# RichealYoung/BRIEF_PyTorch

Hardware: AMD Instinct MI355X
Metric: encode_voxels_per_sec (higher is better)
Workload: dtype f32; 1 GPU; SingleTask 512^3 synthetic uint16 volume, SIREN 4x256 (layers=5, features=256, w0=20), randompoint sample_size=100000, datal2, Adamax lr=1e-3; layers=5, features=256, sample_size=100000, params=198657

## Files before the change

### brief_pytorch_amd/csrc/brief_device.inc

```
typedef float f32x16 __attribute__((ext_vector_type(16)));
#define MFMA(a, b, c) __builtin_amdgcn_mfma_f32_32x32x2f32((a), (b), (c), 0, 0, 0)

#define ROWMAP(r, hi) (((r) & 3) + 8 * ((r) >> 2) + 4 * (hi))
template <int V> struct RoleC { static constexpr int value = V; };

template <int NT, bool INFER = false>
struct KCfg {
    static constexpr int WM = INFER ? brief_wm_infer(NT) : brief_wm(NT);
    static constexpr int WS = 4 / WM;
    static constexpr int MTW = (NT + WM - 1) / WM;
    static constexpr bool EXACT = (NT % WM) == 0;
    static constexpr int FP = 32 * NT;
    static constexpr int XS_FLOATS = WS * NT * 1024;
    static constexpr int TROWS = 32 * MTW;
    static constexpr int RS = (TROWS + 63) / 64;
    static constexpr int T_FLOATS = 4 * TROWS * 33;
    static constexpr int G_FLOATS = 4 * 256;
};

struct GridArgs {
    int ndim;
    int64_t dims[3];
    float lo, hi;
    float step[3];
    int fast;
    uint64_t magic[3];
};

struct BoxArgs {
    int64_t start[3], step[3], extent[3];
    uint64_t magic[3];
    int fast;
};

__device__ __forceinline__ uint32_t fast_div(uint32_t nn, uint64_t magic, uint32_t dv)
{
    return dv == 1 ? nn : (uint32_t)__umul64hi(magic, (uint64_t)nn);
}

struct FusedArgs {
    brief_siren_desc d;
    const float *pk;
    const float *coords;
    const float *targets;
    const float *weights;
    const int64_t *idx;
    int64_t offset;
    int64_t n;
    uint64_t rng_pop, rng_seed, rng_step;
    GridArgs grid;
    int loss_kind;
    float thr, beta, inv_count;
    float *Z;
    float *D;
    int64_t npad;
    float *rec;
    int64_t n_begin, n_end;
    int rec_base;
    void *S16[5];
    float *slabs;
    float *yhat_out;
    void *out;
    int out_kind;
    float scale_min, den, span, vmin;
    int stagger_cus;
    int stagger;
    int pers_wgs;
    int64_t pers_tiles;
    int diag;
};
struct FusedBoxArgs : FusedArgs {
    BoxArgs box;
};
template <bool BOX> struct KArgsT { using type = FusedArgs; };
template <> struct KArgsT<true> { using type = FusedBoxArgs; };
typedef const __attribute__((address_space(4))) FusedBoxArgs *kargs_box;

__device__ __forceinline__ void lds_barrier()
{
    asm volatile("s_waitcnt lgkmcnt(0)" ::: "memory");
    __builtin_amdgcn_s_barrier();
    asm volatile("" ::: "memory");
}

__device__ __forceinline__ float lin_coord(const GridArgs &g, int a, int64_t i)
{
    const int64_t nn = g.dims[a];
    if (nn == 1) return g.lo;
    return i < nn / 2 ? __fmaf_rn(g.step[a], (float)i, g.lo) : __fmaf_rn(-g.step[a], (float)(nn - 1 - i), g.hi);
}

__device__ __forceinline__ float lin_coord32(const GridArgs &g, int a, uint32_t i)
{
    const uint32_t nn = (uint32_t)g.dims[a];
    if (nn == 1) return g.lo;
    return i < nn / 2 ? __fmaf_rn(g.step[a], (float)i, g.lo) : __fmaf_rn(-g.step[a], (float)(nn - 1 - i), g.hi);
}

__device__ __forceinline__ void grid_coords(const GridArgs &g, int cin, int64_t j, float &x0, float &x1, float &x2)
{
    if (cin == 3) {
        int64_t id, ih, iw;
        if (g.fast) {
            const uint32_t ju = (uint32_t)j, d2 = (uint32_t)g.dims[2], d1 = (uint32_t)g.dims[1];
            const uint32_t t2 = fast_div(ju, g.magic[2], d2);
            const uint32_t t1 = fast_div(t2, g.magic[1], d1);
            x0 = lin_coord32(g, 0, t1);
            x1 = lin_coord32(g, 1, t2 - t1 * d1);
            x2 = lin_coord32(g, 2, ju - t2 * d2);
            return;
        } else {
            iw = j % g.dims[2];
            const int64_t t2 = j / g.dims[2];
            ih = t2 % g.dims[1]; id = t2 / g.dims[1];
        }
        x0 = lin_coord(g, 0, id);
        x1 = lin_coord(g, 1, ih);
        x2 = lin_coord(g, 2, iw);
    } else {
        int64_t ih, iw;
        if (g.fast) {
            const uint32_t ju = (uint32_t)j, d1 = (uint32_t)g.dims[1];
            const uint32_t t1 = fast_div(ju, g.magic[1], d1);
            x0 = lin_coord32(g, 0, t1);
            x1 = lin_coord32(g, 1, ju - t1 * d1);
            return;
        } else {
            iw = j % g.dims[1]; ih = j / g.dims[1];
        }
        x0 = lin_coord(g, 0, ih);
        x1 = lin_coord(g, 1, iw);
    }
}

__device__ __forceinline__ void box_coords(const GridArgs &g, int cin, int64_t b, float &x0, float &x1, float &x2)
{
    kargs_box ap = (kargs_box)__builtin_amdgcn_kernarg_segment_ptr();
    asm volatile("" : "+s"(ap));
    uint32_t i0, i1, i2 = 0u;
    if (cin == 3) {
        const uint32_t e2 = (uint32_t)ap->box.extent[2], e1 = (uint32_t)ap->box.extent[1];
        if (ap->box.fast) {
            const uint32_t bu = (uint32_t)b;
            const uint32_t t2 = fast_div(bu, ap->box.magic[2], e2);
            const uint32_t t1 = fast_div(t2, ap->box.magic[1], e1);
            i0 = t1; i1 = t2 - t1 * e1; i2 = bu - t2 * e2;
        } else {
            const int64_t t2 = b / (int64_t)e2, t1 = t2 / (int64_t)e1;
            i0 = (uint32_t)t1; i1 = (uint32_t)(t2 - t1 * e1); i2 = (uint32_t)(b - t2 * e2);
        }
    } else {
        const uint32_t e1 = (uint32_t)ap->box.extent[1];
        if (ap->box.fast) {
            const uint32_t bu = (uint32_t)b;
            const uint32_t t1 = fast_div(bu, ap->box.magic[1], e1);
            i0 = t1; i1 = bu - t1 * e1;
        } else {
            const int64_t t1 = b / (int64_t)e1;
            i0 = (uint32_t)t1; i1 = (uint32_t)(b - t1 * e1);
        }
    }
    x0 = lin_coord32(g, 0, (uint32_t)ap->box.start[0] + (uint32_t)ap->box.step[0] * i0);
    x1 = lin_coord32(g, 1, (uint32_t)ap->box.start[1] + (uint32_t)ap->box.step[1] * i1);
    if (cin == 3) x2 = lin_coord32(g, 2, (uint32_t)ap->box.start[2] + (uint32_t)ap->box.step[2] * i2);
}

template <bool BOX>
__device__ __forceinline__ void sample_coords(const GridArgs &g, int cin, int64_t j, float &x0, float &x1, float &x2)
{
    if constexpr (BOX) box_coords(g, cin, j, x0, x1, x2);
    else grid_coords(g, cin, j, x0, x1, x2);
}

typedef unsigned int u32x4 __attribute__((ext_vector_type(4)));

__device__ __forceinline__ float4 bload4(__amdgpu_buffer_rsrc_t rs, int voff, int soff)
{
    const u32x4 v = __builtin_amdgcn_raw_buffer_load_b128(rs, voff, soff, 0);
    return make_float4(__uint_as_float(v.x), __uint_as_float(v.y), __uint_as_float(v.z), __uint_as_float(v.w));
}
#ifndef BRIEF_WGRAD_AUX
#define BRIEF_WGRAD_AUX 0
#endif
__device__ __forceinline__ float4 bload4w(__amdgpu_buffer_rsrc_t rs, int voff, int soff)
{
    const u32x4 v = __builtin_amdgcn_raw_buffer_load_b128(rs, voff, soff, BRIEF_WGRAD_AUX);
    return make_float4(__uint_as_float(v.x), __uint_as_float(v.y), __uint_as_float(v.z), __uint_as_float(v.w));
}
__device__ __forceinline__ float bload1(__amdgpu_buffer_rsrc_t rs, int voff, int soff)
{
    return __uint_as_float(__builtin_amdgcn_raw_buffer_load_b32(rs, voff, soff, 0));
}
__device__ __forceinline__ void bstore1(float v, __amdgpu_buffer_rsrc_t rs, int voff, int soff)
{
    __builtin_amdgcn_raw_buffer_store_b32(__float_as_uint(v), rs, voff, soff, 0);
}
#ifndef BRIEF_STASH_LD_AUX
#define BRIEF_STASH_LD_AUX 0
#endif
#ifndef BRIEF_X3_STASH_AUX
#define BRIEF_X3_STASH_AUX 0
#endif
__device__ __forceinline__ float bload1s(__amdgpu_buffer_rsrc_t rs, int voff, int soff)
{
    return __uint_as_float(__builtin_amdgcn_raw_buffer_load_b32(rs, voff, soff, BRIEF_STASH_LD_AUX));
}
__device__ __forceinline__ void bstore1s(float v, __amdgpu_buffer_rsrc_t rs, int voff, int soff)
{
    __builtin_amdgcn_raw_buffer_store_b32(__float_as_uint(v), rs, voff, soff, BRIEF_X3_STASH_AUX);
}

template <int NT, bool INFER = false>
__device__ __forceinline__ void chain(f32x16 (&acc)[(KCfg<NT, INFER>::MTW)], __amdgpu_buffer_rsrc_t rs, int soff_layer ,
                                      const float4 *Xs, int wm, int lane, int kit)
{
    using K = KCfg<NT, INFER>;
    constexpr int NIT = NT * 4;
    constexpr int PD = NIT < 4 ? NIT : 4;
    const int voff = lane * 16;
    int soff_w = soff_layer + wm * (NT * 4 * 1024);
    asm volatile("" : "+s"(soff_w));
    constexpr int smul = 1024;
    float4 areg[NIT][K::MTW];
    float4 breg[NIT];
#pragma unroll
    for (int it = 0; it < PD; ++it)
#pragma unroll
        for (int t = 0; t < K::MTW; ++t)
            if (K::EXACT || wm + K::WM * t < NT) areg[it][t] = bload4(rs, voff, soff_w + (K::WM * t * NT * 4 + it) * smul);
    breg[0] = Xs[lane];
#pragma unroll
    for (int it = 0; it < NIT; ++it) {
        if (it >= NIT - 3 && it >= kit) break;
        if (it + PD < NIT) {
#pragma unroll
            for (int t = 0; t < K::MTW; ++t)
                if (K::EXACT || wm + K::WM * t < NT) {
                    areg[it + PD][t] = bload4(rs, voff, soff_w + (K::WM * t * NT * 4 + it + PD) * smul);
                }
        }
        if (it + 1 < NIT) breg[it + 1] = Xs[(it + 1) * 64 + lane];
        __builtin_amdgcn_sched_barrier(0);
        const float4 b = breg[it];
#pragma unroll
        for (int t = 0; t < K::MTW; ++t) {
            if (K::EXACT || wm + K::WM * t < NT) {
                const float4 a = areg[it][t];
                acc[t] = MFMA(a.x, b.x, acc[t]);
                acc[t] = MFMA(a.y, b.y, acc[t]);
                acc[t] = MFMA(a.z, b.z, acc[t]);
                acc[t] = MFMA(a.w, b.w, acc[t]);
            }
        }
    }
}

template <int NT, bool INFER = false>
__device__ __forceinline__ void write_image(float4 *Xs, const f32x16 (&h)[(KCfg<NT, INFER>::MTW)], int wm, int lane)
{
    using K = KCfg<NT, INFER>;
#pragma unroll
    for (int t = 0; t < K::MTW; ++t) {
        const int mt = wm + K::WM * t;
        if (K::EXACT || mt < NT) {
#pragma unroll
            for (int q = 0; q < 4; ++q)
                Xs[(mt * 4 + q) * 64 + lane] = make_float4(h[t][4 * q], h[t][4 * q + 1], h[t][4 * q + 2], h[t][4 * q + 3]);
        }
    }
}

__device__ __forceinline__ void philox_round(uint32_t (&c)[4], uint32_t k0, uint32_t k1)
{
    const uint64_t p0 = (uint64_t)0xD2511F53u * c[0], p1 = (uint64_t)0xCD9E8D57u * c[2];
    const uint32_t n0 = (uint32_t)(p1 >> 32) ^ c[1] ^ k0, n1 = (uint32_t)p1;
    const uint32_t n2 = (uint32_t)(p0 >> 32) ^ c[3] ^ k1, n3 = (uint32_t)p0;
    c[0] = n0; c[1] = n1; c[2] = n2; c[3] = n3;
}

__device__ __forceinline__ int64_t philox_index(int64_t i, uint64_t pop, uint64_t seed, uint64_t step)
{
    uint32_t c[4] = {(uint32_t)i, (uint32_t)((uint64_t)i >> 32), (uint32_t)step, (uint32_t)(step >> 32)};
    uint32_t k0 = (uint32_t)seed, k1 = (uint32_t)(seed >> 32);
#pragma unroll
    for (int r = 0; r < 10; ++r) {
        philox_round(c, k0, k1);
        k0 += 0x9E3779B9u; k1 += 0xBB67AE85u;
    }
    const uint64_t r64 = ((uint64_t)c[0] << 32) | c[1];
    return (int64_t)__umul64hi(r64, pop);
}

#ifndef BRIEF_FUSED64
#ifndef BRIEF_LEAN_RM3
#define BRIEF_LEAN_RM3 1
#endif
#define BRIEF_FUSED64 0
#endif
#ifndef BRIEF_KERNARG_RELOAD
#define BRIEF_KERNARG_RELOAD 1
#endif
#ifndef BRIEF_TRAIN_WPE
#define BRIEF_TRAIN_WPE 2
#endif
#if defined(BRIEF_STAMPS) && BRIEF_STAMPS + 0 != 2
#define STAMP(slot) { const long long t_ = clock64(); st_acc[slot] += (float)(t_ - st_last); st_last = t_; }
#else
#define STAMP(slot)
#endif
```

### brief_pytorch_amd/csrc/brief_fused.inc

```
template <int NT, bool INFER = false>
struct FusedLds {
    using K = KCfg<NT, INFER>;
    static constexpr int R_FLOATS = K::XS_FLOATS > K::T_FLOATS ? K::XS_FLOATS : K::T_FLOATS;
    static constexpr int G_OFF = R_FLOATS;
    static constexpr int HW_OFF = G_OFF + K::G_FLOATS;
    static constexpr int TOTAL = HW_OFF + 4 * K::FP + 4;
};

#ifndef BRIEF_LEAN
#define BRIEF_LEAN 1
#endif
#ifndef BRIEF_LEAN7
#define BRIEF_LEAN7 0
#endif
constexpr bool fused_lean(int NT) { return BRIEF_LEAN && (NT == 8 || NT == BRIEF_LEAN7); }
constexpr int fused_train_wpe(int NT) { return NT > 8 ? 1 : (NT <= 4 || fused_lean(NT) ? (BRIEF_TRAIN_WPE > 3 ? BRIEF_TRAIN_WPE : 3) : BRIEF_TRAIN_WPE); }
template <int NT, bool TRAIN, bool BOX = false>
__global__ __launch_bounds__(256, TRAIN ? fused_train_wpe(NT) : (NT > 8 ? 2 : 3)) void k_fused(const typename KArgsT<BOX>::type a)
{
    static_assert(!(TRAIN && BOX), "the box mapping is an inference instantiation");
#ifdef BRIEF_STAMPS
    float st_acc[10] = {0.f, 0.f, 0.f, 0.f, 0.f, 0.f, 0.f, 0.f, 0.f, 0.f};
    long long st_last = clock64();
    const long long st_c0 = st_last, st_r0 = wall_clock64();
#endif
    using K = KCfg<NT, !TRAIN>;
    using LD = FusedLds<NT, !TRAIN>;
    extern __shared__ __attribute__((aligned(16))) float smem[];
    float4 *X = reinterpret_cast<float4 *>(smem);
    float *T = smem;
    float *G = smem + LD::G_OFF;
    float *HW = smem + LD::HW_OFF;

    const int lane = threadIdx.x & 63;
    const int wave = __builtin_amdgcn_readfirstlane(threadIdx.x >> 6);
    const int hi = lane >> 5, ln = lane & 31;
    const int wm = wave % K::WM, ws = wave / K::WM;
    const brief_siren_desc &d = a.d;
    const int L = d.layers, cin = d.cin, cout = d.cout;
    const int kit = (d.features + 7) >> 3;
    const int64_t npad = a.npad;
    const float *pk = a.pk;
    float4 *Xs = X + ws * (NT * 256);
    float *Tw = T + wave * (K::TROWS * 33);
    float *Gw = G + wave * 256;
    const float4 *W0p = reinterpret_cast<const float4 *>(pk + brief_pk_w0(d));
    const __amdgpu_buffer_rsrc_t rs_pk =
        __builtin_amdgcn_make_buffer_rsrc((void *)pk, 0, (int)(brief_pk_count(d) * 4), 0x00020000);
    const int stash_bytes = (a.diag & 1) ? 0 : (int)((int64_t)K::FP * npad * 4);

    {
        const float *headp = pk + brief_pk_head(d);
        for (int e = threadIdx.x; e < 4 * K::FP + 4; e += 256) HW[e] = headp[e];
    }
    {
        const int slot = (int)blockIdx.x < a.pers_wgs ? blockIdx.x / a.stagger_cus : 0;
        for (int i = 0; i < slot * a.stagger; ++i) __builtin_amdgcn_s_sleep(127);
    }
    lds_barrier();

    float acc0[K::RS][4], accWh[K::RS][4];
#pragma unroll
    for (int rs = 0; rs < K::RS; ++rs)
#pragma unroll
        for (int c = 0; c < 4; ++c) { acc0[rs][c] = 0.f; accWh[rs][c] = 0.f; }
    float accbh[4] = {0.f, 0.f, 0.f, 0.f};
    float lsum = 0.f;

    const bool pers = (int)blockIdx.x < a.pers_wgs;
    const int64_t tile_end = pers ? a.pers_tiles : a.pers_tiles + ((int64_t)blockIdx.x - a.pers_wgs) + 1;
    const int64_t tile_step = pers ? a.pers_wgs : 1;
    for (int64_t tile = pers ? (int64_t)blockIdx.x : a.pers_tiles + ((int64_t)blockIdx.x - a.pers_wgs); tile < tile_end; tile += tile_step) {
        const int64_t n0 = (tile * K::WS + ws) * 32;
        const int64_t n = n0 + ln;
        const bool valid = n < a.n;
#if BRIEF_KERNARG_RELOAD
        typedef const __attribute__((address_space(4))) FusedArgs *kargs_f;
        kargs_f ap = (kargs_f)__builtin_amdgcn_kernarg_segment_ptr();
        asm volatile("" : "+s"(ap));
        const int64_t *k_idx = ap->idx;
        const float *k_tg = ap->targets, *k_wt = ap->weights, *k_co = ap->coords;
        const uint64_t k_pop = ap->rng_pop, k_seed = ap->rng_seed, k_step = ap->rng_step;
        const int64_t k_off = ap->offset;
        GridArgs kg;
        kg.ndim = ap->grid.ndim; kg.lo = ap->grid.lo; kg.hi = ap->grid.hi; kg.fast = ap->grid.fast;
#pragma unroll
        for (int ax = 0; ax < 3; ++ax) { kg.dims[ax] = ap->grid.dims[ax]; kg.step[ax] = ap->grid.step[ax]; kg.magic[ax] = ap->grid.magic[ax]; }
#else
        const int64_t *k_idx = a.idx;
        const float *k_tg = a.targets, *k_wt = a.weights, *k_co = a.coords;
        const uint64_t k_pop = a.rng_pop, k_seed = a.rng_seed, k_step = a.rng_step;
        const int64_t k_off = a.offset;
        const GridArgs &kg = a.grid;
#endif
        int64_t j = 0;
        if (valid) j = k_idx ? k_idx[n] : (k_pop ? philox_index(n, k_pop, k_seed, k_step) : n + k_off);
        float x0 = 0.f, x1 = 0.f, x2 = 0.f;
        float yv[4] = {0.f, 0.f, 0.f, 0.f}, wv4[4] = {1.f, 1.f, 1.f, 1.f};
        if (valid) {
            if (TRAIN) {
#pragma unroll
                for (int c = 0; c < 4; ++c) {
                    if (c < cout) {
                        yv[c] = k_tg[j * cout + c];
                        if (k_wt) wv4[c] = k_wt[j * cout + c];
                    }
                }
            }
            if (k_co) {
                x0 = k_co[j * cin];
                x1 = k_co[j * cin + 1];
                if (cin == 3) x2 = k_co[j * cin + 2];
            } else {
                sample_coords<BOX>(kg, cin, j, x0, x1, x2);
            }
        }
        f32x16 acc[K::MTW];
        f32x16 creg[K::MTW];
        f32x16 hreg[K::MTW];
        float4 bnext[K::MTW][4];
#pragma unroll
        for (int t = 0; t < K::MTW; ++t) {
#pragma unroll
            for (int r = 0; r < 16; ++r) { creg[t][r] = 0.f; hreg[t][r] = 0.f; }
#pragma unroll
            for (int q = 0; q < 4; ++q) bnext[t][q] = make_float4(0.f, 0.f, 0.f, 0.f);
        }
#define FUSED_LOAD_BIAS(layer)                                                                          \
    {                                                                                                   \
        const float *bp_ = pk + brief_pk_hidden(d, (layer)) + 2 * K::FP * K::FP;                        \
        _Pragma("unroll") for (int t = 0; t < K::MTW; ++t) {                                            \
            const int mt = wm + K::WM * t;                                                              \
            if (K::EXACT || mt < NT) {                                                                  \
                _Pragma("unroll") for (int q = 0; q < 4; ++q)                                           \
                    bnext[t][q] = *reinterpret_cast<const float4 *>(bp_ + 32 * mt + 8 * q + 4 * hi);    \
            }                                                                                           \
        }                                                                                               \
    }
        {
            const float b0 = hi ? x1 : x0;
            const float b1 = hi ? 1.0f : x2;
#pragma unroll
            for (int t = 0; t < K::MTW; ++t) {
                const int mt = wm + K::WM * t;
#pragma unroll
                for (int r = 0; r < 16; ++r) acc[t][r] = 0.f;
                if (K::EXACT || mt < NT) {
                    const float4 w = W0p[32 * mt + ln];
                    acc[t] = MFMA(hi ? w.y : w.x, b0, acc[t]);
                    acc[t] = MFMA(hi ? w.w : w.z, b1, acc[t]);
                }
            }
        }
        STAMP(0)
        for (int l = 0; l <= L - 2; ++l) {
            const bool last = (l == L - 2);
            if (l > 0) {
                if (TRAIN && fused_lean(NT)) FUSED_LOAD_BIAS(l)
#pragma unroll
                for (int t = 0; t < K::MTW; ++t) {
#pragma unroll
                    for (int q = 0; q < 4; ++q) {
                        acc[t][4 * q] = bnext[t][q].x; acc[t][4 * q + 1] = bnext[t][q].y;
                        acc[t][4 * q + 2] = bnext[t][q].z; acc[t][4 * q + 3] = bnext[t][q].w;
                    }
                }
                if (TRAIN) __builtin_amdgcn_s_setprio(3);
                chain<NT, !TRAIN>(acc, rs_pk, (int)(brief_pk_hidden(d, l) * 4), Xs, wm, lane, kit);
                if (TRAIN) __builtin_amdgcn_s_setprio(0);
                STAMP(1)
                lds_barrier();
                STAMP(2)
            }
            if (!last && !(TRAIN && fused_lean(NT))) FUSED_LOAD_BIAS(l + 1)
#pragma unroll
            for (int t = 0; t < K::MTW; ++t) {
                const int mt = wm + K::WM * t;
                if (K::EXACT || mt < NT) {
#pragma unroll
                    for (int r = 0; r < 16; ++r) acc[t][r] = __builtin_amdgcn_fractf(acc[t][r]);
                    if (TRAIN && !last) {
                        const __amdgpu_buffer_rsrc_t rz =
                            __builtin_amdgcn_make_buffer_rsrc((void *)(a.Z + (int64_t)l * K::FP * npad), 0, stash_bytes, 0x00020000);
                        const int voff = (int)(n0 * (K::FP * 4)) + ln * 4 + hi * 4 * 128;
#pragma unroll
                        for (int r = 0; r < 16; ++r)
                            bstore1(acc[t][r], rz, voff, (32 * mt + (r & 3) + 8 * (r >> 2)) * 128);
                    }
#pragma unroll
                    for (int r = 0; r < 16; ++r) hreg[t][r] = BRIEF_SIN_REV(acc[t][r]);
                }
            }
            if (TRAIN && last) {
                asm volatile("" ::: "memory");
#pragma unroll
                for (int t = 0; t < K::MTW; ++t) {
                    if (K::EXACT || wm + K::WM * t < NT) {
#pragma unroll
                        for (int r = 0; r < 16; ++r) creg[t][r] = BRIEF_COS_REV(acc[t][r]);
                    }
                }
            }
            write_image<NT, !TRAIN>(Xs, hreg, wm, lane);
            STAMP(3)
            lds_barrier();
            STAMP(4)
        }
        float zo[4], yh[4], g[4];
#pragma unroll
        for (int c = 0; c < 4; ++c) {
            zo[c] = 0.f; yh[c] = 0.f; g[c] = 0.f;
            if (c < cout) {
                float p = 0.f;
                const float *wrow = HW + c * K::FP;
#pragma unroll
                for (int kt = 0; kt < NT; ++kt) {
#pragma unroll
                    for (int q = 0; q < 4; ++q) {
                        const float4 hv = Xs[(kt * 4 + q) * 64 + lane];
                        const float4 wv = *reinterpret_cast<const float4 *>(wrow + 32 * kt + 8 * q + 4 * hi);
                        p = __fmaf_rn(wv.x, hv.x, p); p = __fmaf_rn(wv.y, hv.y, p);
                        p = __fmaf_rn(wv.z, hv.z, p); p = __fmaf_rn(wv.w, hv.w, p);
                    }
                }
                p += __shfl_xor(p, 32);
                zo[c] = p + HW[4 * K::FP + c];
                yh[c] = d.output_act ? brief_fast_sinf(d.w0_hidden * zo[c]) : zo[c];
            }
        }
        if (!TRAIN) {
            if (wm == 0 && hi == 0 && valid) {
#pragma unroll
                for (int c = 0; c < 4; ++c) {
                    if (c >= cout) break;
                    if (a.out_kind == BRIEF_OUT_F32) {
                        reinterpret_cast<float *>(a.out)[n * cout + c] = yh[c];
                    } else {
                        float t = __fsub_rn(yh[c], a.scale_min);
                        t = __fdiv_rn(t, a.den);
                        t = fminf(fmaxf(t, 0.f), 1.f);
                        const float u = __fadd_rn(__fmul_rn(t, a.span), a.vmin);
                        if (a.out_kind == BRIEF_OUT_U16) reinterpret_cast<uint16_t *>(a.out)[n * cout + c] = (uint16_t)(int)u;
                        else reinterpret_cast<uint8_t *>(a.out)[n * cout + c] = (uint8_t)(int)u;
                    }
                }
            }
            lds_barrier();
            continue;
        }
#pragma unroll
        for (int c = 0; c < 4; ++c) {
            if (c < cout && valid) {
                float we = wv4[c];
                if (a.thr != 0.f && yh[c] <= a.thr) we = 1.0f;
                const float df = yh[c] - yv[c];
                float li, gi;
                if (a.loss_kind == BRIEF_LOSS_L2) { li = df * df; gi = 2.0f * df; }
                else if (a.loss_kind == BRIEF_LOSS_SMOOTHL1) {
                    const float ad = fabsf(df);
                    if (ad < a.beta) { li = 0.5f * df * df / a.beta; gi = df / a.beta; }
                    else { li = ad - 0.5f * a.beta; gi = df < 0.f ? -1.0f : 1.0f; }
                } else { li = 0.f; gi = 0.f; }
                if (wm == 0 && hi == 0) lsum += li * we;
                g[c] = a.loss_kind == BRIEF_LOSS_EXTERNAL ? yv[c] : gi * we * a.inv_count;
                if (d.output_act) g[c] *= d.w0_hidden * brief_fast_cosf(d.w0_hidden * zo[c]);
                if (a.yhat_out && wm == 0 && hi == 0) a.yhat_out[n * cout + c] = yh[c];
            }
        }
        STAMP(5)
        lds_barrier();
#pragma unroll
        for (int t = 0; t < K::MTW; ++t) {
#pragma unroll
            for (int r = 0; r < 16; ++r) Tw[(32 * t + ROWMAP(r, hi)) * 33 + ln] = hreg[t][r];
        }
        if (hi == 0) *reinterpret_cast<float4 *>(Gw + ln * 4) = make_float4(g[0], g[1], g[2], g[3]);
        else *reinterpret_cast<float4 *>(Gw + 128 + ln * 4) = make_float4(x0, x1, x2, 1.0f);
        lds_barrier();
#pragma unroll
        for (int rs = 0; rs < K::RS; ++rs) {
            float4 sW = make_float4(0.f, 0.f, 0.f, 0.f), sb = make_float4(0.f, 0.f, 0.f, 0.f);
            const int row = lane + 64 * rs;
            const float *trow = Tw + (row < K::TROWS ? row : 0) * 33;
            if (cout == 1) {
#pragma unroll 8
                for (int s = 0; s < 32; ++s) {
                    const float gv = Gw[s * 4];
                    sW.x = __fmaf_rn(trow[s], gv, sW.x);
                    sb.x += gv;
                }
            } else {
#pragma unroll 4
                for (int s = 0; s < 32; ++s) {
                    const float hv = trow[s];
                    const float4 gv = *reinterpret_cast<const float4 *>(Gw + s * 4);
                    sW.x = __fmaf_rn(hv, gv.x, sW.x); sW.y = __fmaf_rn(hv, gv.y, sW.y);
                    sW.z = __fmaf_rn(hv, gv.z, sW.z); sW.w = __fmaf_rn(hv, gv.w, sW.w);
                    sb.x += gv.x; sb.y += gv.y; sb.z += gv.z; sb.w += gv.w;
                }
            }
            if (row < K::TROWS) { accWh[rs][0] += sW.x; accWh[rs][1] += sW.y; accWh[rs][2] += sW.z; accWh[rs][3] += sW.w; }
            if (rs == 0) { accbh[0] += sb.x; accbh[1] += sb.y; accbh[2] += sb.z; accbh[3] += sb.w; }
        }
        f32x16 dl[K::MTW];
        float gom[4];
        {
            const float om_top = (L - 2) == 0 ? d.w0_first : d.w0_hidden;
#pragma unroll
            for (int c = 0; c < 4; ++c) gom[c] = om_top * g[c];
        }
#pragma unroll
        for (int t = 0; t < K::MTW; ++t) {
            const int mt = wm + K::WM * t;
#pragma unroll
            for (int r = 0; r < 16; ++r) dl[t][r] = 0.f;
            if (K::EXACT || mt < NT) {
#pragma unroll
                for (int q = 0; q < 4; ++q) {
                    float4 sacc = make_float4(0.f, 0.f, 0.f, 0.f);
#pragma unroll
                    for (int c = 0; c < 4; ++c) {
                        if (c < cout) {
                            const float4 wv = *reinterpret_cast<const float4 *>(HW + c * K::FP + 32 * mt + 8 * q + 4 * hi);
                            sacc.x = __fmaf_rn(wv.x, gom[c], sacc.x); sacc.y = __fmaf_rn(wv.y, gom[c], sacc.y);
                            sacc.z = __fmaf_rn(wv.z, gom[c], sacc.z); sacc.w = __fmaf_rn(wv.w, gom[c], sacc.w);
                        }
                    }
                    dl[t][4 * q] = creg[t][4 * q] * sacc.x; dl[t][4 * q + 1] = creg[t][4 * q + 1] * sacc.y;
                    dl[t][4 * q + 2] = creg[t][4 * q + 2] * sacc.z; dl[t][4 * q + 3] = creg[t][4 * q + 3] * sacc.w;
                }
            }
        }
        STAMP(6)
        for (int l = L - 2; l >= 1; --l) {
            const __amdgpu_buffer_rsrc_t rd =
                __builtin_amdgcn_make_buffer_rsrc((void *)(a.D + (int64_t)(l - 1) * K::FP * npad), 0, stash_bytes, 0x00020000);
            const int voff_s = (int)(n0 * (K::FP * 4)) + ln * 4 + hi * 4 * 128;
#pragma unroll
            for (int t = 0; t < K::MTW; ++t) {
                const int mt = wm + K::WM * t;
                if (K::EXACT || mt < NT) {
#pragma unroll
                    for (int r = 0; r < 16; ++r)
                        bstore1(dl[t][r], rd, voff_s, (32 * mt + (r & 3) + 8 * (r >> 2)) * 128);
                }
            }
            const __amdgpu_buffer_rsrc_t rzp =
                __builtin_amdgcn_make_buffer_rsrc((void *)(a.Z + (int64_t)(l - 1) * K::FP * npad), 0, stash_bytes, 0x00020000);
            float zr[K::MTW][16];
            constexpr bool ZPRE = !fused_lean(NT);
#define FUSED_LOAD_Z()                                                                                  \
    _Pragma("unroll") for (int t = 0; t < K::MTW; ++t) {                                                \
        const int mt = wm + K::WM * t;                                                                  \
        _Pragma("unroll") for (int r = 0; r < 16; ++r) {                                                \
            zr[t][r] = 0.f;                                                                             \
            if (K::EXACT || mt < NT) zr[t][r] = bload1s(rzp, voff_s, (32 * mt + (r & 3) + 8 * (r >> 2)) * 128); \
        }                                                                                               \
    }
            if (ZPRE) FUSED_LOAD_Z()
            STAMP(7)
            lds_barrier();
            write_image<NT, !TRAIN>(Xs, dl, wm, lane);
            lds_barrier();
            STAMP(8)
#pragma unroll
            for (int t = 0; t < K::MTW; ++t)
#pragma unroll
                for (int r = 0; r < 16; ++r) acc[t][r] = 0.f;
            __builtin_amdgcn_s_setprio(3);
            chain<NT, !TRAIN>(acc, rs_pk, (int)((brief_pk_hidden(d, l) + K::FP * K::FP) * 4), Xs, wm, lane, kit);
            __builtin_amdgcn_s_setprio(0);
            STAMP(9)
            if (!ZPRE) FUSED_LOAD_Z()
#undef FUSED_LOAD_Z
#pragma unroll
            for (int t = 0; t < K::MTW; ++t) {
                const int mt = wm + K::WM * t;
                if (K::EXACT || mt < NT) {
#pragma unroll
                    for (int r = 0; r < 16; ++r)
                        dl[t][r] = acc[t][r] * BRIEF_COS_REV(zr[t][r]);
                }
            }
        }
        STAMP(7)
        lds_barrier();
#pragma unroll
        for (int t = 0; t < K::MTW; ++t) {
#pragma unroll
            for (int r = 0; r < 16; ++r) Tw[(32 * t + ROWMAP(r, hi)) * 33 + ln] = dl[t][r];
        }
        lds_barrier();
#pragma unroll
        for (int rs = 0; rs < K::RS; ++rs) {
            float4 s0 = make_float4(0.f, 0.f, 0.f, 0.f);
            const int row = lane + 64 * rs;
            const float *trow = Tw + (row < K::TROWS ? row : 0) * 33;
#pragma unroll 4
            for (int s = 0; s < 32; ++s) {
                const float dv = trow[s];
                const float4 xv = *reinterpret_cast<const float4 *>(Gw + 128 + s * 4);
                s0.x = __fmaf_rn(dv, xv.x, s0.x); s0.y = __fmaf_rn(dv, xv.y, s0.y);
                s0.z = __fmaf_rn(dv, xv.z, s0.z); s0.w = __fmaf_rn(dv, xv.w, s0.w);
            }
            if (row < K::TROWS) { acc0[rs][0] += s0.x; acc0[rs][1] += s0.y; acc0[rs][2] += s0.z; acc0[rs][3] += s0.w; }
        }
        lds_barrier();
        STAMP(6)
    }
#undef FUSED_LOAD_BIAS
    if (TRAIN) {
        float *rec = a.rec + (((int64_t)blockIdx.x + a.rec_base) * 4 + wave) * BRIEF_REC_FLOATS;
#pragma unroll
        for (int rs = 0; rs < K::RS; ++rs) {
            const int row = lane + 64 * rs;
            if (row < 128) {
#pragma unroll
                for (int c = 0; c < 4; ++c) {
                    rec[row * 4 + c] = acc0[rs][c];
                    rec[BRIEF_REC_DWH + c * 128 + row] = accWh[rs][c];
                }
            }
        }
        for (int off = 32; off >= 1; off >>= 1) lsum += __shfl_xor(lsum, off);
        if (lane == 0) {
#pragma unroll
            for (int c = 0; c < 4; ++c) rec[BRIEF_REC_DBH + c] = accbh[c];
            rec[BRIEF_REC_LOSS] = lsum;
#ifdef BRIEF_STAMPS
            for (int i = 0; i < 10; ++i) rec[BRIEF_REC_STAMPS + i] = st_acc[i];
            rec[BRIEF_REC_STAMPS + 10] = (float)(clock64() - st_c0);
            rec[BRIEF_REC_STAMPS + 11] = (float)(wall_clock64() - st_r0);
            rec[BRIEF_REC_STAMPS + 12] = (float)(st_r0 & 0xFFFFFF);
            rec[BRIEF_REC_STAMPS + 13] = (float)(__builtin_amdgcn_s_getreg(20 | (0 << 6) | (3 << 11)) & 15);
            rec[BRIEF_REC_STAMPS + 14] = (float)(__builtin_amdgcn_s_getreg(4 | (0 << 6) | (15 << 11)) & 0xFFFF);
#endif
        }
    }
}
```

### brief_pytorch_amd/csrc/brief_layout.h

```cpp
#pragma once
#include <stddef.h>
#include <stdint.h>
#include "../../include/brief_hip.h"

#if defined(__HIPCC__)
#define BL_HD __host__ __device__ __forceinline__
#else
#define BL_HD static inline
#endif

#define BRIEF_MAX_NT 128
#define BRIEF_REC_FLOATS 1056
#define BRIEF_REC_DWH 512
#define BRIEF_REC_DBH 1024
#define BRIEF_REC_LOSS 1028
#define BRIEF_REC_STAMPS 1030
BL_HD int brief_rec_tr(int nt) { return nt > 32 ? 32 * ((nt + 3) / 4) : (nt > 16 ? 256 : 128); }
BL_HD int brief_rec_floats(int nt) { return 8 * brief_rec_tr(nt) + 32; }

BL_HD int64_t brief_canon_hidden_off(const brief_siren_desc &d, int l )
{
    const int64_t F = d.features;
    return F * d.cin + F + (int64_t)(l - 1) * (F * F + F);
}
BL_HD int64_t brief_canon_head_off(const brief_siren_desc &d)
{
    const int64_t F = d.features;
    return F * d.cin + F + (int64_t)(d.layers - 2) * (F * F + F);
}
BL_HD int64_t brief_canon_count(const brief_siren_desc &d)
{
    return brief_canon_head_off(d) + (int64_t)d.features * d.cout + d.cout;
}

BL_HD int brief_nt(const brief_siren_desc &d)
{
    const int nt = (d.features + 31) / 32;
    if (d.precision == BRIEF_PREC_BF16) return nt <= 8 ? 8 : 16;
    if (d.precision == BRIEF_PREC_BF16X3) return 8;
    return nt;
}
#ifndef BRIEF_LEAN3
#define BRIEF_LEAN3 1
#endif
BL_HD bool brief_use_wide(const brief_siren_desc &d) { return d.precision == BRIEF_PREC_F32 && (d.features + 31) / 32 > 32; }
BL_HD bool brief_use_lean(const brief_siren_desc &d, bool train)
{
    const int nt = brief_nt(d);
    if (nt > 32) return false;
    if (train) return (nt >= 5 && nt != 8) || (BRIEF_LEAN3 && nt == 3);
    return (nt >= 5 && nt <= 7) || (nt >= 9 && nt != 12 && nt != 16);
}
BL_HD int64_t brief_pk_w0(const brief_siren_desc &) { return 0; }
BL_HD int64_t brief_pk_hidden_stride(const brief_siren_desc &d)
{
    const int64_t FP = 32 * brief_nt(d);
    return 2 * FP * FP + FP;
}
BL_HD int64_t brief_pk_hidden(const brief_siren_desc &d, int l )
{
    const int64_t FP = 32 * brief_nt(d);
    return FP * 4 + (int64_t)(l - 1) * brief_pk_hidden_stride(d);
}
BL_HD int64_t brief_pk_head(const brief_siren_desc &d)
{
    const int64_t FP = 32 * brief_nt(d);
    return FP * 4 + (int64_t)(d.layers - 2) * brief_pk_hidden_stride(d);
}
BL_HD int64_t brief_pk_count32(const brief_siren_desc &d)
{
    const int64_t FP = 32 * brief_nt(d);
    return brief_pk_head(d) + 4 * FP + 4;
}
BL_HD int64_t brief_pk16_off(const brief_siren_desc &d, int l )
{
    const int64_t FP = 32 * brief_nt(d);
    return ((brief_pk_count32(d) + 3) / 4) * 4 + (int64_t)(l - 1) * FP * FP;
}
BL_HD int64_t brief_pk16_region(const brief_siren_desc &d)
{
    const int64_t FP = 32 * brief_nt(d), hidden = d.layers - 2 > 0 ? d.layers - 2 : 0;
    return hidden * FP * FP;
}
BL_HD int64_t brief_pk_count(const brief_siren_desc &d)
{
    if (d.precision == BRIEF_PREC_BF16) return brief_pk16_off(d, 1) + brief_pk16_region(d);
    if (d.precision == BRIEF_PREC_BF16X3) return brief_pk16_off(d, 1) + 2 * brief_pk16_region(d);
    return brief_pk_count32(d);
}
BL_HD int64_t brief_frag16_index(int NT, int row, int col)
{
    const int mt = row >> 5, i = row & 31, kt = col >> 5, rem = col & 31;
    const int s = rem >> 4, r16 = rem & 15, hi = (r16 >> 2) & 1, j = ((r16 >> 3) << 2) | (r16 & 3);
    return ((((int64_t)mt * NT + kt) * 2 + s) * 64 + 32 * hi + i) * 8 + j;
}

BL_HD float brief_om_prev(const brief_siren_desc &d, int l) { return l - 1 == 0 ? d.w0_first : d.w0_hidden; }
BL_HD float brief_phase_scale(const brief_siren_desc &d, int l) { return (l == 0 ? d.w0_first : d.w0_hidden) * 0.15915494309189535f; }

BL_HD constexpr int brief_wm(int nt) { return nt >= 3 ? 4 : nt; }
BL_HD constexpr int brief_wm_infer(int nt) { return nt == 3 ? 1 : (nt == 5 ? 4 : brief_wm(nt)); }
BL_HD constexpr int brief_ws(int nt) { return 4 / brief_wm(nt); }
BL_HD int64_t brief_wg_samples(int nt) { return 32 * brief_ws(nt); }
BL_HD int64_t brief_npad(int nt, int64_t n)
{
    const int64_t g = brief_wg_samples(nt);
    return (n + g - 1) / g * g;
}
BL_HD int64_t brief_npad_d(const brief_siren_desc &d, int64_t n) { return brief_npad(brief_nt(d), n); }
```

### brief_pytorch_amd/csrc/brief_lean.inc

```
#ifndef BRIEF_LEAN_KTAIL
#define BRIEF_LEAN_KTAIL 1
#endif
constexpr bool lean_ktail(int MTW, bool train) { return BRIEF_LEAN_KTAIL && (!train || MTW != 2); }
struct LeanLds { int r, g_off, hw_off, part_off, total; };
__host__ __device__ inline LeanLds lean_lds(int SH, int MTW, int nt)
{
    LeanLds l;
    const int img = SH * nt * 1024, t = SH * 4 * 32 * MTW * 33;
    l.r = img > t ? img : t;
    l.g_off = l.r;
    l.hw_off = l.g_off + 4 * 256;
    l.part_off = l.hw_off + 4 * 32 * nt;
    l.total = l.part_off + SH * 4 * 32 * 4;
    return l;
}

template <int SH, int MTW, int RM, bool KTAIL>
__device__ __forceinline__ void lean_chain_rt(f32x16 (&acc)[SH][MTW], f32x16 &px, __amdgpu_buffer_rsrc_t rs, int soff_layer , const float4 *X,
                                              int wave, int lane, int nt, int kit, bool two)
{
    constexpr int KF = RM == 0 ? MTW : MTW - 1;
    const int voff = lane * 16;
    const int HALF = nt * 256;
    const int rho = RM == 1 ? ((wave + 1) & 3) : (RM == 2 ? (((wave >> 1) + 1) & 1) : (RM == 3 ? ((0x3201 >> (4 * wave)) & 3) : 0));
    int soff_t[KF > 0 ? KF : 1];
#pragma unroll
    for (int t = 0; t < KF; ++t) {
        const int mt = wave + 4 * t;
        soff_t[t] = soff_layer + (mt < nt ? mt : nt - 1) * nt * 4096;
    }
    const int soff_e = soff_layer + (RM == 1 ? nt - 1 : (RM == 2 ? nt - 2 + (wave & 1) : nt - 3 + ((wave + 1) >> 1))) * nt * 4096;
    const int soff_a = soff_layer + (nt - 3 + (wave & 2)) * nt * 4096;
    float4 areg[4][KF > 0 ? KF : 1];
    float4 aext[RM == 3 ? 3 : 2];
#pragma unroll
    for (int q = 0; q < 4; ++q) {
        const int it0 = (q + rho) & 3;
#pragma unroll
        for (int t = 0; t < KF; ++t) areg[q][t] = bload4(rs, voff, soff_t[t] + it0 * 1024);
        if ((RM == 1 && q == 3) || (RM == 2 && (q & 1))) aext[q >> 1] = bload4(rs, voff, soff_e + it0 * 1024);
        if (RM == 3 && q < 3) aext[q] = bload4(rs, voff, (q == 0 ? soff_a : soff_e) + it0 * 1024);
        __builtin_amdgcn_sched_barrier(0);
    }
#define LEAN_POS_MFMAS(q, B)                                                                                 \
    {                                                                                                        \
        _Pragma("unroll") for (int t = 0; t < KF; ++t) {                                                     \
            const float4 a = areg[q][t];                                                                     \
            _Pragma("unroll") for (int h = 0; h < SH; ++h) {                                                 \
                if (SH == 2 && h == 1 && !two) continue;                                                     \
                acc[h][t] = MFMA(a.x, B[h].x, acc[h][t]);                                                    \
                acc[h][t] = MFMA(a.y, B[h].y, acc[h][t]);                                                    \
                acc[h][t] = MFMA(a.z, B[h].z, acc[h][t]);                                                    \
                acc[h][t] = MFMA(a.w, B[h].w, acc[h][t]);                                                    \
            }                                                                                                \
        }                                                                                                    \
        if ((RM == 1 && q == 3) || (RM == 2 && (q & 1)) || (RM == 3 && (q == 1 || q == 2))) {                \
            const float4 a = aext[RM == 3 ? q : q >> 1];                                                     \
            _Pragma("unroll") for (int h = 0; h < SH; ++h) {                                                 \
                if (SH == 2 && h == 1 && !two) continue;                                                     \
                acc[h][MTW - 1] = MFMA(a.x, B[h].x, acc[h][MTW - 1]);                                        \
                acc[h][MTW - 1] = MFMA(a.y, B[h].y, acc[h][MTW - 1]);                                        \
                acc[h][MTW - 1] = MFMA(a.z, B[h].z, acc[h][MTW - 1]);                                        \
                acc[h][MTW - 1] = MFMA(a.w, B[h].w, acc[h][MTW - 1]);                                        \
            }                                                                                                \
        }                                                                                                    \
        if (RM == 3 && q == 0) {                                                                             \
            const float4 a = aext[0];                                                                        \
            px = MFMA(a.x, B[0].x, px); px = MFMA(a.y, B[0].y, px);                                          \
            px = MFMA(a.z, B[0].z, px); px = MFMA(a.w, B[0].w, px);                                          \
        }                                                                                                    \
    }
    float4 bcur[SH], bnxt[SH];
#pragma unroll
    for (int h = 0; h < SH; ++h) bcur[h] = X[h * HALF + rho * 64 + lane];
    const int nkt = KTAIL ? kit >> 2 : (kit + 3) >> 2;
    for (int kt = 0; kt < nkt; ++kt) {
#pragma unroll
        for (int q = 0; q < 4; ++q) {
            const int it = kt * 4 + ((q + rho) & 3);
            const int itn = q < 3 ? kt * 4 + ((q + 1 + rho) & 3) : kt * 4 + 4 + rho;
#pragma unroll
            for (int h = 0; h < SH; ++h) bnxt[h] = X[h * HALF + itn * 64 + lane];
            __builtin_amdgcn_sched_barrier(0);
            LEAN_POS_MFMAS(q, bcur)
            __builtin_amdgcn_sched_barrier(0);
#pragma unroll
            for (int t = 0; t < KF; ++t) areg[q][t] = bload4(rs, voff, soff_t[t] + (it + 4) * 1024);
            if ((RM == 1 && q == 3) || (RM == 2 && (q & 1))) aext[q >> 1] = bload4(rs, voff, soff_e + (it + 4) * 1024);
            if (RM == 3 && q < 3) aext[q] = bload4(rs, voff, (q == 0 ? soff_a : soff_e) + (it + 4) * 1024);
#pragma unroll
            for (int h = 0; h < SH; ++h) bcur[h] = bnxt[h];
        }
    }
    if (KTAIL && (kit & 3)) {
#pragma unroll
        for (int q = 0; q < 4; ++q) {
            const int it = nkt * 4 + ((q + rho) & 3);
            if (it < kit) {
                float4 bt[SH];
#pragma unroll
                for (int h = 0; h < SH; ++h) bt[h] = X[h * HALF + it * 64 + lane];
                LEAN_POS_MFMAS(q, bt)
            }
        }
    }
#undef LEAN_POS_MFMAS
}

template <int SH, int MTW, int RM>
__device__ __forceinline__ void lean_fold_shared(f32x16 (&acc)[SH][MTW], float *PS, int wave, int lane, bool two)
{
    if (RM != 0) {
        const bool giver = RM == 1 ? wave != 0 : wave >= 2;
        const int slot = RM == 1 ? wave - 1 : wave - 2;
        if (giver) {
#pragma unroll
            for (int h = 0; h < SH; ++h) {
                if (SH == 2 && h == 1 && !two) continue;
#pragma unroll
                for (int r = 0; r < 16; ++r) PS[((h * 3 + slot) * 16 + r) * 64 + lane] = acc[h][MTW - 1][r];
            }
        }
    }
    lds_barrier();
    if (RM == 1 && wave == 0) {
#pragma unroll
        for (int h = 0; h < SH; ++h) {
            if (SH == 2 && h == 1 && !two) continue;
#pragma unroll
            for (int s3 = 0; s3 < 3; ++s3)
#pragma unroll
                for (int r = 0; r < 16; ++r) acc[h][MTW - 1][r] += PS[((h * 3 + s3) * 16 + r) * 64 + lane];
        }
    }
    if (RM == 2 && wave < 2) {
#pragma unroll
        for (int h = 0; h < SH; ++h) {
            if (SH == 2 && h == 1 && !two) continue;
#pragma unroll
            for (int r = 0; r < 16; ++r) acc[h][MTW - 1][r] += PS[((h * 3 + wave) * 16 + r) * 64 + lane];
        }
    }
}

template <int MTW>
__device__ __forceinline__ void lean_fold3(f32x16 (&acc)[1][MTW], f32x16 &px, float *img, int wave, int lane)
{
    lds_barrier();
    if (wave == 3) {
#pragma unroll
        for (int r = 0; r < 16; ++r) img[2048 + r * 64 + lane] = acc[0][MTW - 1][r] + px[r];
    } else if (wave == 2) {
#pragma unroll
        for (int r = 0; r < 16; ++r) { img[1024 + r * 64 + lane] = acc[0][MTW - 1][r]; acc[0][MTW - 1][r] = px[r]; }
    } else if (wave == 1) {
#pragma unroll
        for (int r = 0; r < 16; ++r) img[r * 64 + lane] = px[r];
    } else {
#pragma unroll
        for (int r = 0; r < 16; ++r) acc[0][MTW - 1][r] += px[r];
    }
    lds_barrier();
    if (wave < 3) {
#pragma unroll
        for (int r = 0; r < 16; ++r) acc[0][MTW - 1][r] += img[wave * 1024 + r * 64 + lane];
    }
}

template <int SH, int MTW, int NTC>
__device__ __forceinline__ void lean_chain_ct(f32x16 (&acc)[SH][MTW], __amdgpu_buffer_rsrc_t rs, int soff_layer , const float4 *X,
                                              int wave, int lane, int kit, bool two)
{
    constexpr int NT = NTC > 0 ? NTC : 1, NIT = NT * 4, PD = 4, HALF = NT * 256;
    constexpr bool EXACT = MTW * 4 == NT;
    const int voff = lane * 16;
    int soff_w = soff_layer + wave * (NT * 4 * 1024);
    asm volatile("" : "+s"(soff_w));
    float4 areg[NIT][MTW];
    float4 breg[NIT][SH];
#pragma unroll
    for (int it = 0; it < PD; ++it)
#pragma unroll
        for (int t = 0; t < MTW; ++t)
            if (EXACT || wave + 4 * t < NT) areg[it][t] = bload4(rs, voff, soff_w + (4 * t * NT * 4 + it) * 1024);
#pragma unroll
    for (int h = 0; h < SH; ++h) breg[0][h] = X[h * HALF + lane];
#pragma unroll
    for (int it = 0; it < NIT; ++it) {
        if (it >= NIT - 3 && it >= kit) break;
        if (it + PD < NIT) {
#pragma unroll
            for (int t = 0; t < MTW; ++t)
                if (EXACT || wave + 4 * t < NT) areg[it + PD][t] = bload4(rs, voff, soff_w + (4 * t * NT * 4 + it + PD) * 1024);
        }
        if (it + 1 < NIT) {
#pragma unroll
            for (int h = 0; h < SH; ++h) breg[it + 1][h] = X[h * HALF + (it + 1) * 64 + lane];
        }
        __builtin_amdgcn_sched_barrier(0);
#pragma unroll
        for (int t = 0; t < MTW; ++t) {
            if (EXACT || wave + 4 * t < NT) {
                const float4 a = areg[it][t];
#pragma unroll
                for (int h = 0; h < SH; ++h) {
                    if (h == 1 && !two) continue;
                    const float4 b = breg[it][h];
                    acc[h][t] = MFMA(a.x, b.x, acc[h][t]);
                    acc[h][t] = MFMA(a.y, b.y, acc[h][t]);
                    acc[h][t] = MFMA(a.z, b.z, acc[h][t]);
                    acc[h][t] = MFMA(a.w, b.w, acc[h][t]);
                }
            }
        }
    }
}

#ifndef BRIEF_LEAN_WPE2
#define BRIEF_LEAN_WPE2 3
#endif
constexpr int lean_wpe(int SH, int MTW) { return SH == 1 && MTW <= 2 ? BRIEF_LEAN_WPE2 : (SH == 2 || MTW <= 4 ? 2 : 1); }

template <int SH, int MTW, int NTC, bool TRAIN, int RM = 0, bool BOX = false>
__global__ __launch_bounds__(256, lean_wpe(SH, MTW)) void k_lean(const typename KArgsT<BOX>::type a)
{
    static_assert(!(TRAIN && BOX), "the box mapping is an inference instantiation");
    static_assert(SH == 1 || SH == 2, "one or two 32-sample halves per tile");
    static_assert(RM == 0 || (NTC == 0 && SH == 1 && (MTW >= 2 || RM == 3)), "shared left-over tiles: run-time widths only (MTW = 1: the three tiles of a 3-tile net)");
    constexpr int TROWS = 32 * MTW;
    constexpr int RS = (TROWS + 63) / 64;
    constexpr int TR = MTW > 4 ? 256 : 128;
    const brief_siren_desc &d = a.d;
    const int nt = NTC > 0 ? NTC : brief_nt(d);
    const int FP = 32 * nt, HALF = nt * 256;
    extern __shared__ __attribute__((aligned(16))) float smem[];
    const LeanLds lds = lean_lds(SH, MTW, nt);
    float4 *X = reinterpret_cast<float4 *>(smem);
    float *T = smem;
    float *G = smem + lds.g_off;
    float *HW = smem + lds.hw_off;
    float4 *PART = reinterpret_cast<float4 *>(smem + lds.part_off);
    const int lane = threadIdx.x & 63;
    const int wave_hw = __builtin_amdgcn_readfirstlane(threadIdx.x >> 6);
    const int wave = (NTC == 0 && lean_wpe(SH, MTW) == 2) ? ((wave_hw + 2 * (((int)blockIdx.x / a.stagger_cus) & 1)) & 3) : wave_hw;
    const int hi = lane >> 5, ln = lane & 31;
    const int L = d.layers, cin = d.cin, cout = d.cout;
    const int kit = (d.features + 7) >> 3;
    const int64_t npad = a.npad;
    const float *pk = a.pk;
    float *Gw = G + wave * 256;
    const float4 *W0p = reinterpret_cast<const float4 *>(pk + brief_pk_w0(d));
    const __amdgpu_buffer_rsrc_t rs_pk = __builtin_amdgcn_make_buffer_rsrc((void *)pk, 0, (int)(brief_pk_count(d) * 4), 0x00020000);
    const int stash_bytes = (int)((int64_t)FP * npad * 4);
    const int64_t hstride = brief_pk_hidden_stride(d);
    bool tv[MTW];
#pragma unroll
    for (int t = 0; t < MTW; ++t) tv[t] = wave + 4 * t < nt;
    {
        const float *headp = pk + brief_pk_head(d);
        for (int e = threadIdx.x; e < 4 * FP; e += 256) HW[e] = headp[e];
    }
    lds_barrier();
    float acc0[RS][4], accWh[RS][4];
#pragma unroll
    for (int rs = 0; rs < RS; ++rs)
#pragma unroll
        for (int c = 0; c < 4; ++c) { acc0[rs][c] = 0.f; accWh[rs][c] = 0.f; }
    float accbh[4] = {0.f, 0.f, 0.f, 0.f};
    float lsum = 0.f;
    const int64_t T0 = SH == 1 ? a.n_begin >> 5 : 0;
    const int64_t Hn = ((SH == 1 && a.n_end > 0 ? a.n_end : a.n) + 31) >> 5;
    const int64_t G_ = gridDim.x, w_ = blockIdx.x;
    const int64_t R_ = SH == 2 ? Hn / (2 * G_) : (Hn - T0 > w_ ? (Hn - T0 - w_ + G_ - 1) / G_ : 0);
    const int64_t Hr = Hn - 2 * G_ * R_;
    const int64_t npair_x = Hr > G_ ? Hr - G_ : 0;
    const int64_t nsing_x = Hr > G_ ? G_ - npair_x : Hr;
    const int extra = SH == 2 ? (w_ < npair_x ? 2 : (w_ < npair_x + nsing_x ? 1 : 0)) : 0;
    const int64_t ht_x = 2 * G_ * R_ + (w_ < npair_x ? 2 * w_ : 2 * npair_x + (w_ - npair_x));
    for (int64_t it_ = 0; it_ < R_ + (extra ? 1 : 0); ++it_) {
        const int64_t ht = SH == 2 ? (it_ < R_ ? 2 * (it_ * G_ + w_) : ht_x) : T0 + it_ * G_ + w_;
        const bool two = SH == 2 && (it_ < R_ || extra == 2);
        typedef const __attribute__((address_space(4))) FusedArgs *kargs_f;
        kargs_f ap = (kargs_f)__builtin_amdgcn_kernarg_segment_ptr();
        asm volatile("" : "+s"(ap));
        const int64_t *k_idx = ap->idx;
        const float *k_tg = ap->targets, *k_wt = ap->weights, *k_co = ap->coords;
        const uint64_t k_pop = ap->rng_pop, k_seed = ap->rng_seed, k_step = ap->rng_step;
        const int64_t k_off = ap->offset;
        GridArgs kg;
        kg.ndim = ap->grid.ndim; kg.lo = ap->grid.lo; kg.hi = ap->grid.hi; kg.fast = ap->grid.fast;
#pragma unroll
        for (int ax = 0; ax < 3; ++ax) { kg.dims[ax] = ap->grid.dims[ax]; kg.step[ax] = ap->grid.step[ax]; kg.magic[ax] = ap->grid.magic[ax]; }
        float x0[SH], x1[SH], x2[SH];
        int64_t jidx[SH];
        bool valid[SH];
        f32x16 acc[SH][MTW];
        f32x16 px;
        {
            const int64_t n64 = ht * 32 + (SH == 2 ? lane : ln);
            const bool v64 = (SH == 1 || lane < 32 || two) && n64 < a.n;
            int64_t j = 0;
            if (v64) j = k_idx ? k_idx[n64] : (k_pop ? philox_index(n64, k_pop, k_seed, k_step) : n64 + k_off);
            float c0 = 0.f, c1 = 0.f, c2 = 0.f;
            if (v64) {
                if (k_co) {
                    c0 = k_co[j * cin];
                    c1 = k_co[j * cin + 1];
                    if (cin == 3) c2 = k_co[j * cin + 2];
                } else {
                    sample_coords<BOX>(kg, cin, j, c0, c1, c2);
                }
            }
            if (SH == 2) {
                const int jl = (int)(uint32_t)(uint64_t)j, jh = (int)(uint32_t)((uint64_t)j >> 32);
#pragma unroll
                for (int h = 0; h < SH; ++h) {
                    const int src = 32 * h + ln;
                    x0[h] = __shfl(c0, src); x1[h] = __shfl(c1, src); x2[h] = __shfl(c2, src);
                    jidx[h] = (int64_t)(((uint64_t)(uint32_t)__shfl(jh, src) << 32) | (uint32_t)__shfl(jl, src));
                    valid[h] = (h == 0 || two) && (ht + h) * 32 + ln < a.n;
                }
            } else {
                x0[0] = c0; x1[0] = c1; x2[0] = c2; jidx[0] = j; valid[0] = v64;
            }
        }
#pragma unroll
        for (int h = 0; h < SH; ++h) {
            const float b0 = hi ? x1[h] : x0[h];
            const float b1 = hi ? 1.0f : x2[h];
#pragma unroll
            for (int t = 0; t < MTW; ++t) {
#pragma unroll
                for (int r = 0; r < 16; ++r) acc[h][t][r] = 0.f;
                if (tv[t]) {
                    const float4 w = W0p[32 * (wave + 4 * t) + ln];
                    acc[h][t] = MFMA(hi ? w.y : w.x, b0, acc[h][t]);
                    acc[h][t] = MFMA(hi ? w.w : w.z, b1, acc[h][t]);
                }
            }
        }
        for (int l = 0; l <= L - 2; ++l) {
            const bool last = (l == L - 2);
            if (l > 0) {
                const float *bp_ = pk + FP * 4 + (int64_t)(l - 1) * hstride + 2 * (int64_t)FP * FP;
#pragma unroll
                for (int t = 0; t < MTW; ++t) {
                    if (tv[t]) {
#pragma unroll
                        for (int q = 0; q < 4; ++q) {
                            const float4 b4 = *reinterpret_cast<const float4 *>(bp_ + 32 * (wave + 4 * t) + 8 * q + 4 * hi);
#pragma unroll
                            for (int h = 0; h < SH; ++h) {
                                acc[h][t][4 * q] = b4.x; acc[h][t][4 * q + 1] = b4.y; acc[h][t][4 * q + 2] = b4.z; acc[h][t][4 * q + 3] = b4.w;
                            }
                        }
                    } else if (RM != 0 && t == MTW - 1) {
#pragma unroll
                        for (int h = 0; h < SH; ++h)
#pragma unroll
                            for (int r = 0; r < 16; ++r) acc[h][t][r] = 0.f;
                    }
                }
                const int soff_l = (int)((FP * 4 + (int64_t)(l - 1) * hstride) * 4);
                __builtin_amdgcn_s_setprio(3);
                if (RM == 3) {
#pragma unroll
                    for (int r = 0; r < 16; ++r) {
                        px[r] = wave == 2 ? acc[0][MTW - 1][r] : 0.f;
                        if (wave == 2) acc[0][MTW - 1][r] = 0.f;
                    }
                }
                if (NTC > 0) lean_chain_ct<SH, MTW, NTC>(acc, rs_pk, soff_l, X, wave, lane, kit, two);
                else lean_chain_rt<SH, MTW, RM, lean_ktail(MTW, TRAIN)>(acc, px, rs_pk, soff_l, X, wave, lane, nt, kit, two);
                __builtin_amdgcn_s_setprio(0);
                if constexpr (RM == 3) lean_fold3<MTW>(acc, px, T, wave, lane);
                else lean_fold_shared<SH, MTW, RM>(acc, T + SH * nt * 1024, wave, lane, two);
                if (RM != 0 && TRAIN && last) lds_barrier();
            }
            float pph[SH][4];
#pragma unroll
            for (int h = 0; h < SH; ++h) {
#pragma unroll
                for (int c = 0; c < 4; ++c) pph[h][c] = 0.f;
                if (h == 1 && !two) continue;
                const int voff = (int)(((ht + h) * 32) * ((int64_t)FP * 4)) + ln * 4 + hi * 4 * 128;
#pragma unroll
                for (int t = 0; t < MTW; ++t) {
                    if (!tv[t]) continue;
                    const int mt = wave + 4 * t;
#pragma unroll
                    for (int r = 0; r < 16; ++r) acc[h][t][r] = __builtin_amdgcn_fractf(acc[h][t][r]);
                    f32x16 hv;
                    if (!last) {
                        if (TRAIN) {
                            const __amdgpu_buffer_rsrc_t rz =
                                __builtin_amdgcn_make_buffer_rsrc((void *)(a.Z + (int64_t)l * FP * npad), 0, stash_bytes, 0x00020000);
#pragma unroll
                            for (int r = 0; r < 16; ++r) bstore1(acc[h][t][r], rz, voff, (32 * mt + (r & 3) + 8 * (r >> 2)) * 128);
                        }
#pragma unroll
                        for (int r = 0; r < 16; ++r) hv[r] = BRIEF_SIN_REV(acc[h][t][r]);
#pragma unroll
                        for (int q = 0; q < 4; ++q)
                            X[h * HALF + (mt * 4 + q) * 64 + lane] = make_float4(hv[4 * q], hv[4 * q + 1], hv[4 * q + 2], hv[4 * q + 3]);
                    } else {
#pragma unroll
                        for (int r = 0; r < 16; ++r) { hv[r] = BRIEF_SIN_REV(acc[h][t][r]); if (TRAIN) acc[h][t][r] = BRIEF_COS_REV(acc[h][t][r]); }
#pragma unroll
                        for (int c = 0; c < 4; ++c) {
                            if (c < cout) {
#pragma unroll
                                for (int q = 0; q < 4; ++q) {
                                    const float4 wv = *reinterpret_cast<const float4 *>(HW + c * FP + 32 * mt + 8 * q + 4 * hi);
                                    pph[h][c] = __fmaf_rn(wv.x, hv[4 * q], pph[h][c]); pph[h][c] = __fmaf_rn(wv.y, hv[4 * q + 1], pph[h][c]);
                                    pph[h][c] = __fmaf_rn(wv.z, hv[4 * q + 2], pph[h][c]); pph[h][c] = __fmaf_rn(wv.w, hv[4 * q + 3], pph[h][c]);
                                }
                            }
                        }
                        if (TRAIN) {
                            float *Th = T + (wave * SH + h) * (TROWS * 33);
#pragma unroll
                            for (int r = 0; r < 16; ++r) Th[(32 * t + ROWMAP(r, hi)) * 33 + ln] = hv[r];
                        }
                    }
                }
                if (last) {
#pragma unroll
                    for (int c = 0; c < 4; ++c) pph[h][c] += __shfl_xor(pph[h][c], 32);
                    if (hi == 0) PART[(h * 4 + wave) * 32 + ln] = make_float4(pph[h][0], pph[h][1], pph[h][2], pph[h][3]);
                }
            }
            lds_barrier();
        }
        float zo[SH][4], yh[SH][4], g[SH][4];
#pragma unroll
        for (int h = 0; h < SH; ++h) {
            float4 tot = PART[(h * 4) * 32 + ln];
#pragma unroll
            for (int w = 1; w < 4; ++w) {
                const float4 v = PART[(h * 4 + w) * 32 + ln];
                tot.x += v.x; tot.y += v.y; tot.z += v.z; tot.w += v.w;
            }
            const float tt[4] = {tot.x, tot.y, tot.z, tot.w};
            const int64_t n = (ht + h) * 32 + ln;
#pragma unroll
            for (int c = 0; c < 4; ++c) {
                zo[h][c] = 0.f; yh[h][c] = 0.f; g[h][c] = 0.f;
                if (c < cout) {
                    zo[h][c] = tt[c] + pk[brief_pk_head(d) + 4 * (int64_t)FP + c];
                    yh[h][c] = d.output_act ? brief_fast_sinf(d.w0_hidden * zo[h][c]) : zo[h][c];
                }
                if (!TRAIN) {
                    if (c < cout && valid[h] && wave == 0 && hi == 0) {
                        if (a.out_kind == BRIEF_OUT_F32) {
                            reinterpret_cast<float *>(a.out)[n * cout + c] = yh[h][c];
                        } else {
                            float t_ = __fsub_rn(yh[h][c], a.scale_min);
                            t_ = __fdiv_rn(t_, a.den);
                            t_ = fminf(fmaxf(t_, 0.f), 1.f);
                            const float u_ = __fadd_rn(__fmul_rn(t_, a.span), a.vmin);
                            if (a.out_kind == BRIEF_OUT_U16) reinterpret_cast<uint16_t *>(a.out)[n * cout + c] = (uint16_t)(int)u_;
                            else reinterpret_cast<uint8_t *>(a.out)[n * cout + c] = (uint8_t)(int)u_;
                        }
                    }
                    continue;
                }
                if (c < cout && valid[h]) {
                    const float yvc = k_tg[jidx[h] * cout + c];
                    float we = k_wt ? k_wt[jidx[h] * cout + c] : 1.0f;
                    if (a.thr != 0.f && yh[h][c] <= a.thr) we = 1.0f;
                    const float df = yh[h][c] - yvc;
                    float li, gi;
                    if (a.loss_kind == BRIEF_LOSS_L2) { li = df * df; gi = 2.0f * df; }
                    else if (a.loss_kind == BRIEF_LOSS_SMOOTHL1) {
                        const float ad = fabsf(df);
                        if (ad < a.beta) { li = 0.5f * df * df / a.beta; gi = df / a.beta; }
                        else { li = ad - 0.5f * a.beta; gi = df < 0.f ? -1.0f : 1.0f; }
                    } else { li = 0.f; gi = 0.f; }
                    if (wave == 0 && hi == 0) lsum += li * we;
                    g[h][c] = a.loss_kind == BRIEF_LOSS_EXTERNAL ? yvc : gi * we * a.inv_count;
                    if (d.output_act) g[h][c] *= d.w0_hidden * brief_fast_cosf(d.w0_hidden * zo[h][c]);
                    if (a.yhat_out && wave == 0 && hi == 0) a.yhat_out[n * cout + c] = yh[h][c];
                }
            }
        }
        if (!TRAIN) {
            lds_barrier();
            continue;
        }
#pragma unroll
        for (int h = 0; h < SH; ++h) {
            if (h == 1 && !two) continue;
            if (hi == 0) *reinterpret_cast<float4 *>(Gw + ln * 4) = make_float4(g[h][0], g[h][1], g[h][2], g[h][3]);
            asm volatile("s_waitcnt lgkmcnt(0)" ::: "memory");
#pragma unroll
            for (int rs = 0; rs < RS; ++rs) {
                float4 sW = make_float4(0.f, 0.f, 0.f, 0.f), sb = make_float4(0.f, 0.f, 0.f, 0.f);
                const int row = lane + 64 * rs;
                const float *trow = T + (wave * SH + h) * (TROWS * 33) + (row < TROWS ? row : 0) * 33;
                if (cout == 1) {
#pragma unroll 8
                    for (int s = 0; s < 32; ++s) {
                        const float gv = Gw[s * 4];
                        sW.x = __fmaf_rn(trow[s], gv, sW.x);
                        sb.x += gv;
                    }
                } else {
#pragma unroll 4
                    for (int s = 0; s < 32; ++s) {
                        const float hv = trow[s];
                        const float4 gv = *reinterpret_cast<const float4 *>(Gw + s * 4);
                        sW.x = __fmaf_rn(hv, gv.x, sW.x); sW.y = __fmaf_rn(hv, gv.y, sW.y);
                        sW.z = __fmaf_rn(hv, gv.z, sW.z); sW.w = __fmaf_rn(hv, gv.w, sW.w);
                        sb.x += gv.x; sb.y += gv.y; sb.z += gv.z; sb.w += gv.w;
                    }
                }
                if (row < TROWS) { accWh[rs][0] += sW.x; accWh[rs][1] += sW.y; accWh[rs][2] += sW.z; accWh[rs][3] += sW.w; }
                if (rs == 0) { accbh[0] += sb.x; accbh[1] += sb.y; accbh[2] += sb.z; accbh[3] += sb.w; }
            }
            asm volatile("s_waitcnt lgkmcnt(0)" ::: "memory");
        }
        {
            const float om_top = (L - 2) == 0 ? d.w0_first : d.w0_hidden;
#pragma unroll
            for (int h = 0; h < SH; ++h) {
                if (h == 1 && !two) continue;
                float gom[4];
#pragma unroll
                for (int c = 0; c < 4; ++c) gom[c] = om_top * g[h][c];
#pragma unroll
                for (int t = 0; t < MTW; ++t) {
                    if (!tv[t]) continue;
                    const int mt = wave + 4 * t;
#pragma unroll
                    for (int q = 0; q < 4; ++q) {
                        float4 sacc = make_float4(0.f, 0.f, 0.f, 0.f);
#pragma unroll
                        for (int c = 0; c < 4; ++c) {
                            if (c < cout) {
                                const float4 wv = *reinterpret_cast<const float4 *>(HW + c * FP + 32 * mt + 8 * q + 4 * hi);
                                sacc.x = __fmaf_rn(wv.x, gom[c], sacc.x); sacc.y = __fmaf_rn(wv.y, gom[c], sacc.y);
                                sacc.z = __fmaf_rn(wv.z, gom[c], sacc.z); sacc.w = __fmaf_rn(wv.w, gom[c], sacc.w);
                            }
                        }
                        acc[h][t][4 * q] *= sacc.x; acc[h][t][4 * q + 1] *= sacc.y;
                        acc[h][t][4 * q + 2] *= sacc.z; acc[h][t][4 * q + 3] *= sacc.w;
                    }
                }
            }
        }
        for (int l = L - 2; l >= 1; --l) {
            const __amdgpu_buffer_rsrc_t rd =
                __builtin_amdgcn_make_buffer_rsrc((void *)(a.D + (int64_t)(l - 1) * FP * npad), 0, stash_bytes, 0x00020000);
            const __amdgpu_buffer_rsrc_t rzp =
                __builtin_amdgcn_make_buffer_rsrc((void *)(a.Z + (int64_t)(l - 1) * FP * npad), 0, stash_bytes, 0x00020000);
#pragma unroll
            for (int h = 0; h < SH; ++h) {
                if (h == 1 && !two) continue;
                const int voff_s = (int)(((ht + h) * 32) * ((int64_t)FP * 4)) + ln * 4 + hi * 4 * 128;
#pragma unroll
                for (int t = 0; t < MTW; ++t) {
                    if (!tv[t]) continue;
                    const int mt = wave + 4 * t;
#pragma unroll
                    for (int r = 0; r < 16; ++r) bstore1(acc[h][t][r], rd, voff_s, (32 * mt + (r & 3) + 8 * (r >> 2)) * 128);
                }
            }
            lds_barrier();
#pragma unroll
            for (int h = 0; h < SH; ++h) {
                if (h == 1 && !two) continue;
#pragma unroll
                for (int t = 0; t < MTW; ++t) {
                    if (!tv[t]) continue;
                    const int mt = wave + 4 * t;
#pragma unroll
                    for (int q = 0; q < 4; ++q)
                        X[h * HALF + (mt * 4 + q) * 64 + lane] = make_float4(acc[h][t][4 * q], acc[h][t][4 * q + 1], acc[h][t][4 * q + 2], acc[h][t][4 * q + 3]);
                }
            }
            lds_barrier();
#pragma unroll
            for (int h = 0; h < SH; ++h)
#pragma unroll
                for (int t = 0; t < MTW; ++t)
#pragma unroll
                    for (int r = 0; r < 16; ++r) acc[h][t][r] = 0.f;
            const int soff_b = (int)((FP * 4 + (int64_t)(l - 1) * hstride + (int64_t)FP * FP) * 4);
            __builtin_amdgcn_s_setprio(3);
            if (RM == 3) {
#pragma unroll
                for (int r = 0; r < 16; ++r) px[r] = 0.f;
            }
            if (NTC > 0) lean_chain_ct<SH, MTW, NTC>(acc, rs_pk, soff_b, X, wave, lane, kit, two);
            else lean_chain_rt<SH, MTW, RM, lean_ktail(MTW, TRAIN)>(acc, px, rs_pk, soff_b, X, wave, lane, nt, kit, two);
            __builtin_amdgcn_s_setprio(0);
            if constexpr (RM == 3) lean_fold3<MTW>(acc, px, T, wave, lane);
            else if (RM != 0) lean_fold_shared<SH, MTW, RM>(acc, T + SH * nt * 1024, wave, lane, two);
#pragma unroll
            for (int h = 0; h < SH; ++h) {
                if (h == 1 && !two) continue;
                const int voff_s = (int)(((ht + h) * 32) * ((int64_t)FP * 4)) + ln * 4 + hi * 4 * 128;
#pragma unroll
                for (int t2 = 0; t2 < MTW; t2 += 2) {
                    float zr[2][16];
#pragma unroll
                    for (int u = 0; u < 2; ++u) {
                        const int t = t2 + u;
                        if (t < MTW && tv[t < MTW ? t : 0]) {
                            const int mt = wave + 4 * t;
#pragma unroll
                            for (int r = 0; r < 16; ++r) zr[u][r] = bload1s(rzp, voff_s, (32 * mt + (r & 3) + 8 * (r >> 2)) * 128);
                        }
                    }
#pragma unroll
                    for (int u = 0; u < 2; ++u) {
                        const int t = t2 + u;
                        if (t < MTW && tv[t < MTW ? t : 0]) {
#pragma unroll
                            for (int r = 0; r < 16; ++r) acc[h][t < MTW ? t : 0][r] *= BRIEF_COS_REV(zr[u][r]);
                        }
                    }
                }
            }
        }
#pragma unroll
        for (int h = 0; h < SH; ++h) {
            if (h == 1 && !two) continue;
            if (h == 0) lds_barrier();
            float *Tf = T + (wave * SH + h) * (TROWS * 33);
#pragma unroll
            for (int t = 0; t < MTW; ++t)
#pragma unroll
                for (int r = 0; r < 16; ++r) Tf[(32 * t + ROWMAP(r, hi)) * 33 + ln] = acc[h][t][r];
            if (hi == 1) *reinterpret_cast<float4 *>(Gw + 128 + ln * 4) = make_float4(x0[h], x1[h], x2[h], 1.0f);
            asm volatile("s_waitcnt lgkmcnt(0)" ::: "memory");
#pragma unroll
            for (int rs = 0; rs < RS; ++rs) {
                float4 s0 = make_float4(0.f, 0.f, 0.f, 0.f);
                const int row = lane + 64 * rs;
                const float *trow = Tf + (row < TROWS ? row : 0) * 33;
#pragma unroll 4
                for (int s = 0; s < 32; ++s) {
                    const float dv = trow[s];
                    const float4 xv = *reinterpret_cast<const float4 *>(Gw + 128 + s * 4);
                    s0.x = __fmaf_rn(dv, xv.x, s0.x); s0.y = __fmaf_rn(dv, xv.y, s0.y);
                    s0.z = __fmaf_rn(dv, xv.z, s0.z); s0.w = __fmaf_rn(dv, xv.w, s0.w);
                }
                if (row < TROWS) { acc0[rs][0] += s0.x; acc0[rs][1] += s0.y; acc0[rs][2] += s0.z; acc0[rs][3] += s0.w; }
            }
            asm volatile("s_waitcnt lgkmcnt(0)" ::: "memory");
        }
        lds_barrier();
    }
    if (!TRAIN) return;
    float *rec = a.rec + (((int64_t)blockIdx.x + a.rec_base) * 4 + wave) * (8 * TR + 32);
#pragma unroll
    for (int rs = 0; rs < RS; ++rs) {
        const int row = lane + 64 * rs;
        if (row < TROWS) {
#pragma unroll
            for (int c = 0; c < 4; ++c) {
                rec[row * 4 + c] = acc0[rs][c];
                rec[4 * TR + c * TR + row] = accWh[rs][c];
            }
        }
    }
    for (int off = 32; off >= 1; off >>= 1) lsum += __shfl_xor(lsum, off);
    if (lane == 0) {
#pragma unroll
        for (int c = 0; c < 4; ++c) rec[8 * TR + c] = accbh[c];
        rec[8 * TR + 4] = lsum;
    }
}
```

### brief_pytorch_amd/csrc/brief_wgrad.inc

```
struct WgradArgs {
    brief_siren_desc d;
    const float *Z;
    const float *D;
    int64_t npad;
    int nsplit;
    int64_t kb_lo, kb_hi;
    int split_lo, nsplit_here;
    int uneven, n_norm;
    int64_t kfix_n, kfix_s;
    float *slabs;
    float *stamps;
};

constexpr int wgrad_nq(int NT) { return (NT + 7) / 8; }
constexpr int wgrad_qt(int NT) { return (NT + wgrad_nq(NT) - 1) / wgrad_nq(NT); }
#ifndef BRIEF_WGRAD_XSPLIT
#define BRIEF_WGRAD_XSPLIT 1
#endif
#ifndef BRIEF_WGRAD_LIST
#define BRIEF_WGRAD_LIST(QT) ((QT) == 3 || (QT) == 5)
#endif
#ifndef BRIEF_WGRAD_STAGE_BIAS
#define BRIEF_WGRAD_STAGE_BIAS 1
#endif
#ifndef BRIEF_WGRAD_FRAG_PIPE
#define BRIEF_WGRAD_FRAG_PIPE 1
#endif
#ifndef BRIEF_WGRAD_FRAG_PIPE2
#define BRIEF_WGRAD_FRAG_PIPE2 1
#endif
constexpr int wgrad_wmk(int QT) { return QT >= 2 ? 2 : 1; }
constexpr int wgrad_wnk(int QT) { return QT >= 7 ? 4 : (QT >= 2 ? 2 : 1); }
constexpr bool wgrad_list(int QT) { return BRIEF_WGRAD_LIST(QT); }
constexpr int wgrad_wk(int QT) { return QT >= 7 || wgrad_list(QT) ? 1 : (QT >= 2 ? 2 : 4); }
constexpr int wgrad_lds_floats(int NT)
{
    const int QT = wgrad_qt(NT);
    const int WMk = wgrad_wmk(QT), WNk = wgrad_wnk(QT), WK = wgrad_wk(QT);
    const int NWv = WMk * WNk, TN = (QT + WNk - 1) / WNk;
    const int fold = (WK - 1) * NWv * TN * 1024 + (WK - 1) * NWv * 64, panels = 4 * 32 * QT * 36;
    return fold > panels ? fold : panels;
}

template <int NT, int QTR = 0>
__global__ __launch_bounds__(512, 2) void k_wgrad(const WgradArgs a)
{
    constexpr bool RTW = NT == 0;
    const int nt_w = RTW ? brief_nt(a.d) : NT;
    const int FP = 32 * nt_w;
    const int NQ = RTW ? (nt_w + 7) / 8 : wgrad_nq(NT);
    constexpr int QT = RTW ? QTR : wgrad_qt(NT), QP = 32 * QT;
    constexpr bool LIST = wgrad_list(QT);
    constexpr int LCNT = QT * QT / 8, LREM = QT * QT % 8;
    constexpr bool HET7 = QT == 7 && !LIST;
    constexpr bool XS = BRIEF_WGRAD_XSPLIT && (LIST || HET7) && QT * QT % 8 == 1;
    constexpr int XSLOT = LIST ? LCNT : 6;
    constexpr int WMk = HET7 || LIST ? 2 : wgrad_wmk(QT), WNk = HET7 || LIST ? 4 : wgrad_wnk(QT);
    constexpr int WK = wgrad_wk(QT);
    constexpr int NWv = WMk * WNk;
    constexpr int TM = HET7 || LIST ? 1 : (QT + WMk - 1) / WMk, TN = LIST ? LCNT + (LREM ? 1 : 0) : (HET7 ? 7 : (QT + WNk - 1) / WNk);
    constexpr bool MEX = QT % WMk == 0, NEX = QT % WNk == 0;
    constexpr int LDSW = 36;
    constexpr int NLD = (QP * 8 + 511) / 512;
    constexpr int PANEL = QP * LDSW;
    constexpr bool FULL = (QP * 8) % 512 == 0;
    extern __shared__ __attribute__((aligned(16))) float smem[];

    const int tid = threadIdx.x;
    const int lane = tid & 63;
    const int wave = __builtin_amdgcn_readfirstlane(tid >> 6);
    const int hi = lane >> 5, ln = lane & 31;
    const int wk = wave / NWv, wrem = wave % NWv;
    const int wmk = wrem / WNk, wnk = wrem % WNk;
    const bool kactive = wk < WK;
    const int quad = blockIdx.x % (NQ * NQ), bsl = blockIdx.x / (NQ * NQ);
    const int qm = quad / NQ, qn = quad % NQ;
    const bool uneven = RTW && a.uneven;
    const int hidden_l = a.d.layers - 2;
    const int l = uneven ? 1 + bsl % hidden_l : 1 + bsl / a.nsplit_here;
    const int split = uneven ? bsl / hidden_l : bsl % a.nsplit_here;
    const int64_t nchunks = a.kb_hi - a.kb_lo;
    int64_t c0 = a.kb_lo + nchunks * split / a.nsplit_here, c1 = a.kb_lo + nchunks * (split + 1) / a.nsplit_here;
    if (uneven) {
        const int g0 = a.split_lo + split, g1 = g0 + 1;
        c0 = (g0 <= a.n_norm ? g0 * a.kfix_n : a.n_norm * a.kfix_n + (g0 - a.n_norm) * a.kfix_s) >> 16;
        c1 = g1 >= a.nsplit ? a.kb_hi : ((g1 <= a.n_norm ? g1 * a.kfix_n : a.n_norm * a.kfix_n + (g1 - a.n_norm) * a.kfix_s) >> 16);
    }
    const float *Dl = a.D + (int64_t)(l - 1) * FP * a.npad + qm * QP * 32;
    const float *Zl = a.Z + (int64_t)(l - 1) * FP * a.npad + qn * QP * 32;

    f32x16 acc[TM][TN];
    float dbacc[TM];
#pragma unroll
    for (int i = 0; i < TM; ++i) {
        dbacc[i] = 0.f;
#pragma unroll
        for (int jn = 0; jn < TN; ++jn)
#pragma unroll
            for (int r = 0; r < 16; ++r) acc[i][jn][r] = 0.f;
    }
    float dbl[LIST ? TN : 1];
    int lmt[LIST ? TN : 1], lnt[LIST ? TN : 1];
    if (LIST) {
        const int first = XS ? wave * LCNT : wave * LCNT + (wave > 8 - LREM ? wave - (8 - LREM) : 0);
#pragma unroll
        for (int k = 0; k < TN; ++k) {
            const int t = first + k < QT * QT ? first + k : QT * QT - 1;
            lmt[k] = t / QT; lnt[k] = t % QT; dbl[k] = 0.f;
        }
    }
    constexpr bool SBIAS = BRIEF_WGRAD_STAGE_BIAS && QT == 8;
    const bool want_bias = SBIAS && qn == 0;
    float bsum[NLD];
#pragma unroll
    for (int i = 0; i < NLD; ++i) bsum[i] = 0.f;
    float4 ra[NLD], rb[NLD];
    const int panel_bytes = (int)((int64_t)FP * a.npad * 4) - (RTW ? 0 : (NQ - 1) * QP * 128);
    const int rows_m = RTW ? FP - qm * QP : QP, rows_n = RTW ? FP - qn * QP : QP;
    const __amdgpu_buffer_rsrc_t rsD = __builtin_amdgcn_make_buffer_rsrc((void *)Dl, 0, panel_bytes, 0x00020000);
    const __amdgpu_buffer_rsrc_t rsZ = __builtin_amdgcn_make_buffer_rsrc((void *)Zl, 0, panel_bytes, 0x00020000);
    int voffs[NLD];
#pragma unroll
    for (int i = 0; i < NLD; ++i) {
        const int e = tid + 512 * i;
        voffs[i] = e * 16;
    }
#define WG_ISSUE(cc)                                                                              \
    _Pragma("unroll") for (int i = 0; i < NLD; ++i) {                                             \
        const int e = tid + 512 * i;                                                              \
        ra[i] = make_float4(0.f, 0.f, 0.f, 0.f);                                                  \
        rb[i] = make_float4(0.f, 0.f, 0.f, 0.f);                                                  \
        if (FULL || e < QP * 8) {                                                                 \
            if (!RTW || (e >> 3) < rows_m) ra[i] = bload4w(rsD, voffs[i], (int)((cc) * (FP * 128)));     \
            if (!RTW || (e >> 3) < rows_n) rb[i] = bload4w(rsZ, voffs[i], (int)((cc) * (FP * 128)));     \
        }                                                                                         \
    }
#define WG_STAGE_A(buf, i)                                                                        \
    {                                                                                             \
        const int e = tid + 512 * (i);                                                            \
        if (FULL || e < QP * 8)                                                                   \
            *reinterpret_cast<float4 *>(smem + (buf) * 2 * PANEL + (e >> 3) * LDSW + (e & 7) * 4) = ra[i]; \
    }
#define WG_STAGE_B(buf, i)                                                                        \
    {                                                                                             \
        const int e = tid + 512 * (i);                                                            \
        if (FULL || e < QP * 8) {                                                                 \
            float4 h;                                                                             \
            h.x = BRIEF_SIN_REV(rb[i].x); h.y = BRIEF_SIN_REV(rb[i].y);    \
            h.z = BRIEF_SIN_REV(rb[i].z); h.w = BRIEF_SIN_REV(rb[i].w);                           \
            *reinterpret_cast<float4 *>(smem + (buf) * 2 * PANEL + PANEL + (e >> 3) * LDSW + (e & 7) * 4) = h; \
        }                                                                                         \
    }
#define WG_BIAS_M(i, cm_) { bsum[i] = __fmaf_rn((cm_), (ra[i].x + ra[i].y) + (ra[i].z + ra[i].w), bsum[i]); }
#define WG_BIAS(i) WG_BIAS_M(i, 1.0f)
    WG_ISSUE(c0)
#pragma unroll
    for (int i = 0; i < NLD; ++i) { WG_STAGE_A(0, i) WG_STAGE_B(0, i) }
    if (want_bias) {
#pragma unroll
        for (int i = 0; i < NLD; ++i) WG_BIAS(i)
    }
    {
        const int64_t cn = c0 + 1 < c1 ? c0 + 1 : c1 - 1;
        WG_ISSUE(cn)
    }
    lds_barrier();
#ifdef BRIEF_STAMPS
    float st_acc[10] = {0.f, 0.f, 0.f, 0.f, 0.f, 0.f, 0.f, 0.f, 0.f, 0.f};
    long long st_last = clock64();
#endif
    if constexpr (LIST || HET7) {
    auto chunk_loop = [&](auto role_c) __attribute__((always_inline)) {
    constexpr int ROLE = decltype(role_c)::value;
    for (int64_t c = c0; c < c1; ++c) {
        const int cur = (int)(c - c0) & 1;
        const float *As = smem + cur * 2 * PANEL, *Bs = As + PANEL;
        const float cm_l = want_bias && c + 1 < c1 ? 1.0f : 0.0f;
        STAMP(0)
        if constexpr (LIST) {
            constexpr int CNT = XS ? LCNT : LCNT + ROLE;
#pragma unroll
            for (int gq = 0; gq < 4; ++gq) {
#pragma unroll
                for (int k = 0; k < CNT; ++k) {
                    const float4 a_ = *reinterpret_cast<const float4 *>(As + (32 * lmt[k] + ln) * LDSW + 8 * gq + 4 * hi);
                    const float4 b_ = *reinterpret_cast<const float4 *>(Bs + (32 * lnt[k] + ln) * LDSW + 8 * gq + 4 * hi);
                    if (!SBIAS) dbl[k] += (a_.x + a_.y) + (a_.z + a_.w);
                    acc[0][k] = MFMA(a_.x, b_.x, acc[0][k]); acc[0][k] = MFMA(a_.y, b_.y, acc[0][k]);
                    acc[0][k] = MFMA(a_.z, b_.z, acc[0][k]); acc[0][k] = MFMA(a_.w, b_.w, acc[0][k]);
                }
                if (XS && gq == ROLE) {
                    const float4 a_ = *reinterpret_cast<const float4 *>(As + (32 * (QT - 1) + ln) * LDSW + 8 * gq + 4 * hi);
                    const float4 b_ = *reinterpret_cast<const float4 *>(Bs + (32 * (QT - 1) + ln) * LDSW + 8 * gq + 4 * hi);
                    acc[0][XSLOT] = MFMA(a_.x, b_.x, acc[0][XSLOT]); acc[0][XSLOT] = MFMA(a_.y, b_.y, acc[0][XSLOT]);
                    acc[0][XSLOT] = MFMA(a_.z, b_.z, acc[0][XSLOT]); acc[0][XSLOT] = MFMA(a_.w, b_.w, acc[0][XSLOT]);
                }
                if (gq >= 2) {
#pragma unroll
                    for (int i = 0; i < NLD; ++i)
                        if ((i & 1) == (gq & 1)) { WG_STAGE_A(cur ^ 1, i) WG_STAGE_B(cur ^ 1, i) if (SBIAS) WG_BIAS_M(i, cm_l) }
                }
            }
        } else if constexpr (HET7) {
#define WG_FRAG(P, row) (*reinterpret_cast<const float4 *>((P) + (32 * (row) + ln) * LDSW + 8 * gq + 4 * hi))
#define WG_MFMA4(k, A_, B_) { acc[0][k] = MFMA((A_).x, (B_).x, acc[0][k]); acc[0][k] = MFMA((A_).y, (B_).y, acc[0][k]); \
                              acc[0][k] = MFMA((A_).z, (B_).z, acc[0][k]); acc[0][k] = MFMA((A_).w, (B_).w, acc[0][k]); }
#define WG_STAGE_NEXT                                                                   \
            if (gq >= 2) {                                                              \
                _Pragma("unroll") for (int i = 0; i < NLD; ++i)                         \
                    if ((i & 1) == (gq & 1)) { WG_STAGE_A(cur ^ 1, i) WG_STAGE_B(cur ^ 1, i) if (SBIAS) WG_BIAS_M(i, cm_l) } \
            }
            if constexpr (XS ? ROLE < 5 : ROLE == 0) {
#pragma unroll
                for (int gq = 0; gq < 4; ++gq) {
                    const float4 a_ = WG_FRAG(As, wave);
                    if (!SBIAS) dbacc[0] += (a_.x + a_.y) + (a_.z + a_.w);
#pragma unroll
                    for (int jn = 0; jn < 6; ++jn) {
                        const float4 b_ = WG_FRAG(Bs, jn);
                        WG_MFMA4(jn, a_, b_)
                    }
                    if (XS && gq == ROLE) {
                        const float4 a6 = WG_FRAG(As, 6), b6 = WG_FRAG(Bs, 6);
                        WG_MFMA4(6, a6, b6)
                    }
                    WG_STAGE_NEXT
                }
            } else {
#pragma unroll
                for (int gq = 0; gq < 4; ++gq) {
                    const float4 b6 = WG_FRAG(Bs, 6);
#pragma unroll
                    for (int i = 0; i < (XS ? 6 : 7); ++i) {
                        const float4 a_ = WG_FRAG(As, i);
                        WG_MFMA4(i, a_, b6)
                    }
                    WG_STAGE_NEXT
                }
            }
#undef WG_FRAG
#undef WG_MFMA4
#undef WG_STAGE_NEXT
        }
        STAMP(1)
        {
            const int64_t cn = c + 2 < c1 ? c + 2 : c1 - 1, cn1 = c + 1 < c1 ? c + 1 : c1 - 1;
            WG_ISSUE(cn)
        }
        STAMP(2)
        lds_barrier();
        STAMP(3)
    }
    };
    if constexpr (XS) {
        if (wave == 0) chunk_loop(RoleC<0>{});
        else if (wave == 1) chunk_loop(RoleC<1>{});
        else if (wave == 2) chunk_loop(RoleC<2>{});
        else if (wave == 3) chunk_loop(RoleC<3>{});
        else if (HET7 && wave == 7) chunk_loop(RoleC<5>{});
        else chunk_loop(RoleC<4>{});
        if (wave >= 1 && wave <= 3) {
#pragma unroll
            for (int r = 0; r < 16; ++r) smem[(wave - 1) * 1024 + r * 64 + lane] = acc[0][XSLOT][r];
        }
        lds_barrier();
        if (wave == 0) {
#pragma unroll
            for (int w = 0; w < 3; ++w)
#pragma unroll
                for (int r = 0; r < 16; ++r) acc[0][XSLOT][r] += smem[w * 1024 + r * 64 + lane];
        }
    } else {
        if (LIST ? (LREM > 0 && wave >= 8 - LREM) : wave == 7) chunk_loop(RoleC<1>{});
        else chunk_loop(RoleC<0>{});
    }
    } else {
    for (int64_t c = c0; c < c1; ++c) {
        const int cur = (int)(c - c0) & 1;
        const float *As = smem + cur * 2 * PANEL, *Bs = As + PANEL;
        const float cm_r = want_bias && c + 1 < c1 ? 1.0f : 0.0f;
        STAMP(0)
#define WG_READ_FRAGS(gq_, AF, BF)                                                                                     \
        {                                                                                                              \
            _Pragma("unroll") for (int i = 0; i < TM; ++i) {                                                           \
                const int mt = wmk * TM + i;                                                                           \
                AF[i] = make_float4(0.f, 0.f, 0.f, 0.f);                                                               \
                if (MEX || mt < QT) AF[i] = *reinterpret_cast<const float4 *>(As + (32 * mt + ln) * LDSW + 8 * (gq_) + 4 * hi); \
            }                                                                                                          \
            _Pragma("unroll") for (int jn = 0; jn < TN; ++jn) {                                                        \
                const int nt = wnk * TN + jn;                                                                          \
                BF[jn] = make_float4(0.f, 0.f, 0.f, 0.f);                                                              \
                if (NEX || nt < QT) BF[jn] = *reinterpret_cast<const float4 *>(Bs + (32 * nt + ln) * LDSW + 8 * (gq_) + 4 * hi); \
            }                                                                                                          \
        }
#define WG_MFMAS(AF, BF)                                                                                               \
        {                                                                                                              \
            _Pragma("unroll") for (int i = 0; i < TM; ++i) {                                                           \
                _Pragma("unroll") for (int jn = 0; jn < TN; ++jn) {                                                    \
                    if ((MEX || wmk * TM + i < QT) && (NEX || wnk * TN + jn < QT)) {                                   \
                        acc[i][jn] = MFMA(AF[i].x, BF[jn].x, acc[i][jn]);                                              \
                        acc[i][jn] = MFMA(AF[i].y, BF[jn].y, acc[i][jn]);                                              \
                        acc[i][jn] = MFMA(AF[i].z, BF[jn].z, acc[i][jn]);                                              \
                        acc[i][jn] = MFMA(AF[i].w, BF[jn].w, acc[i][jn]);                                              \
                    }                                                                                                  \
                }                                                                                                      \
            }                                                                                                          \
        }
#define WG_STAGE_NEXT(gq_)                                                                                             \
        if ((gq_) >= 2) {                                                                                              \
            _Pragma("unroll") for (int i = 0; i < NLD; ++i)                                                            \
                if ((i & 1) == ((gq_) & 1)) {                                                                          \
                    WG_STAGE_A(cur ^ 1, i) WG_STAGE_B(cur ^ 1, i)                                                      \
                    if (SBIAS) WG_BIAS_M(i, cm_r)                                                                      \
                }                                                                                                      \
        }
        if constexpr (BRIEF_WGRAD_FRAG_PIPE && WK == 1 && QT == 8) {
            float4 af0[TM], bf0[TN], af1[TM], bf1[TN];
            WG_READ_FRAGS(0, af0, bf0)
            WG_READ_FRAGS(1, af1, bf1)
            __builtin_amdgcn_sched_barrier(0);
            WG_MFMAS(af0, bf0)
            WG_READ_FRAGS(2, af0, bf0)
            __builtin_amdgcn_sched_barrier(0);
            WG_MFMAS(af1, bf1)
            WG_READ_FRAGS(3, af1, bf1)
            __builtin_amdgcn_sched_barrier(0);
            WG_MFMAS(af0, bf0)
            WG_STAGE_NEXT(2)
            WG_MFMAS(af1, bf1)
            WG_STAGE_NEXT(3)
        } else if constexpr (BRIEF_WGRAD_FRAG_PIPE2 && WK == 2 && QT >= 4) {
            float4 af0[TM], bf0[TN], af1[TM], bf1[TN];
            WG_READ_FRAGS(wk, af0, bf0)
            WG_READ_FRAGS(wk + 2, af1, bf1)
            __builtin_amdgcn_sched_barrier(0);
#pragma unroll
            for (int i = 0; i < TM; ++i)
                if (wnk == 0) {
                    dbacc[i] += (af0[i].x + af0[i].y) + (af0[i].z + af0[i].w);
                    dbacc[i] += (af1[i].x + af1[i].y) + (af1[i].z + af1[i].w);
                }
            WG_MFMAS(af0, bf0)
            WG_STAGE_NEXT(2)
            WG_MFMAS(af1, bf1)
            WG_STAGE_NEXT(3)
        } else {
#pragma unroll
        for (int gq = 0; gq < 4; ++gq) {
            if (kactive && (WK == 1 || (gq % WK) == wk)) {
                float4 af[TM], bf[TN];
                WG_READ_FRAGS(gq, af, bf)
                if (!SBIAS) {
#pragma unroll
                    for (int i = 0; i < TM; ++i)
                        if (wnk == 0) dbacc[i] += (af[i].x + af[i].y) + (af[i].z + af[i].w);
                }
                WG_MFMAS(af, bf)
            }
            WG_STAGE_NEXT(gq)
        }
        }
#undef WG_READ_FRAGS
#undef WG_MFMAS
#undef WG_STAGE_NEXT
        STAMP(1)
        {
            const int64_t cn = c + 2 < c1 ? c + 2 : c1 - 1, cn1 = c + 1 < c1 ? c + 1 : c1 - 1;
            WG_ISSUE(cn)
        }
        STAMP(2)
        lds_barrier();
        STAMP(3)
    }
    }
#ifdef BRIEF_STAMPS
    if (lane == 0 && a.stamps) for (int i = 0; i < 4; ++i) a.stamps[((int64_t)blockIdx.x * 8 + wave) * 8 + i] = st_acc[i];
#endif
#undef WG_ISSUE
#undef WG_STAGE_A
#undef WG_STAGE_B
#undef WG_BIAS
#undef WG_BIAS_M
    if (WK > 1) {
        float *red = smem;
        float *redb = smem + (WK - 1) * NWv * TN * 1024;
#pragma unroll
        for (int i = 0; i < TM; ++i) {
            if (i > 0) lds_barrier();
            if (kactive && wk > 0) {
#pragma unroll
                for (int jn = 0; jn < TN; ++jn)
#pragma unroll
                    for (int r = 0; r < 16; ++r)
                        red[(((wk - 1) * NWv + wrem) * TN + jn) * 1024 + r * 64 + lane] = acc[i][jn][r];
                redb[((wk - 1) * NWv + wrem) * 64 + lane] = dbacc[i];
            }
            lds_barrier();
            if (wk == 0) {
                for (int w = 1; w < WK; ++w) {
#pragma unroll
                    for (int jn = 0; jn < TN; ++jn)
#pragma unroll
                        for (int r = 0; r < 16; ++r)
                            acc[i][jn][r] += red[(((w - 1) * NWv + wrem) * TN + jn) * 1024 + r * 64 + lane];
                    dbacc[i] += redb[((w - 1) * NWv + wrem) * 64 + lane];
                }
            }
        }
    }
    float *slab = a.slabs + ((int64_t)(l - 1) * a.nsplit + a.split_lo + split) * ((int64_t)FP * FP + FP);
    if (want_bias) {
#pragma unroll
        for (int i = 0; i < NLD; ++i) {
            const int e = tid + 512 * i;
            if (FULL || e < QP * 8) {
                float v = bsum[i];
                v += __shfl_xor(v, 1); v += __shfl_xor(v, 2); v += __shfl_xor(v, 4);
                if ((tid & 7) == 0 && (e >> 3) < rows_m) slab[(int64_t)FP * FP + qm * QP + (e >> 3)] = v;
            }
        }
    }
    if (wk != 0) return;
    if (LIST) {
        const int cnt = XS ? LCNT + (wave == 0 ? 1 : 0) : LCNT + (LREM > 0 && wave >= 8 - LREM ? 1 : 0);
#pragma unroll
        for (int k = 0; k < TN; ++k) {
            if (k >= cnt) break;
            const int mt = XS && k == LCNT ? QT - 1 : lmt[k], nt = XS && k == LCNT ? QT - 1 : lnt[k];
            if ((!RTW || qm * QT + mt < nt_w) && (!RTW || qn * QT + nt < nt_w)) {
#pragma unroll
                for (int r = 0; r < 16; ++r)
                    slab[(int64_t)(qm * QP + 32 * mt + ROWMAP(r, hi)) * FP + qn * QP + 32 * nt + ln] = acc[0][k][r];
            }
            if (!SBIAS && qn == 0 && nt == 0 && !(XS && k == LCNT)) {
                const float tot = dbl[k] + __shfl_xor(dbl[k], 32);
                if (hi == 0 && (!RTW || qm * QT + mt < nt_w)) slab[(int64_t)FP * FP + qm * QP + 32 * mt + ln] = tot;
            }
        }
        return;
    }
    if (HET7) {
#pragma unroll
        for (int k = 0; k < 7; ++k) {
            int mt = wave < 7 ? wave : k, nt = wave < 7 ? k : 6;
            if (XS) {
                if (k == 6) { if (wave != 0) continue; mt = 6; nt = 6; }
            } else if (wave < 7 && k == 6) continue;
            if ((!RTW || qm * QT + mt < nt_w) && (!RTW || qn * QT + nt < nt_w)) {
#pragma unroll
                for (int r = 0; r < 16; ++r)
                    slab[(int64_t)(qm * QP + 32 * mt + ROWMAP(r, hi)) * FP + qn * QP + 32 * nt + ln] = acc[0][k][r];
            }
        }
        if (!SBIAS && qn == 0 && wave < 7) {
            const float tot = dbacc[0] + __shfl_xor(dbacc[0], 32);
            if (hi == 0 && (!RTW || qm * QT + wave < nt_w)) slab[(int64_t)FP * FP + qm * QP + 32 * wave + ln] = tot;
        }
        return;
    }
#pragma unroll
    for (int i = 0; i < TM; ++i) {
        const int mt = wmk * TM + i;
        if (mt < QT && (!RTW || qm * QT + mt < nt_w)) {
#pragma unroll
            for (int jn = 0; jn < TN; ++jn) {
                const int nt = wnk * TN + jn;
                if (nt < QT && (!RTW || qn * QT + nt < nt_w)) {
#pragma unroll
                    for (int r = 0; r < 16; ++r)
                        slab[(int64_t)(qm * QP + 32 * mt + ROWMAP(r, hi)) * FP + qn * QP + 32 * nt + ln] = acc[i][jn][r];
                }
            }
            if (!SBIAS && wnk == 0 && qn == 0) {
                const float tot = dbacc[i] + __shfl_xor(dbacc[i], 32);
                if (hi == 0) slab[(int64_t)FP * FP + qm * QP + 32 * mt + ln] = tot;
            }
        }
    }
}
```

### brief_pytorch_amd/csrc/brief_wide.inc

```
constexpr int WIDE_SLAB = 32;
__host__ __device__ inline int wide_mtw(int nt)
{
    int best = 8;
    float best_cost = 1e30f;
    for (int m = 8; m >= 3; --m) {
        const int P = (nt + 4 * m - 1) / (4 * m);
        const float cost = (float)(4 * m * P) * (1.0f + 0.015f * (float)P);
        if (cost < best_cost - 1e-3f) { best_cost = cost; best = m; }
    }
    return best;
}
struct WideLds { int r, g_off, part_off, total; };
__host__ __device__ inline WideLds wide_lds(int MTW)
{
    WideLds l;
    const int slab = WIDE_SLAB * 1024, t = 4 * 32 * MTW * 33;
    l.r = (slab > t ? slab : t) + 256;
    l.g_off = l.r;
    l.part_off = l.g_off + 4 * 256;
    l.total = l.part_off + 4 * 32 * 4;
    return l;
}

__device__ __forceinline__ void wide_mem_barrier()
{
    asm volatile("s_waitcnt vmcnt(0) lgkmcnt(0)" ::: "memory");
    __builtin_amdgcn_s_barrier();
    asm volatile("" ::: "memory");
}

#ifndef BRIEF_WIDE_GLDS
#define BRIEF_WIDE_GLDS 0
#endif
__device__ __forceinline__ void wide_stage(float4 *X, const float4 *plane, int k0, int kt_n, int wave, int lane)
{
    const int nkq = kt_n * 4;
    const float4 *src = plane + (int64_t)k0 * 256 + lane;
#if BRIEF_WIDE_GLDS
    for (int e = wave; e < nkq; e += 4)
        __builtin_amdgcn_global_load_lds((const __attribute__((address_space(1))) void *)(src + e * 64),
                                         (__attribute__((address_space(3))) void *)(X + e * 64), 16, 0, 0);
    asm volatile("s_waitcnt vmcnt(0)" ::: "memory");
#else
    for (int e0 = wave; e0 < nkq; e0 += 32) {
        float4 v[8];
#pragma unroll
        for (int u = 0; u < 8; ++u) v[u] = e0 + 4 * u < nkq ? src[(e0 + 4 * u) * 64] : make_float4(0.f, 0.f, 0.f, 0.f);
#pragma unroll
        for (int u = 0; u < 8; ++u)
            if (e0 + 4 * u < nkq) X[(e0 + 4 * u) * 64 + lane] = v[u];
    }
#endif
}

__device__ __forceinline__ void wide_store_image(float4 *plane, int mt, int lane, const f32x16 &v)
{
#pragma unroll
    for (int q = 0; q < 4; ++q) plane[(mt * 4 + q) * 64 + lane] = make_float4(v[4 * q], v[4 * q + 1], v[4 * q + 2], v[4 * q + 3]);
    asm volatile("s_nop 2" ::: "memory");
}

template <int MTW, bool TRAIN, bool BOX = false>
__global__ __launch_bounds__(256, 1) void k_wide(const typename KArgsT<BOX>::type a)
{
    static_assert(!(TRAIN && BOX), "the box mapping is an inference instantiation");
    constexpr int TROWS = 32 * MTW;
    constexpr int RS = (TROWS + 63) / 64;
    const brief_siren_desc &d = a.d;
    const int nt = brief_nt(d), FP = 32 * nt;
    const int P = (nt + 4 * MTW - 1) / (4 * MTW);
    const int TR = brief_rec_tr(nt);
    extern __shared__ __attribute__((aligned(16))) float smem[];
    const WideLds lds = wide_lds(MTW);
    float4 *X = reinterpret_cast<float4 *>(smem);
    float *T = smem;
    float *G = smem + lds.g_off;
    float4 *PART = reinterpret_cast<float4 *>(smem + lds.part_off);
    const int lane = threadIdx.x & 63;
    const int wave = __builtin_amdgcn_readfirstlane(threadIdx.x >> 6);
    const int hi = lane >> 5, ln = lane & 31;
    const int L = d.layers, cin = d.cin, cout = d.cout;
    const int kit = (d.features + 7) >> 3;
    const int64_t npad = a.npad;
    const float *pk = a.pk;
    float *Gw = G + wave * 256;
    float *Tw = T + wave * (TROWS * 33);
    const float4 *W0p = reinterpret_cast<const float4 *>(pk + brief_pk_w0(d));
    const float *headp = pk + brief_pk_head(d);
    const int64_t hstride = brief_pk_hidden_stride(d);
    const int plane_bytes = FP * 128;
    const int voff = ln * 4 + hi * 512;
    float *rec = a.rec + (((int64_t)blockIdx.x + a.rec_base) * 4 + wave) * (8 * TR + 32);
    if (TRAIN) {
        for (int e = lane; e < 8 * TR + 32; e += 64) rec[e] = 0.f;
    }
    float accbh[4] = {0.f, 0.f, 0.f, 0.f};
    float lsum = 0.f;
    const int64_t Hn = ((a.n_end > 0 ? a.n_end : a.n) + 31) >> 5;
    for (int64_t tile = (a.n_begin >> 5) + blockIdx.x; tile < Hn; tile += gridDim.x) {
        typedef const __attribute__((address_space(4))) FusedArgs *kargs_f;
        kargs_f ap = (kargs_f)__builtin_amdgcn_kernarg_segment_ptr();
        asm volatile("" : "+s"(ap));
        const int64_t *k_idx = ap->idx;
        const float *k_tg = ap->targets, *k_wt = ap->weights, *k_co = ap->coords;
        const uint64_t k_pop = ap->rng_pop, k_seed = ap->rng_seed, k_step = ap->rng_step;
        const int64_t k_off = ap->offset;
        const int64_t n = tile * 32 + ln;
        const bool valid = n < a.n;
        int64_t j = 0;
        if (valid) j = k_idx ? k_idx[n] : (k_pop ? philox_index(n, k_pop, k_seed, k_step) : n + k_off);
        float x0 = 0.f, x1 = 0.f, x2 = 0.f;
        if (valid) {
            if (k_co) {
                x0 = k_co[j * cin];
                x1 = k_co[j * cin + 1];
                if (cin == 3) x2 = k_co[j * cin + 2];
            } else {
                GridArgs kg;
                kg.ndim = ap->grid.ndim; kg.lo = ap->grid.lo; kg.hi = ap->grid.hi; kg.fast = ap->grid.fast;
#pragma unroll
                for (int ax = 0; ax < 3; ++ax) { kg.dims[ax] = ap->grid.dims[ax]; kg.step[ax] = ap->grid.step[ax]; kg.magic[ax] = ap->grid.magic[ax]; }
                sample_coords<BOX>(kg, cin, j, x0, x1, x2);
            }
        }
        auto zplane = [&](int l) -> float * { return a.Z + ((int64_t)l * FP * npad + tile * (int64_t)FP * 32); };
        auto dplane = [&](int l) -> float * { return a.D + ((int64_t)(l - 1) * FP * npad + tile * (int64_t)FP * 32); };
        auto iplane = [&](int l) -> float4 * {
            return reinterpret_cast<float4 *>((TRAIN ? a.slabs : a.Z) + ((int64_t)blockIdx.x * 2 + (l & 1)) * (int64_t)FP * 32);
        };
        f32x16 acc[1][MTW];
        f32x16 px;
        bool tv[MTW];
        float pph[4] = {0.f, 0.f, 0.f, 0.f};
        for (int l = 0; l <= L - 2; ++l) {
            const bool last = (l == L - 2);
            const __amdgpu_buffer_rsrc_t rz = __builtin_amdgcn_make_buffer_rsrc((void *)(TRAIN ? zplane(l) : a.Z), 0, plane_bytes, 0x00020000);
            const float *wl = pk + FP * 4 + (int64_t)(l > 0 ? l - 1 : 0) * hstride;
            const __amdgpu_buffer_rsrc_t rsW = __builtin_amdgcn_make_buffer_rsrc((void *)wl, 0, (int)((int64_t)FP * FP * 8), 0x00020000);
            if (l > 0) wide_mem_barrier();
            for (int p = 0; p < P; ++p) {
                const int wv = wave + 4 * p * MTW;
#pragma unroll
                for (int t = 0; t < MTW; ++t) tv[t] = wv + 4 * t < nt;
                if (l == 0) {
                    const float b0 = hi ? x1 : x0;
                    const float b1 = hi ? 1.0f : x2;
#pragma unroll
                    for (int t = 0; t < MTW; ++t) {
#pragma unroll
                        for (int r = 0; r < 16; ++r) acc[0][t][r] = 0.f;
                        if (tv[t]) {
                            const float4 w = W0p[32 * (wv + 4 * t) + ln];
                            acc[0][t] = MFMA(hi ? w.y : w.x, b0, acc[0][t]);
                            acc[0][t] = MFMA(hi ? w.w : w.z, b1, acc[0][t]);
                        }
                    }
                } else {
                    const float *bp_ = wl + 2 * (int64_t)FP * FP;
#pragma unroll
                    for (int t = 0; t < MTW; ++t) {
#pragma unroll
                        for (int q = 0; q < 4; ++q) {
                            float4 b4 = make_float4(0.f, 0.f, 0.f, 0.f);
                            if (tv[t]) b4 = *reinterpret_cast<const float4 *>(bp_ + 32 * (wv + 4 * t) + 8 * q + 4 * hi);
                            acc[0][t][4 * q] = b4.x; acc[0][t][4 * q + 1] = b4.y; acc[0][t][4 * q + 2] = b4.z; acc[0][t][4 * q + 3] = b4.w;
                        }
                    }
                    for (int k0 = 0; k0 < nt; k0 += WIDE_SLAB) {
                        const int kt_n = nt - k0 < WIDE_SLAB ? nt - k0 : WIDE_SLAB;
                        const int ksteps = kit - 4 * k0 < 4 * kt_n ? kit - 4 * k0 : 4 * kt_n;
                        if (p > 0 || k0 > 0) lds_barrier();
                        wide_stage(X, iplane(l - 1), k0, kt_n, wave, lane);
                        lds_barrier();
                        __builtin_amdgcn_s_setprio(3);
                        lean_chain_rt<1, MTW, 0, true>(acc, px, rsW, k0 * 4096, X, wv, lane, nt, ksteps, false);
                        __builtin_amdgcn_s_setprio(0);
                    }
                }
#pragma unroll
                for (int t = 0; t < MTW; ++t) {
                    if (!tv[t]) continue;
                    const int mt = wv + 4 * t;
                    f32x16 hv;
#pragma unroll
                    for (int r = 0; r < 16; ++r) acc[0][t][r] = __builtin_amdgcn_fractf(acc[0][t][r]);
                    if (TRAIN) {
#pragma unroll
                        for (int r = 0; r < 16; ++r) bstore1(acc[0][t][r], rz, voff, (32 * mt + (r & 3) + 8 * (r >> 2)) * 128);
                    }
#pragma unroll
                    for (int r = 0; r < 16; ++r) hv[r] = BRIEF_SIN_REV(acc[0][t][r]);
                    if (!last) wide_store_image(iplane(l), mt, lane, hv);
                    if (last) {
#pragma unroll
                        for (int c = 0; c < 4; ++c) {
                            if (c < cout) {
#pragma unroll
                                for (int q = 0; q < 4; ++q) {
                                    const float4 wv4 = *reinterpret_cast<const float4 *>(headp + (int64_t)c * FP + 32 * mt + 8 * q + 4 * hi);
                                    pph[c] = __fmaf_rn(wv4.x, hv[4 * q], pph[c]); pph[c] = __fmaf_rn(wv4.y, hv[4 * q + 1], pph[c]);
                                    pph[c] = __fmaf_rn(wv4.z, hv[4 * q + 2], pph[c]); pph[c] = __fmaf_rn(wv4.w, hv[4 * q + 3], pph[c]);
                                }
                            }
                        }
                    }
                }
            }
        }
#pragma unroll
        for (int c = 0; c < 4; ++c) pph[c] += __shfl_xor(pph[c], 32);
        if (hi == 0) PART[wave * 32 + ln] = make_float4(pph[0], pph[1], pph[2], pph[3]);
        lds_barrier();
        float zo[4], yh[4], g[4];
        {
            float4 tot = PART[ln];
#pragma unroll
            for (int w = 1; w < 4; ++w) {
                const float4 v = PART[w * 32 + ln];
                tot.x += v.x; tot.y += v.y; tot.z += v.z; tot.w += v.w;
            }
            const float tt[4] = {tot.x, tot.y, tot.z, tot.w};
#pragma unroll
            for (int c = 0; c < 4; ++c) {
                zo[c] = 0.f; yh[c] = 0.f; g[c] = 0.f;
                if (c < cout) {
                    zo[c] = tt[c] + headp[4 * (int64_t)FP + c];
                    yh[c] = d.output_act ? brief_fast_sinf(d.w0_hidden * zo[c]) : zo[c];
                }
                if (!TRAIN) {
                    if (c < cout && valid && wave == 0 && hi == 0) {
                        if (a.out_kind == BRIEF_OUT_F32) {
                            reinterpret_cast<float *>(a.out)[n * cout + c] = yh[c];
                        } else {
                            float t_ = __fsub_rn(yh[c], a.scale_min);
                            t_ = __fdiv_rn(t_, a.den);
                            t_ = fminf(fmaxf(t_, 0.f), 1.f);
                            const float u_ = __fadd_rn(__fmul_rn(t_, a.span), a.vmin);
                            if (a.out_kind == BRIEF_OUT_U16) reinterpret_cast<uint16_t *>(a.out)[n * cout + c] = (uint16_t)(int)u_;
                            else reinterpret_cast<uint8_t *>(a.out)[n * cout + c] = (uint8_t)(int)u_;
                        }
                    }
                    continue;
                }
                if (c < cout && valid) {
                    const float yvc = k_tg[j * cout + c];
                    float we = k_wt ? k_wt[j * cout + c] : 1.0f;
                    if (a.thr != 0.f && yh[c] <= a.thr) we = 1.0f;
                    const float df = yh[c] - yvc;
                    float li, gi;
                    if (a.loss_kind == BRIEF_LOSS_L2) { li = df * df; gi = 2.0f * df; }
                    else if (a.loss_kind == BRIEF_LOSS_SMOOTHL1) {
                        const float ad = fabsf(df);
                        if (ad < a.beta) { li = 0.5f * df * df / a.beta; gi = df / a.beta; }
                        else { li = ad - 0.5f * a.beta; gi = df < 0.f ? -1.0f : 1.0f; }
                    } else { li = 0.f; gi = 0.f; }
                    if (wave == 0 && hi == 0) lsum += li * we;
                    g[c] = a.loss_kind == BRIEF_LOSS_EXTERNAL ? yvc : gi * we * a.inv_count;
                    if (d.output_act) g[c] *= d.w0_hidden * brief_fast_cosf(d.w0_hidden * zo[c]);
                    if (a.yhat_out && wave == 0 && hi == 0) a.yhat_out[n * cout + c] = yh[c];
                }
            }
        }
        if (!TRAIN) {
            lds_barrier();
            continue;
        }
        if (hi == 0) *reinterpret_cast<float4 *>(Gw + ln * 4) = make_float4(g[0], g[1], g[2], g[3]);
        else *reinterpret_cast<float4 *>(Gw + 128 + ln * 4) = make_float4(x0, x1, x2, 1.0f);
        float gom[4];
        {
            const float om_top = (L - 2) == 0 ? d.w0_first : d.w0_hidden;
#pragma unroll
            for (int c = 0; c < 4; ++c) gom[c] = om_top * g[c];
        }
        auto skinny0 = [&](int p) {
#pragma unroll
            for (int t = 0; t < MTW; ++t)
#pragma unroll
                for (int r = 0; r < 16; ++r) Tw[(32 * t + ROWMAP(r, hi)) * 33 + ln] = tv[t] ? acc[0][t][r] : 0.f;
            asm volatile("s_waitcnt lgkmcnt(0)" ::: "memory");
#pragma unroll
            for (int rs = 0; rs < RS; ++rs) {
                float4 s0 = make_float4(0.f, 0.f, 0.f, 0.f);
                const int row = lane + 64 * rs;
                const float *trow = Tw + (row < TROWS ? row : 0) * 33;
#pragma unroll 4
                for (int s = 0; s < 32; ++s) {
                    const float dv = trow[s];
                    const float4 xv = *reinterpret_cast<const float4 *>(Gw + 128 + s * 4);
                    s0.x = __fmaf_rn(dv, xv.x, s0.x); s0.y = __fmaf_rn(dv, xv.y, s0.y);
                    s0.z = __fmaf_rn(dv, xv.z, s0.z); s0.w = __fmaf_rn(dv, xv.w, s0.w);
                }
                if (row < TROWS && wave + 4 * (p * MTW + (row >> 5)) < nt) {
                    float *r0 = rec + ((int64_t)p * TROWS + row) * 4;
                    r0[0] += s0.x; r0[1] += s0.y; r0[2] += s0.z; r0[3] += s0.w;
                }
            }
            asm volatile("s_waitcnt lgkmcnt(0)" ::: "memory");
        };
        lds_barrier();
        {
            const __amdgpu_buffer_rsrc_t rzl = __builtin_amdgcn_make_buffer_rsrc((void *)zplane(L - 2), 0, plane_bytes, 0x00020000);
            const __amdgpu_buffer_rsrc_t rd = __builtin_amdgcn_make_buffer_rsrc((void *)(L - 2 >= 1 ? dplane(L - 2) : zplane(0)), 0, plane_bytes, 0x00020000);
            for (int p = 0; p < P; ++p) {
                const int wv = wave + 4 * p * MTW;
#pragma unroll
                for (int t = 0; t < MTW; ++t) tv[t] = wv + 4 * t < nt;
#pragma unroll
                for (int t = 0; t < MTW; ++t) {
#pragma unroll
                    for (int r = 0; r < 16; ++r) {
                        acc[0][t][r] = 0.f;
                        if (tv[t]) acc[0][t][r] = bload1(rzl, voff, (32 * (wv + 4 * t) + (r & 3) + 8 * (r >> 2)) * 128);
                    }
                }
#pragma unroll
                for (int t = 0; t < MTW; ++t)
#pragma unroll
                    for (int r = 0; r < 16; ++r) {
                        Tw[(32 * t + ROWMAP(r, hi)) * 33 + ln] = tv[t] ? BRIEF_SIN_REV(acc[0][t][r]) : 0.f;
                        acc[0][t][r] = BRIEF_COS_REV(acc[0][t][r]);
                    }
                asm volatile("s_waitcnt lgkmcnt(0)" ::: "memory");
#pragma unroll
                for (int rs = 0; rs < RS; ++rs) {
                    float4 sW = make_float4(0.f, 0.f, 0.f, 0.f), sb = make_float4(0.f, 0.f, 0.f, 0.f);
                    const int row = lane + 64 * rs;
                    const float *trow = Tw + (row < TROWS ? row : 0) * 33;
#pragma unroll 4
                    for (int s = 0; s < 32; ++s) {
                        const float hvs = trow[s];
                        const float4 gv = *reinterpret_cast<const float4 *>(Gw + s * 4);
                        sW.x = __fmaf_rn(hvs, gv.x, sW.x); sW.y = __fmaf_rn(hvs, gv.y, sW.y);
                        sW.z = __fmaf_rn(hvs, gv.z, sW.z); sW.w = __fmaf_rn(hvs, gv.w, sW.w);
                        sb.x += gv.x; sb.y += gv.y; sb.z += gv.z; sb.w += gv.w;
                    }
                    if (row < TROWS && wave + 4 * (p * MTW + (row >> 5)) < nt) {
                        float *rh = rec + 4 * TR + p * TROWS + row;
                        rh[0] += sW.x; rh[TR] += sW.y; rh[2 * TR] += sW.z; rh[3 * TR] += sW.w;
                    }
                    if (rs == 0 && p == 0) { accbh[0] += sb.x; accbh[1] += sb.y; accbh[2] += sb.z; accbh[3] += sb.w; }
                }
                asm volatile("s_waitcnt lgkmcnt(0)" ::: "memory");
#pragma unroll
                for (int t = 0; t < MTW; ++t) {
                    if (!tv[t]) continue;
                    const int mt = wv + 4 * t;
#pragma unroll
                    for (int q = 0; q < 4; ++q) {
                        float4 sacc = make_float4(0.f, 0.f, 0.f, 0.f);
#pragma unroll
                        for (int c = 0; c < 4; ++c) {
                            if (c < cout) {
                                const float4 wv4 = *reinterpret_cast<const float4 *>(headp + (int64_t)c * FP + 32 * mt + 8 * q + 4 * hi);
                                sacc.x = __fmaf_rn(wv4.x, gom[c], sacc.x); sacc.y = __fmaf_rn(wv4.y, gom[c], sacc.y);
                                sacc.z = __fmaf_rn(wv4.z, gom[c], sacc.z); sacc.w = __fmaf_rn(wv4.w, gom[c], sacc.w);
                            }
                        }
                        acc[0][t][4 * q] *= sacc.x; acc[0][t][4 * q + 1] *= sacc.y;
                        acc[0][t][4 * q + 2] *= sacc.z; acc[0][t][4 * q + 3] *= sacc.w;
                    }
                    if (L - 2 >= 1) {
#pragma unroll
                        for (int r = 0; r < 16; ++r) bstore1(acc[0][t][r], rd, voff, (32 * mt + (r & 3) + 8 * (r >> 2)) * 128);
                        wide_store_image(iplane(L - 2), mt, lane, acc[0][t]);
                    }
                }
                if (L - 2 == 0) skinny0(p);
            }
        }
        for (int l = L - 2; l >= 1; --l) {
            const __amdgpu_buffer_rsrc_t rzp = __builtin_amdgcn_make_buffer_rsrc((void *)zplane(l - 1), 0, plane_bytes, 0x00020000);
            const __amdgpu_buffer_rsrc_t rdout = __builtin_amdgcn_make_buffer_rsrc((void *)(l - 1 >= 1 ? dplane(l - 1) : zplane(0)), 0, plane_bytes, 0x00020000);
            const float *wl = pk + FP * 4 + (int64_t)(l - 1) * hstride;
            const __amdgpu_buffer_rsrc_t rsW = __builtin_amdgcn_make_buffer_rsrc((void *)wl, 0, (int)((int64_t)FP * FP * 8), 0x00020000);
            wide_mem_barrier();
            for (int p = 0; p < P; ++p) {
                const int wv = wave + 4 * p * MTW;
#pragma unroll
                for (int t = 0; t < MTW; ++t) {
                    tv[t] = wv + 4 * t < nt;
#pragma unroll
                    for (int r = 0; r < 16; ++r) acc[0][t][r] = 0.f;
                }
                for (int k0 = 0; k0 < nt; k0 += WIDE_SLAB) {
                    const int kt_n = nt - k0 < WIDE_SLAB ? nt - k0 : WIDE_SLAB;
                    const int ksteps = kit - 4 * k0 < 4 * kt_n ? kit - 4 * k0 : 4 * kt_n;
                    if (p > 0 || k0 > 0) lds_barrier();
                    wide_stage(X, iplane(l), k0, kt_n, wave, lane);
                    lds_barrier();
                    __builtin_amdgcn_s_setprio(3);
                    lean_chain_rt<1, MTW, 0, true>(acc, px, rsW, FP * FP * 4 + k0 * 4096, X, wv, lane, nt, ksteps, false);
                    __builtin_amdgcn_s_setprio(0);
                }
#pragma unroll
                for (int t2 = 0; t2 < MTW; t2 += 2) {
                    float zr[2][16];
#pragma unroll
                    for (int u = 0; u < 2; ++u) {
                        const int t = t2 + u < MTW ? t2 + u : MTW - 1;
#pragma unroll
                        for (int r = 0; r < 16; ++r) {
                            zr[u][r] = 0.f;
                            if (t2 + u < MTW && tv[t]) zr[u][r] = bload1s(rzp, voff, (32 * (wv + 4 * t) + (r & 3) + 8 * (r >> 2)) * 128);
                        }
                    }
#pragma unroll
                    for (int u = 0; u < 2; ++u) {
                        const int t = t2 + u < MTW ? t2 + u : MTW - 1;
                        if (t2 + u < MTW && tv[t]) {
#pragma unroll
                            for (int r = 0; r < 16; ++r) acc[0][t][r] *= BRIEF_COS_REV(zr[u][r]);
                        }
                    }
                }
                if (l - 1 >= 1) {
#pragma unroll
                    for (int t = 0; t < MTW; ++t) {
                        if (!tv[t]) continue;
#pragma unroll
                        for (int r = 0; r < 16; ++r) bstore1(acc[0][t][r], rdout, voff, (32 * (wv + 4 * t) + (r & 3) + 8 * (r >> 2)) * 128);
                        wide_store_image(iplane(l - 1), wv + 4 * t, lane, acc[0][t]);
                    }
                } else {
                    lds_barrier();
                    skinny0(p);
                }
            }
        }
        lds_barrier();
    }
    if (!TRAIN) return;
    for (int off = 32; off >= 1; off >>= 1) lsum += __shfl_xor(lsum, off);
    if (lane == 0) {
#pragma unroll
        for (int c = 0; c < 4; ++c) rec[8 * TR + c] = accbh[c];
        rec[8 * TR + 4] = lsum;
    }
}
```

### brief_pytorch_amd/csrc/brief_x3.inc

```
typedef __bf16 x3_bf16x8 __attribute__((ext_vector_type(8)));
typedef _Float16 x3_f16x8 __attribute__((ext_vector_type(8)));
union X3Frag { uint4 u; x3_bf16x8 v; x3_f16x8 f; };
#define MFMA_X3(a, b, c) __builtin_amdgcn_mfma_f32_32x32x16_bf16((a), (b), (c), 0, 0, 0)
#define MFMA_X3F(a, b, c) __builtin_amdgcn_mfma_f32_32x32x16_f16((a), (b), (c), 0, 0, 0)
#define BRIEF_X3_FWD_SCALE 64.0f
#define BRIEF_X3_FWD_UNSCALE 0.015625f
__device__ __forceinline__ void x3_split_f16(float x, uint16_t &hi, uint16_t &lo)
{
    union { _Float16 h; uint16_t u; } a, b;
    a.h = (_Float16)x;
    b.h = (_Float16)(x - (float)a.h);
    hi = a.u; lo = b.u;
}
__device__ __forceinline__ void x3_split_bf16(float x, uint16_t &hi, uint16_t &lo)
{
    union { __bf16 h; uint16_t u; } a, b;
    a.h = (__bf16)x;
    b.h = (__bf16)(x - (float)a.h);
    hi = a.u; lo = b.u;
}

template <bool F16>
__device__ __forceinline__ void x3_pack(const f32x16 &x, int s, uint4 &hi, uint4 &lo)
{
    X3Frag h, l;
#pragma unroll
    for (int j = 0; j < 8; ++j) {
        if (F16) {
            const _Float16 b = (_Float16)x[8 * s + j];
            h.f[j] = b;
            l.f[j] = (_Float16)(x[8 * s + j] - (float)b);
        } else {
            const __bf16 b = (__bf16)x[8 * s + j];
            h.v[j] = b;
            l.v[j] = (__bf16)(x[8 * s + j] - (float)b);
        }
    }
    hi = h.u; lo = l.u;
}

template <int NT, bool F16>
__device__ __forceinline__ void x3_write_image(uint4 *X16, const f32x16 (&h)[KCfg<NT>::MTW], int wm, int lane)
{
    using K = KCfg<NT>;
#pragma unroll
    for (int t = 0; t < K::MTW; ++t) {
        const int mt = wm + K::WM * t;
        if (K::EXACT || mt < NT) {
#pragma unroll
            for (int sx = 0; sx < 2; ++sx) {
                uint4 hi, lo;
                x3_pack<F16>(h[t], sx, hi, lo);
                X16[(mt * 2 + sx) * 64 + lane] = hi;
                X16[NT * 2 * 64 + (mt * 2 + sx) * 64 + lane] = lo;
            }
        }
    }
}

template <bool F16>
__device__ __forceinline__ void x3_write_tile(uint4 *X16, const f32x16 &h, int mt, int lane)
{
#pragma unroll
    for (int sx = 0; sx < 2; ++sx) {
        uint4 hi, lo;
        x3_pack<F16>(h, sx, hi, lo);
        X16[(mt * 2 + sx) * 64 + lane] = hi;
        X16[8 * 2 * 64 + (mt * 2 + sx) * 64 + lane] = lo;
    }
}

#ifndef BRIEF_X3_PD
#define BRIEF_X3_PD 2
#endif
template <int NT>
struct X3Pre { uint4 hi[BRIEF_X3_PD][KCfg<NT>::MTW], lo[BRIEF_X3_PD][KCfg<NT>::MTW]; };

#define X3_LOAD_INTO(dh_, dl_, it_)                                                                          \
    _Pragma("unroll") for (int t = 0; t < K::MTW; ++t) {                                                     \
        if (K::EXACT || wm + K::WM * t < NT) {                                                               \
            const u32x4 vh = __builtin_amdgcn_raw_buffer_load_b128(rs, voff, soff_w + (K::WM * t * NT * 2 + (it_)) * 1024, 0); \
            const u32x4 vl = __builtin_amdgcn_raw_buffer_load_b128(rs, voff, soff_w + soff_lo + (K::WM * t * NT * 2 + (it_)) * 1024, 0); \
            dh_[t] = make_uint4(vh.x, vh.y, vh.z, vh.w);                                                     \
            dl_[t] = make_uint4(vl.x, vl.y, vl.z, vl.w);                                                     \
        }                                                                                                    \
    }

template <int NT>
__device__ __forceinline__ void x3_preload(X3Pre<NT> &pre, __amdgpu_buffer_rsrc_t rs, int soff_layer, int lo_bytes, int wm, int lane)
{
    using K = KCfg<NT>;
    const int voff = lane * 16;
    int soff_w = soff_layer + wm * (NT * 2 * 1024);
    asm volatile("" : "+s"(soff_w));
    int soff_lo = lo_bytes;
    asm volatile("" : "+s"(soff_lo));
#pragma unroll
    for (int it = 0; it < BRIEF_X3_PD; ++it) X3_LOAD_INTO(pre.hi[it], pre.lo[it], it)
}

#undef X3_LOAD_INTO

struct X3TLds {
    static constexpr int IMG_FLOATS = 2 * 4 * 64 * 33;
    static constexpr int G_OFF = IMG_FLOATS;
    static constexpr int HW_OFF = G_OFF + 4 * 256;
    static constexpr int PART_OFF = HW_OFF + 4 * 256 + 4;
    static constexpr int TOTAL = PART_OFF + 2 * 4 * 32 * 4;
};

template <bool F16, bool BPRE>
__device__ __forceinline__ void x3_chain2(f32x16 (&acc)[2][2], const X3Pre<8> &pre, __amdgpu_buffer_rsrc_t rs, int soff_layer, int lo_bytes,
                                          const uint4 *X16, int wm, int lane, int kit, bool two)
{
    constexpr int NT = 8, NIT = 16, PD = BRIEF_X3_PD, HALF = 2 * NT * 2 * 64;
    using K = KCfg<8>;
    const int voff = lane * 16;
    int soff_w = soff_layer + wm * (NT * 2 * 1024);
    asm volatile("" : "+s"(soff_w));
    int soff_lo = lo_bytes;
    asm volatile("" : "+s"(soff_lo));
    uint4 ahi[NIT][2], alo[NIT][2];
    uint4 bhi[NIT][2], blo[NIT][2];
#pragma unroll
    for (int it = 0; it < PD; ++it)
#pragma unroll
        for (int t = 0; t < 2; ++t) { ahi[it][t] = pre.hi[it][t]; alo[it][t] = pre.lo[it][t]; }
#pragma unroll
    for (int h = 0; h < 2; ++h) { bhi[0][h] = X16[h * HALF + lane]; blo[0][h] = X16[h * HALF + NT * 2 * 64 + lane]; }
#pragma unroll
    for (int it = 0; it < NIT; ++it) {
        if (it + PD < NIT) {
#pragma unroll
            for (int t = 0; t < 2; ++t) {
                const u32x4 vh = __builtin_amdgcn_raw_buffer_load_b128(rs, voff, soff_w + (K::WM * t * NT * 2 + it + PD) * 1024, 0);
                const u32x4 vl = __builtin_amdgcn_raw_buffer_load_b128(rs, voff, soff_w + soff_lo + (K::WM * t * NT * 2 + it + PD) * 1024, 0);
                ahi[it + PD][t] = make_uint4(vh.x, vh.y, vh.z, vh.w);
                alo[it + PD][t] = make_uint4(vl.x, vl.y, vl.z, vl.w);
            }
        }
        if (BPRE ? it + 1 < NIT : it > 0) {
            constexpr int ahead = BPRE ? 1 : 0;
#pragma unroll
            for (int h = 0; h < 2; ++h) {
                bhi[it + ahead][h] = X16[h * HALF + (it + ahead) * 64 + lane];
                blo[it + ahead][h] = X16[h * HALF + NT * 2 * 64 + (it + ahead) * 64 + lane];
            }
        }
        __builtin_amdgcn_sched_barrier(0);
        if (it < kit) {
#pragma unroll
            for (int t = 0; t < 2; ++t) {
                X3Frag fah, fal;
                fah.u = ahi[it][t]; fal.u = alo[it][t];
#pragma unroll
                for (int h = 0; h < 2; ++h) {
                    if (h == 1 && !two) continue;
                    X3Frag fbh, fbl;
                    fbh.u = bhi[it][h]; fbl.u = blo[it][h];
                    if (F16) {
                        acc[h][t] = MFMA_X3F(fah.f, fbh.f, acc[h][t]);
                        acc[h][t] = MFMA_X3F(fah.f, fbl.f, acc[h][t]);
                        acc[h][t] = MFMA_X3F(fal.f, fbh.f, acc[h][t]);
                    } else {
                        acc[h][t] = MFMA_X3(fah.v, fbh.v, acc[h][t]);
                        acc[h][t] = MFMA_X3(fah.v, fbl.v, acc[h][t]);
                        acc[h][t] = MFMA_X3(fal.v, fbh.v, acc[h][t]);
                    }
                }
            }
        }
    }
}

template <bool TRAIN, bool BOX = false>
__global__ __launch_bounds__(256, 2) void k_fused_x3(const typename KArgsT<BOX>::type a)
{
    static_assert(!(TRAIN && BOX), "the box mapping is an inference instantiation");
#ifdef BRIEF_STAMPS
    float st_acc[10] = {0.f, 0.f, 0.f, 0.f, 0.f, 0.f, 0.f, 0.f, 0.f, 0.f};
    long long st_last = clock64();
    const long long st_c0 = st_last, st_r0 = wall_clock64();
#endif
    constexpr int NT = 8, FP = 256, HALF = 2 * NT * 2 * 64;
    using K = KCfg<8>;
    extern __shared__ __attribute__((aligned(16))) float smem[];
    uint4 *X16 = reinterpret_cast<uint4 *>(smem);
    float *T = smem;
    float *G = smem + X3TLds::G_OFF;
    float *HW = smem + X3TLds::HW_OFF;
    float4 *PART = reinterpret_cast<float4 *>(smem + X3TLds::PART_OFF);
    const int lane = threadIdx.x & 63;
    const int wave = __builtin_amdgcn_readfirstlane(threadIdx.x >> 6);
    const int hi = lane >> 5, ln = lane & 31;
    const int wm = wave;
    const brief_siren_desc &d = a.d;
    const int L = d.layers, cin = d.cin, cout = d.cout;
    const int kit16 = (d.features + 15) >> 4;
    const int64_t npad = a.npad;
    const float *pk = a.pk;
    float *Tw = T + wave * 2 * (K::TROWS * 33);
    float *Gw = G + wave * 256;
    const float4 *W0p = reinterpret_cast<const float4 *>(pk + brief_pk_w0(d));
    const __amdgpu_buffer_rsrc_t rs_x3 =
        __builtin_amdgcn_make_buffer_rsrc((void *)(a.pk + brief_pk16_off(a.d, 1)), 0, (int)(2 * brief_pk16_region(a.d) * 4), 0x00020000);
    const int x3_lo_bytes = (int)(brief_pk16_region(a.d) * 4);
    const int stash_bytes = (a.diag & 1) ? 0 : (int)((int64_t)FP * npad * 4);
    {
        const float *headp = pk + brief_pk_head(d);
        for (int e = threadIdx.x; e < 4 * FP + 4; e += 256) HW[e] = headp[e];
    }
    lds_barrier();
    float acc0[4] = {0.f, 0.f, 0.f, 0.f}, accWh[4] = {0.f, 0.f, 0.f, 0.f}, accbh[4] = {0.f, 0.f, 0.f, 0.f};
    float lsum = 0.f;
    const int64_t Hn = (a.n + 31) >> 5;
    const int64_t G_ = gridDim.x, w_ = blockIdx.x;
    const int64_t R_ = Hn / (2 * G_), Hr = Hn - 2 * G_ * R_;
    const int64_t npair_x = Hr > G_ ? Hr - G_ : 0;
    const int64_t nsing_x = Hr > G_ ? G_ - npair_x : Hr;
    const int extra = w_ < npair_x ? 2 : (w_ < npair_x + nsing_x ? 1 : 0);
    const int64_t ht_x = 2 * G_ * R_ + (w_ < npair_x ? 2 * w_ : 2 * npair_x + (w_ - npair_x));
    for (int64_t it_ = 0; it_ < R_ + (extra ? 1 : 0); ++it_) {
        const int64_t ht = it_ < R_ ? 2 * (it_ * G_ + w_) : ht_x;
        const bool two = it_ < R_ || extra == 2;
        typedef const __attribute__((address_space(4))) FusedArgs *kargs_f;
        kargs_f ap = (kargs_f)__builtin_amdgcn_kernarg_segment_ptr();
        asm volatile("" : "+s"(ap));
        const int64_t *k_idx = ap->idx;
        const float *k_tg = ap->targets, *k_wt = ap->weights, *k_co = ap->coords;
        const uint64_t k_pop = ap->rng_pop, k_seed = ap->rng_seed, k_step = ap->rng_step;
        const int64_t k_off = ap->offset;
        GridArgs kg;
        kg.ndim = ap->grid.ndim; kg.lo = ap->grid.lo; kg.hi = ap->grid.hi; kg.fast = ap->grid.fast;
#pragma unroll
        for (int ax = 0; ax < 3; ++ax) { kg.dims[ax] = ap->grid.dims[ax]; kg.step[ax] = ap->grid.step[ax]; kg.magic[ax] = ap->grid.magic[ax]; }
        float x0[2], x1[2], x2[2];
        int64_t jidx[2];
        bool valid[2];
        f32x16 acc[2][2];
        {
            const int64_t n64 = ht * 32 + lane;
            const bool v64 = (lane < 32 || two) && n64 < a.n;
            int64_t j = 0;
            if (v64) j = k_idx ? k_idx[n64] : (k_pop ? philox_index(n64, k_pop, k_seed, k_step) : n64 + k_off);
            float c0 = 0.f, c1 = 0.f, c2 = 0.f;
            if (v64) {
                if (k_co) {
                    c0 = k_co[j * cin];
                    c1 = k_co[j * cin + 1];
                    if (cin == 3) c2 = k_co[j * cin + 2];
                } else {
                    sample_coords<BOX>(kg, cin, j, c0, c1, c2);
                }
            }
            const int jl = (int)(uint32_t)(uint64_t)j, jh = (int)(uint32_t)((uint64_t)j >> 32);
#pragma unroll
            for (int h = 0; h < 2; ++h) {
                const int src = 32 * h + ln;
                x0[h] = __shfl(c0, src); x1[h] = __shfl(c1, src); x2[h] = __shfl(c2, src);
                jidx[h] = (int64_t)(((uint64_t)(uint32_t)__shfl(jh, src) << 32) | (uint32_t)__shfl(jl, src));
                valid[h] = (h == 0 || two) && (ht + h) * 32 + ln < a.n;
            }
        }
        X3Pre<8> x3pre;
        float4 bnext[2][4];
#pragma unroll
        for (int t = 0; t < 2; ++t)
#pragma unroll
            for (int q = 0; q < 4; ++q) bnext[t][q] = make_float4(0.f, 0.f, 0.f, 0.f);
#define X3T_LOAD_BIAS(layer)                                                                            \
    {                                                                                                   \
        const float *bp_ = pk + brief_pk_hidden(d, (layer)) + 2 * FP * FP;                              \
        _Pragma("unroll") for (int t = 0; t < 2; ++t) {                                                 \
            const int mt = wm + 4 * t;                                                                  \
            _Pragma("unroll") for (int q = 0; q < 4; ++q)                                               \
                bnext[t][q] = *reinterpret_cast<const float4 *>(bp_ + 32 * mt + 8 * q + 4 * hi);        \
        }                                                                                               \
    }
#pragma unroll
        for (int h = 0; h < 2; ++h) {
            const float b0 = hi ? x1[h] : x0[h];
            const float b1 = hi ? 1.0f : x2[h];
#pragma unroll
            for (int t = 0; t < 2; ++t) {
                const int mt = wm + 4 * t;
#pragma unroll
                for (int r = 0; r < 16; ++r) acc[h][t][r] = 0.f;
                const float4 w = W0p[32 * mt + ln];
                acc[h][t] = MFMA(hi ? w.y : w.x, b0, acc[h][t]);
                acc[h][t] = MFMA(hi ? w.w : w.z, b1, acc[h][t]);
            }
        }
        STAMP(0)
        for (int l = 0; l <= L - 2; ++l) {
            const bool last = (l == L - 2);
            if (l > 0) {
#pragma unroll
                for (int h = 0; h < 2; ++h)
#pragma unroll
                    for (int t = 0; t < 2; ++t)
#pragma unroll
                        for (int q = 0; q < 4; ++q) {
                            acc[h][t][4 * q] = BRIEF_X3_FWD_SCALE * bnext[t][q].x; acc[h][t][4 * q + 1] = BRIEF_X3_FWD_SCALE * bnext[t][q].y;
                            acc[h][t][4 * q + 2] = BRIEF_X3_FWD_SCALE * bnext[t][q].z; acc[h][t][4 * q + 3] = BRIEF_X3_FWD_SCALE * bnext[t][q].w;
                        }
                __builtin_amdgcn_s_setprio(3);
                x3_chain2<true, !TRAIN>(acc, x3pre, rs_x3, (l - 1) * FP * FP * 4, x3_lo_bytes, X16, wm, lane, kit16, two);
                __builtin_amdgcn_s_setprio(0);
                STAMP(1)
                lds_barrier();
                STAMP(2)
            }
            if (!last) {
                x3_preload<8>(x3pre, rs_x3, l * FP * FP * 4, x3_lo_bytes, wm, lane);
                X3T_LOAD_BIAS(l + 1)
            }
            float pph[2][4];
#pragma unroll
            for (int h = 0; h < 2; ++h) {
#pragma unroll
                for (int c = 0; c < 4; ++c) pph[h][c] = 0.f;
                if (h == 1 && !two) continue;
                const int voff = (int)(((ht + h) * 32) * (FP * 4)) + ln * 4 + hi * 4 * 128;
#pragma unroll
                for (int t = 0; t < 2; ++t) {
                    const int mt = wm + 4 * t;
#pragma unroll
                    for (int r = 0; r < 16; ++r) acc[h][t][r] = __builtin_amdgcn_fractf(l > 0 ? acc[h][t][r] * BRIEF_X3_FWD_UNSCALE : acc[h][t][r]);
                    f32x16 hv;
                    if (!last) {
                        if (TRAIN) {
                        const __amdgpu_buffer_rsrc_t rz =
                            __builtin_amdgcn_make_buffer_rsrc((void *)(a.Z + (int64_t)l * FP * npad), 0, stash_bytes, 0x00020000);
#pragma unroll
                        for (int r = 0; r < 16; ++r) bstore1s(acc[h][t][r], rz, voff, (32 * mt + (r & 3) + 8 * (r >> 2)) * 128);
                        }
#pragma unroll
                        for (int r = 0; r < 16; ++r) hv[r] = BRIEF_SIN_REV(acc[h][t][r]);
                        x3_write_tile<true>(X16 + h * HALF, hv, mt, lane);
                    } else {
#pragma unroll
                        for (int r = 0; r < 16; ++r) { hv[r] = BRIEF_SIN_REV(acc[h][t][r]); if (TRAIN) acc[h][t][r] = BRIEF_COS_REV(acc[h][t][r]); }
#pragma unroll
                        for (int c = 0; c < 4; ++c) {
                            if (c < cout) {
#pragma unroll
                                for (int q = 0; q < 4; ++q) {
                                    const float4 wv = *reinterpret_cast<const float4 *>(HW + c * FP + 32 * mt + 8 * q + 4 * hi);
                                    pph[h][c] = __fmaf_rn(wv.x, hv[4 * q], pph[h][c]); pph[h][c] = __fmaf_rn(wv.y, hv[4 * q + 1], pph[h][c]);
                                    pph[h][c] = __fmaf_rn(wv.z, hv[4 * q + 2], pph[h][c]); pph[h][c] = __fmaf_rn(wv.w, hv[4 * q + 3], pph[h][c]);
                                }
                            }
                        }
                        if (TRAIN) {
                            float *Th = T + (wave * 2 + h) * (K::TROWS * 33);
#pragma unroll
                            for (int r = 0; r < 16; ++r) Th[(32 * t + ROWMAP(r, hi)) * 33 + ln] = hv[r];
                        }
                    }
                }
                if (last) {
#pragma unroll
                    for (int c = 0; c < 4; ++c) pph[h][c] += __shfl_xor(pph[h][c], 32);
                    if (hi == 0) PART[(h * 4 + wave) * 32 + ln] = make_float4(pph[h][0], pph[h][1], pph[h][2], pph[h][3]);
                }
            }
            STAMP(3)
            lds_barrier();
            STAMP(4)
        }
        float zo[2][4], yh[2][4], g[2][4];
#pragma unroll
        for (int h = 0; h < 2; ++h) {
            float4 tot = PART[(h * 4) * 32 + ln];
#pragma unroll
            for (int w = 1; w < 4; ++w) {
                const float4 v = PART[(h * 4 + w) * 32 + ln];
                tot.x += v.x; tot.y += v.y; tot.z += v.z; tot.w += v.w;
            }
            const float tt[4] = {tot.x, tot.y, tot.z, tot.w};
            const int64_t n = (ht + h) * 32 + ln;
#pragma unroll
            for (int c = 0; c < 4; ++c) {
                zo[h][c] = 0.f; yh[h][c] = 0.f; g[h][c] = 0.f;
                if (c < cout) {
                    zo[h][c] = tt[c] + HW[4 * FP + c];
                    yh[h][c] = d.output_act ? brief_fast_sinf(d.w0_hidden * zo[h][c]) : zo[h][c];
                }
                if (!TRAIN) {
                    if (c < cout && valid[h] && wm == 0 && hi == 0) {
                        if (a.out_kind == BRIEF_OUT_F32) {
                            reinterpret_cast<float *>(a.out)[n * cout + c] = yh[h][c];
                        } else {
                            float t_ = __fsub_rn(yh[h][c], a.scale_min);
                            t_ = __fdiv_rn(t_, a.den);
                            t_ = fminf(fmaxf(t_, 0.f), 1.f);
                            const float u_ = __fadd_rn(__fmul_rn(t_, a.span), a.vmin);
                            if (a.out_kind == BRIEF_OUT_U16) reinterpret_cast<uint16_t *>(a.out)[n * cout + c] = (uint16_t)(int)u_;
                            else reinterpret_cast<uint8_t *>(a.out)[n * cout + c] = (uint8_t)(int)u_;
                        }
                    }
                    continue;
                }
                if (c < cout && valid[h]) {
                    const float yvc = k_tg[jidx[h] * cout + c];
                    float we = k_wt ? k_wt[jidx[h] * cout + c] : 1.0f;
                    if (a.thr != 0.f && yh[h][c] <= a.thr) we = 1.0f;
                    const float df = yh[h][c] - yvc;
                    float li, gi;
                    if (a.loss_kind == BRIEF_LOSS_L2) { li = df * df; gi = 2.0f * df; }
                    else if (a.loss_kind == BRIEF_LOSS_SMOOTHL1) {
                        const float ad = fabsf(df);
                        if (ad < a.beta) { li = 0.5f * df * df / a.beta; gi = df / a.beta; }
                        else { li = ad - 0.5f * a.beta; gi = df < 0.f ? -1.0f : 1.0f; }
                    } else { li = 0.f; gi = 0.f; }
                    if (wm == 0 && hi == 0) lsum += li * we;
                    g[h][c] = a.loss_kind == BRIEF_LOSS_EXTERNAL ? yvc : gi * we * a.inv_count;
                    if (d.output_act) g[h][c] *= d.w0_hidden * brief_fast_cosf(d.w0_hidden * zo[h][c]);
                    if (a.yhat_out && wm == 0 && hi == 0) a.yhat_out[n * cout + c] = yh[h][c];
                }
            }
        }
        STAMP(5)
        if (!TRAIN) continue;
#pragma unroll
        for (int h = 0; h < 2; ++h) {
            if (h == 1 && !two) continue;
            if (hi == 0) *reinterpret_cast<float4 *>(Gw + ln * 4) = make_float4(g[h][0], g[h][1], g[h][2], g[h][3]);
            asm volatile("s_waitcnt lgkmcnt(0)" ::: "memory");
            {
                float4 sW = make_float4(0.f, 0.f, 0.f, 0.f), sb = make_float4(0.f, 0.f, 0.f, 0.f);
                const float *trow = T + (wave * 2 + h) * (K::TROWS * 33) + lane * 33;
                if (cout == 1) {
#pragma unroll 8
                    for (int s = 0; s < 32; ++s) {
                        const float gv = Gw[s * 4];
                        sW.x = __fmaf_rn(trow[s], gv, sW.x);
                        sb.x += gv;
                    }
                } else {
#pragma unroll 4
                    for (int s = 0; s < 32; ++s) {
                        const float hv = trow[s];
                        const float4 gv = *reinterpret_cast<const float4 *>(Gw + s * 4);
                        sW.x = __fmaf_rn(hv, gv.x, sW.x); sW.y = __fmaf_rn(hv, gv.y, sW.y);
                        sW.z = __fmaf_rn(hv, gv.z, sW.z); sW.w = __fmaf_rn(hv, gv.w, sW.w);
                        sb.x += gv.x; sb.y += gv.y; sb.z += gv.z; sb.w += gv.w;
                    }
                }
                accWh[0] += sW.x; accWh[1] += sW.y; accWh[2] += sW.z; accWh[3] += sW.w;
                accbh[0] += sb.x; accbh[1] += sb.y; accbh[2] += sb.z; accbh[3] += sb.w;
            }
        }
        {
            const float om_top = (L - 2) == 0 ? d.w0_first : d.w0_hidden;
#pragma unroll
            for (int h = 0; h < 2; ++h) {
                if (h == 1 && !two) continue;
                float gom[4];
#pragma unroll
                for (int c = 0; c < 4; ++c) gom[c] = om_top * g[h][c];
#pragma unroll
                for (int t = 0; t < 2; ++t) {
                    const int mt = wm + 4 * t;
#pragma unroll
                    for (int q = 0; q < 4; ++q) {
                        float4 sacc = make_float4(0.f, 0.f, 0.f, 0.f);
#pragma unroll
                        for (int c = 0; c < 4; ++c) {
                            if (c < cout) {
                                const float4 wv = *reinterpret_cast<const float4 *>(HW + c * FP + 32 * mt + 8 * q + 4 * hi);
                                sacc.x = __fmaf_rn(wv.x, gom[c], sacc.x); sacc.y = __fmaf_rn(wv.y, gom[c], sacc.y);
                                sacc.z = __fmaf_rn(wv.z, gom[c], sacc.z); sacc.w = __fmaf_rn(wv.w, gom[c], sacc.w);
                            }
                        }
                        acc[h][t][4 * q] *= sacc.x; acc[h][t][4 * q + 1] *= sacc.y;
                        acc[h][t][4 * q + 2] *= sacc.z; acc[h][t][4 * q + 3] *= sacc.w;
                    }
                }
            }
        }
        STAMP(6)
        for (int l = L - 2; l >= 1; --l) {
            const __amdgpu_buffer_rsrc_t rd =
                __builtin_amdgcn_make_buffer_rsrc((void *)(a.D + (int64_t)(l - 1) * FP * npad), 0, stash_bytes, 0x00020000);
            const __amdgpu_buffer_rsrc_t rzp =
                __builtin_amdgcn_make_buffer_rsrc((void *)(a.Z + (int64_t)(l - 1) * FP * npad), 0, stash_bytes, 0x00020000);
            x3_preload<8>(x3pre, rs_x3, (l - 1) * FP * FP * 4 + FP * FP * 2, x3_lo_bytes, wm, lane);
#pragma unroll
            for (int h = 0; h < 2; ++h) {
                if (h == 1 && !two) continue;
                const int voff_s = (int)(((ht + h) * 32) * (FP * 4)) + ln * 4 + hi * 4 * 128;
#pragma unroll
                for (int t = 0; t < 2; ++t) {
                    const int mt = wm + 4 * t;
#pragma unroll
                    for (int r = 0; r < 16; ++r) bstore1s(acc[h][t][r], rd, voff_s, (32 * mt + (r & 3) + 8 * (r >> 2)) * 128);
                }
            }
            STAMP(7)
            lds_barrier();
#pragma unroll
            for (int h = 0; h < 2; ++h)
                if (h == 0 || two) x3_write_image<8, false>(X16 + h * HALF, acc[h], wm, lane);
            lds_barrier();
#pragma unroll
            for (int h = 0; h < 2; ++h)
#pragma unroll
                for (int t = 0; t < 2; ++t)
#pragma unroll
                    for (int r = 0; r < 16; ++r) acc[h][t][r] = 0.f;
            STAMP(8)
            __builtin_amdgcn_s_setprio(3);
            x3_chain2<false, false>(acc, x3pre, rs_x3, (l - 1) * FP * FP * 4 + FP * FP * 2, x3_lo_bytes, X16, wm, lane, kit16, two);
            __builtin_amdgcn_s_setprio(0);
            STAMP(9)
#pragma unroll
            for (int h = 0; h < 2; ++h) {
                if (h == 1 && !two) continue;
                float zr[2][16];
                const int voff_s = (int)(((ht + h) * 32) * (FP * 4)) + ln * 4 + hi * 4 * 128;
#pragma unroll
                for (int t = 0; t < 2; ++t) {
                    const int mt = wm + 4 * t;
#pragma unroll
                    for (int r = 0; r < 16; ++r) zr[t][r] = bload1s(rzp, voff_s, (32 * mt + (r & 3) + 8 * (r >> 2)) * 128);
                }
#pragma unroll
                for (int t = 0; t < 2; ++t)
#pragma unroll
                    for (int r = 0; r < 16; ++r) acc[h][t][r] *= BRIEF_COS_REV(zr[t][r]);
            }
        }
        STAMP(7)
#pragma unroll
        for (int h = 0; h < 2; ++h) {
            if (h == 1 && !two) continue;
            if (h == 0) lds_barrier();
            float *Tf = Tw + h * (K::TROWS * 33);
#pragma unroll
            for (int t = 0; t < 2; ++t)
#pragma unroll
                for (int r = 0; r < 16; ++r) Tf[(32 * t + ROWMAP(r, hi)) * 33 + ln] = acc[h][t][r];
            if (hi == 1) *reinterpret_cast<float4 *>(Gw + 128 + ln * 4) = make_float4(x0[h], x1[h], x2[h], 1.0f);
            asm volatile("s_waitcnt lgkmcnt(0)" ::: "memory");
            float4 s0 = make_float4(0.f, 0.f, 0.f, 0.f);
            const float *trow = Tf + lane * 33;
#pragma unroll 4
            for (int s = 0; s < 32; ++s) {
                const float dv = trow[s];
                const float4 xv = *reinterpret_cast<const float4 *>(Gw + 128 + s * 4);
                s0.x = __fmaf_rn(dv, xv.x, s0.x); s0.y = __fmaf_rn(dv, xv.y, s0.y);
                s0.z = __fmaf_rn(dv, xv.z, s0.z); s0.w = __fmaf_rn(dv, xv.w, s0.w);
            }
            acc0[0] += s0.x; acc0[1] += s0.y; acc0[2] += s0.z; acc0[3] += s0.w;
        }
        lds_barrier();
        STAMP(6)
    }
#undef X3T_LOAD_BIAS
    if (!TRAIN) return;
    float *rec = a.rec + ((int64_t)blockIdx.x * 4 + wave) * BRIEF_REC_FLOATS;
#pragma unroll
    for (int c = 0; c < 4; ++c) {
        rec[lane * 4 + c] = acc0[c];
        rec[BRIEF_REC_DWH + c * 128 + lane] = accWh[c];
    }
    for (int off = 32; off >= 1; off >>= 1) lsum += __shfl_xor(lsum, off);
    if (lane == 0) {
#pragma unroll
        for (int c = 0; c < 4; ++c) rec[BRIEF_REC_DBH + c] = accbh[c];
        rec[BRIEF_REC_LOSS] = lsum;
#ifdef BRIEF_STAMPS
        for (int i = 0; i < 10; ++i) rec[BRIEF_REC_STAMPS + i] = st_acc[i];
        rec[BRIEF_REC_STAMPS + 10] = (float)(clock64() - st_c0);
        rec[BRIEF_REC_STAMPS + 11] = (float)(wall_clock64() - st_r0);
#endif
    }
}
#ifndef BRIEF_X3W_DLY
#define BRIEF_X3W_DLY 0
#endif
__global__ __launch_bounds__(512, 2) void k_wgrad_x3(const WgradArgs a)
{
    constexpr int FP = 256, QT = 8, WNk = 4, TM = 4, TN = 2, LDSW = 36, NLD = 4, PANEL = FP * LDSW;
    extern __shared__ __attribute__((aligned(16))) float smem[];
    const int tid = threadIdx.x;
    const int lane = tid & 63;
    const int wave = __builtin_amdgcn_readfirstlane(tid >> 6);
    const int hi = lane >> 5, ln = lane & 31;
    const int wmk = wave / WNk, wnk = wave % WNk;
    const int l = 1 + (int)blockIdx.x / a.nsplit;
    const int split = (int)blockIdx.x % a.nsplit;
    const int64_t nchunks = a.npad / 32;
    const int64_t c0 = nchunks * split / a.nsplit, c1 = nchunks * (split + 1) / a.nsplit;
    const float *Dl = a.D + (int64_t)(l - 1) * FP * a.npad;
    const float *Zl = a.Z + (int64_t)(l - 1) * FP * a.npad;
    (void)QT;

    f32x16 acc[TM][TN];
#pragma unroll
    for (int i = 0; i < TM; ++i)
#pragma unroll
        for (int jn = 0; jn < TN; ++jn)
#pragma unroll
            for (int r = 0; r < 16; ++r) acc[i][jn][r] = 0.f;
    float bsum[NLD] = {0.f, 0.f, 0.f, 0.f};
    u32x4 ra[NLD], rb[NLD];
#ifdef BRIEF_X3W_NOLOAD
    const int panel_bytes = 0;
#else
    const int panel_bytes = (int)((int64_t)FP * a.npad * 4);
#endif
    const __amdgpu_buffer_rsrc_t rsD = __builtin_amdgcn_make_buffer_rsrc((void *)Dl, 0, panel_bytes, 0x00020000);
    const __amdgpu_buffer_rsrc_t rsZ = __builtin_amdgcn_make_buffer_rsrc((void *)Zl, 0, panel_bytes, 0x00020000);
    int voffs[NLD];
#pragma unroll
    for (int i = 0; i < NLD; ++i) {
        const int e = tid + 512 * i;
        voffs[i] = e * 16;
    }
#define X3F(u_) __uint_as_float(u_)
#ifndef BRIEF_X3W_AUX
#define BRIEF_X3W_AUX 2
#endif
#define X3W_LD(rs_, base_, voff_, soff_) __builtin_amdgcn_raw_buffer_load_b128(rs_, voff_, soff_, BRIEF_X3W_AUX)
#define X3W_ISSUE(cc)                                                                             \
    _Pragma("unroll") for (int i = 0; i < NLD; ++i) {                                             \
        ra[i] = X3W_LD(rsD, Dl, voffs[i], (int)((cc) * (FP * 128)));       \
        rb[i] = X3W_LD(rsZ, Zl, voffs[i], (int)((cc) * (FP * 128)));       \
    }
#define X3W_PUT(dst_, v_)                                                                         \
    {                                                                                             \
        union { uint2 u; __bf16 h[4]; } ph_, pl_;                                                 \
        const float f_[4] = {__uint_as_float((v_).x), __uint_as_float((v_).y), __uint_as_float((v_).z), __uint_as_float((v_).w)}; \
        _Pragma("unroll") for (int j_ = 0; j_ < 4; ++j_) {                                        \
            ph_.h[j_] = (__bf16)f_[j_];                                                           \
            pl_.h[j_] = (__bf16)(f_[j_] - (float)ph_.h[j_]);                                      \
        }                                                                                         \
        *reinterpret_cast<uint2 *>(dst_) = ph_.u;                                                 \
        *reinterpret_cast<uint2 *>((dst_) + 16) = pl_.u;             \
    }
#define X3W_STAGE(buf, count_)                                                                    \
    _Pragma("unroll") for (int i = 0; i < NLD; ++i) {                                             \
        const int e = tid + 512 * i;                                                              \
        float *pa_ = smem + (buf) * 2 * PANEL + (e >> 3) * LDSW + (e & 7) * 2;                    \
        X3W_PUT(pa_, ra[i])                                                                       \
        if (count_) bsum[i] += (X3F(ra[i].x) + X3F(ra[i].y)) + (X3F(ra[i].z) + X3F(ra[i].w));     \
        u32x4 h_;                                                                                 \
        h_.x = __float_as_uint(BRIEF_SIN_REV(X3F(rb[i].x))); h_.y = __float_as_uint(BRIEF_SIN_REV(X3F(rb[i].y))); \
        h_.z = __float_as_uint(BRIEF_SIN_REV(X3F(rb[i].z))); h_.w = __float_as_uint(BRIEF_SIN_REV(X3F(rb[i].w))); \
        X3W_PUT(pa_ + PANEL, h_)                                                                  \
    }
    X3W_ISSUE(c0)
    X3W_STAGE(0, true)
    {
        const int64_t cn = c0 + 1 < c1 ? c0 + 1 : c1 - 1;
        X3W_ISSUE(cn)
    }
    lds_barrier();
    for (int64_t c = c0; c < c1; ++c) {
        const int cur = (int)(c - c0) & 1;
        const float *As = smem + cur * 2 * PANEL, *Bs = As + PANEL;
        const float flag = c + 1 < c1 ? 1.0f : 0.0f;
        const int64_t cn = c + 2 < c1 ? c + 2 : c1 - 1, cn1 = c + 1 < c1 ? c + 1 : c1 - 1;
        u32x4 hs = {0u, 0u, 0u, 0u};
#pragma unroll
        for (int ks = 0; ks < 2; ++ks) {
            X3Frag ah[2], al[2], bh[TN], bl[TN];
            {
                const float *p_ = As + (32 * (wmk * TM) + ln) * LDSW + 8 * ks + 4 * hi;
                ah[0].u = *reinterpret_cast<const uint4 *>(p_);
                al[0].u = *reinterpret_cast<const uint4 *>(p_ + 16);
            }
#pragma unroll
            for (int jn = 0; jn < TN; ++jn) {
                const float *p_ = Bs + (32 * (wnk * TN + jn) + ln) * LDSW + 8 * ks + 4 * hi;
                bh[jn].u = *reinterpret_cast<const uint4 *>(p_);
                bl[jn].u = *reinterpret_cast<const uint4 *>(p_ + 16);
            }
#pragma unroll
            for (int i = 0; i < TM; ++i)
#pragma unroll
                for (int jn = 0; jn < TN; ++jn) {
                    if (jn == 0 && i + 1 < TM) {
                        const float *p_ = As + (32 * (wmk * TM + i + 1) + ln) * LDSW + 8 * ks + 4 * hi;
                        ah[(i + 1) & 1].u = *reinterpret_cast<const uint4 *>(p_);
                        al[(i + 1) & 1].u = *reinterpret_cast<const uint4 *>(p_ + 16);
                    }
#ifndef BRIEF_X3W_NOMFMA
                    acc[i][jn] = MFMA_X3(ah[i & 1].v, bh[jn].v, acc[i][jn]);
                    acc[i][jn] = MFMA_X3(ah[i & 1].v, bl[jn].v, acc[i][jn]);
                    acc[i][jn] = MFMA_X3(al[i & 1].v, bh[jn].v, acc[i][jn]);
#endif
                    __builtin_amdgcn_sched_barrier(0);
                    const int g = ks * (TM * TN) + i * TN + jn, slot = g >> 2, sub = g & 3;
                    const int e = tid + 512 * slot;
                    float *pa_ = smem + (cur ^ 1) * 2 * PANEL + (e >> 3) * LDSW + (e & 7) * 2;
#ifndef BRIEF_X3W_NOSTAGE
                    if (sub == 0) {
                        asm volatile("" : "+v"(ra[slot]));
                        X3W_PUT(pa_, ra[slot])
                        float rs_ = (X3F(ra[slot].x) + X3F(ra[slot].y)) + (X3F(ra[slot].z) + X3F(ra[slot].w));
                        asm volatile("" : "+v"(rs_));
                        bsum[slot] += flag * rs_;
                    } else if (sub == 1) {
                        asm volatile("" : "+v"(rb[slot]));
                        hs.x = __float_as_uint(BRIEF_SIN_REV(X3F(rb[slot].x))); hs.y = __float_as_uint(BRIEF_SIN_REV(X3F(rb[slot].y)));
                        hs.z = __float_as_uint(BRIEF_SIN_REV(X3F(rb[slot].z))); hs.w = __float_as_uint(BRIEF_SIN_REV(X3F(rb[slot].w)));
                    } else if (sub == 2) {
                        X3W_PUT(pa_ + PANEL, hs)
                    }
                    {
                        const int gl = (g + 16 - 3 - BRIEF_X3W_DLY) & 15;
                        if ((gl & 3) == 0) {
                            const int sl = gl >> 2;
                            const int64_t cl = (4 * sl + 3 + BRIEF_X3W_DLY < 16) ? cn : cn1;
                            ra[sl] = X3W_LD(rsD, Dl, voffs[sl], (int)(cl * (FP * 128)));
                            rb[sl] = X3W_LD(rsZ, Zl, voffs[sl], (int)(cl * (FP * 128)));
                        }
                    }
#else
                    if (sub == 3) {
                        float rs_ = X3F(ra[slot].x) + X3F(rb[slot].x);
                        asm volatile("" : "+v"(rs_));
                        bsum[slot] += flag * rs_;
                        ra[slot] = X3W_LD(rsD, Dl, voffs[slot], (int)(cn * (FP * 128)));
                        rb[slot] = X3W_LD(rsZ, Zl, voffs[slot], (int)(cn * (FP * 128)));
                    }
#endif
                    __builtin_amdgcn_sched_barrier(0);
                }
        }
        lds_barrier();
    }
#undef X3W_ISSUE
#undef X3W_LD
#undef X3F
#undef X3W_PUT
#undef X3W_STAGE
    float *slab = a.slabs + ((int64_t)(l - 1) * a.nsplit + split) * ((int64_t)FP * FP + FP);
#pragma unroll
    for (int i = 0; i < TM; ++i) {
        const int mt = wmk * TM + i;
#pragma unroll
        for (int jn = 0; jn < TN; ++jn) {
            const int nt = wnk * TN + jn;
#pragma unroll
            for (int r = 0; r < 16; ++r) slab[(int64_t)(32 * mt + ROWMAP(r, hi)) * FP + 32 * nt + ln] = acc[i][jn][r];
        }
    }
#pragma unroll
    for (int i = 0; i < NLD; ++i) {
        float v = bsum[i];
        v += __shfl_xor(v, 1); v += __shfl_xor(v, 2); v += __shfl_xor(v, 4);
        if ((tid & 7) == 0) slab[(int64_t)FP * FP + (tid >> 3) + 64 * i] = v;
    }
}
```

Before: 102.0 million voxels/s.

## Use vec4-interleaved stash layout for NT=8 fused training and wgrad staging

Adds a stash tile layout for 256-feature f32 models in which each lane's four consecutive rows sit contiguously. The fused kernel can then write Z/D activations and read Z back with 128-bit buffer ops instead of 16 scalar ones per tile. The weight-gradient kernel de-interleaves the vec4 loads into LDS with strided scalar writes. Its bias sum now reads from the staged LDS panel instead of the registers. The change trades fewer global memory instructions for extra LDS scatter stores and a layout coupling that every stash producer and consumer must respect.

After: 102.9 million voxels/s, median of 6. About the same (+0.9%).

```diff
diff --git a/brief_pytorch_amd/csrc/brief_device.inc b/brief_pytorch_amd/csrc/brief_device.inc
--- a/brief_pytorch_amd/csrc/brief_device.inc
+++ b/brief_pytorch_amd/csrc/brief_device.inc
@@ -209,6 +209,18 @@
 {
     __builtin_amdgcn_raw_buffer_store_b32(__float_as_uint(v), rs, voff, soff, BRIEF_X3_STASH_AUX);
 }
+__device__ __forceinline__ void bstore4(float v0, float v1, float v2, float v3, __amdgpu_buffer_rsrc_t rs, int voff, int soff)
+{
+    u32x4 v;
+    v.x = __float_as_uint(v0); v.y = __float_as_uint(v1); v.z = __float_as_uint(v2); v.w = __float_as_uint(v3);
+    __builtin_amdgcn_raw_buffer_store_b128(v, rs, voff, soff, 0);
+    asm volatile("s_nop 2" :: "v"(v) : "memory");
+}
+__device__ __forceinline__ float4 bload4s(__amdgpu_buffer_rsrc_t rs, int voff, int soff)
+{
+    const u32x4 v = __builtin_amdgcn_raw_buffer_load_b128(rs, voff, soff, BRIEF_STASH_LD_AUX);
+    return make_float4(__uint_as_float(v.x), __uint_as_float(v.y), __uint_as_float(v.z), __uint_as_float(v.w));
+}
 
 template <int NT, bool INFER = false>
 __device__ __forceinline__ void chain(f32x16 (&acc)[(KCfg<NT, INFER>::MTW)], __amdgpu_buffer_rsrc_t rs, int soff_layer ,
diff --git a/brief_pytorch_amd/csrc/brief_fused.inc b/brief_pytorch_amd/csrc/brief_fused.inc
--- a/brief_pytorch_amd/csrc/brief_fused.inc
+++ b/brief_pytorch_amd/csrc/brief_fused.inc
@@ -26,6 +26,7 @@
 #endif
     using K = KCfg<NT, !TRAIN>;
     using LD = FusedLds<NT, !TRAIN>;
+    constexpr bool V4 = TRAIN && brief_stash_vec4_nt(NT);
     extern __shared__ __attribute__((aligned(16))) float smem[];
     float4 *X = reinterpret_cast<float4 *>(smem);
     float *T = smem;
@@ -182,10 +183,17 @@
                     if (TRAIN && !last) {
                         const __amdgpu_buffer_rsrc_t rz =
                             __builtin_amdgcn_make_buffer_rsrc((void *)(a.Z + (int64_t)l * K::FP * npad), 0, stash_bytes, 0x00020000);
-                        const int voff = (int)(n0 * (K::FP * 4)) + ln * 4 + hi * 4 * 128;
-#pragma unroll
-                        for (int r = 0; r < 16; ++r)
-                            bstore1(acc[t][r], rz, voff, (32 * mt + (r & 3) + 8 * (r >> 2)) * 128);
+                        const int voff = (int)(n0 * (K::FP * 4)) + 4 * brief_stash_tile_off(V4, 4 * hi, ln);
+                        if constexpr (V4) {
+#pragma unroll
+                            for (int q = 0; q < 4; ++q)
+                                bstore4(acc[t][4 * q], acc[t][4 * q + 1], acc[t][4 * q + 2], acc[t][4 * q + 3], rz, voff,
+                                        4 * brief_stash_tile_off(true, 32 * mt + 8 * q, 0));
+                        } else {
+#pragma unroll
+                            for (int r = 0; r < 16; ++r)
+                                bstore1(acc[t][r], rz, voff, 4 * brief_stash_tile_off(false, 32 * mt + (r & 3) + 8 * (r >> 2), 0));
+                        }
                     }
 #pragma unroll
                     for (int r = 0; r < 16; ++r) hreg[t][r] = BRIEF_SIN_REV(acc[t][r]);
@@ -335,14 +343,21 @@
         for (int l = L - 2; l >= 1; --l) {
             const __amdgpu_buffer_rsrc_t rd =
                 __builtin_amdgcn_make_buffer_rsrc((void *)(a.D + (int64_t)(l - 1) * K::FP * npad), 0, stash_bytes, 0x00020000);
-            const int voff_s = (int)(n0 * (K::FP * 4)) + ln * 4 + hi * 4 * 128;
+            const int voff_s = (int)(n0 * (K::FP * 4)) + 4 * brief_stash_tile_off(V4, 4 * hi, ln);
 #pragma unroll
             for (int t = 0; t < K::MTW; ++t) {
                 const int mt = wm + K::WM * t;
                 if (K::EXACT || mt < NT) {
-#pragma unroll
-                    for (int r = 0; r < 16; ++r)
-                        bstore1(dl[t][r], rd, voff_s, (32 * mt + (r & 3) + 8 * (r >> 2)) * 128);
+                    if constexpr (V4) {
+#pragma unroll
+                        for (int q = 0; q < 4; ++q)
+                            bstore4(dl[t][4 * q], dl[t][4 * q + 1], dl[t][4 * q + 2], dl[t][4 * q + 3], rd, voff_s,
+                                    4 * brief_stash_tile_off(true, 32 * mt + 8 * q, 0));
+                    } else {
+#pragma unroll
+                        for (int r = 0; r < 16; ++r)
+                            bstore1(dl[t][r], rd, voff_s, 4 * brief_stash_tile_off(false, 32 * mt + (r & 3) + 8 * (r >> 2), 0));
+                    }
                 }
             }
             const __amdgpu_buffer_rsrc_t rzp =
@@ -352,9 +367,18 @@
 #define FUSED_LOAD_Z()                                                                                  \
     _Pragma("unroll") for (int t = 0; t < K::MTW; ++t) {                                                \
         const int mt = wm + K::WM * t;                                                                  \
-        _Pragma("unroll") for (int r = 0; r < 16; ++r) {                                                \
-            zr[t][r] = 0.f;                                                                             \
-            if (K::EXACT || mt < NT) zr[t][r] = bload1s(rzp, voff_s, (32 * mt + (r & 3) + 8 * (r >> 2)) * 128); \
+        if constexpr (V4) {                                                                             \
+            _Pragma("unroll") for (int q = 0; q < 4; ++q) {                                             \
+                float4 z4 = make_float4(0.f, 0.f, 0.f, 0.f);                                            \
+                if (K::EXACT || mt < NT) z4 = bload4s(rzp, voff_s, 4 * brief_stash_tile_off(true, 32 * mt + 8 * q, 0)); \
+                zr[t][4 * q] = z4.x; zr[t][4 * q + 1] = z4.y; zr[t][4 * q + 2] = z4.z; zr[t][4 * q + 3] = z4.w; \
+            }                                                                                           \
+        } else {                                                                                        \
+            _Pragma("unroll") for (int r = 0; r < 16; ++r) {                                            \
+                zr[t][r] = 0.f;                                                                         \
+                if (K::EXACT || mt < NT)                                                                \
+                    zr[t][r] = bload1s(rzp, voff_s, 4 * brief_stash_tile_off(false, 32 * mt + (r & 3) + 8 * (r >> 2), 0)); \
+            }                                                                                           \
         }                                                                                               \
     }
             if (ZPRE) FUSED_LOAD_Z()
diff --git a/brief_pytorch_amd/csrc/brief_layout.h b/brief_pytorch_amd/csrc/brief_layout.h
--- a/brief_pytorch_amd/csrc/brief_layout.h
+++ b/brief_pytorch_amd/csrc/brief_layout.h
@@ -108,3 +108,22 @@
     return (n + g - 1) / g * g;
 }
 BL_HD int64_t brief_npad_d(const brief_siren_desc &d, int64_t n) { return brief_npad(brief_nt(d), n); }
+
+#ifndef BRIEF_STASH_VEC4
+#define BRIEF_STASH_VEC4 1
+#endif
+#if defined(BRIEF_FUSED64) && BRIEF_FUSED64
+#define BRIEF_STASH_VEC4_ON 0
+#else
+#define BRIEF_STASH_VEC4_ON BRIEF_STASH_VEC4
+#endif
+BL_HD constexpr bool brief_stash_vec4_nt(int nt) { return BRIEF_STASH_VEC4_ON && nt == 8; }
+BL_HD constexpr bool brief_stash_vec4(const brief_siren_desc &d)
+{
+    return d.precision == BRIEF_PREC_F32 && brief_stash_vec4_nt((d.features + 31) / 32);
+}
+BL_HD constexpr int brief_stash_tile_off(bool vec4, int row, int s) { return vec4 ? (row >> 2) * 128 + s * 4 + (row & 3) : row * 32 + s; }
+BL_HD constexpr int64_t brief_stash_index(bool vec4, int FP, int64_t tile, int row, int s)
+{
+    return tile * FP * 32 + brief_stash_tile_off(vec4, row, s);
+}
diff --git a/brief_pytorch_amd/csrc/brief_lean.inc b/brief_pytorch_amd/csrc/brief_lean.inc
--- a/brief_pytorch_amd/csrc/brief_lean.inc
+++ b/brief_pytorch_amd/csrc/brief_lean.inc
@@ -383,7 +383,7 @@
 #pragma unroll
                 for (int c = 0; c < 4; ++c) pph[h][c] = 0.f;
                 if (h == 1 && !two) continue;
-                const int voff = (int)(((ht + h) * 32) * ((int64_t)FP * 4)) + ln * 4 + hi * 4 * 128;
+                const int voff = (int)(((ht + h) * 32) * ((int64_t)FP * 4)) + 4 * brief_stash_tile_off(false, 4 * hi, ln);
 #pragma unroll
                 for (int t = 0; t < MTW; ++t) {
                     if (!tv[t]) continue;
@@ -396,7 +396,7 @@
                             const __amdgpu_buffer_rsrc_t rz =
                                 __builtin_amdgcn_make_buffer_rsrc((void *)(a.Z + (int64_t)l * FP * npad), 0, stash_bytes, 0x00020000);
 #pragma unroll
-                            for (int r = 0; r < 16; ++r) bstore1(acc[h][t][r], rz, voff, (32 * mt + (r & 3) + 8 * (r >> 2)) * 128);
+                            for (int r = 0; r < 16; ++r) bstore1(acc[h][t][r], rz, voff, 4 * brief_stash_tile_off(false, 32 * mt + (r & 3) + 8 * (r >> 2), 0));
                         }
 #pragma unroll
                         for (int r = 0; r < 16; ++r) hv[r] = BRIEF_SIN_REV(acc[h][t][r]);
@@ -557,13 +557,13 @@
 #pragma unroll
             for (int h = 0; h < SH; ++h) {
                 if (h == 1 && !two) continue;
-                const int voff_s = (int)(((ht + h) * 32) * ((int64_t)FP * 4)) + ln * 4 + hi * 4 * 128;
+                const int voff_s = (int)(((ht + h) * 32) * ((int64_t)FP * 4)) + 4 * brief_stash_tile_off(false, 4 * hi, ln);
 #pragma unroll
                 for (int t = 0; t < MTW; ++t) {
                     if (!tv[t]) continue;
                     const int mt = wave + 4 * t;
 #pragma unroll
-                    for (int r = 0; r < 16; ++r) bstore1(acc[h][t][r], rd, voff_s, (32 * mt + (r & 3) + 8 * (r >> 2)) * 128);
+                    for (int r = 0; r < 16; ++r) bstore1(acc[h][t][r], rd, voff_s, 4 * brief_stash_tile_off(false, 32 * mt + (r & 3) + 8 * (r >> 2), 0));
                 }
             }
             lds_barrier();
@@ -600,7 +600,7 @@
 #pragma unroll
             for (int h = 0; h < SH; ++h) {
                 if (h == 1 && !two) continue;
-                const int voff_s = (int)(((ht + h) * 32) * ((int64_t)FP * 4)) + ln * 4 + hi * 4 * 128;
+                const int voff_s = (int)(((ht + h) * 32) * ((int64_t)FP * 4)) + 4 * brief_stash_tile_off(false, 4 * hi, ln);
 #pragma unroll
                 for (int t2 = 0; t2 < MTW; t2 += 2) {
                     float zr[2][16];
@@ -610,7 +610,7 @@
                         if (t < MTW && tv[t < MTW ? t : 0]) {
                             const int mt = wave + 4 * t;
 #pragma unroll
-                            for (int r = 0; r < 16; ++r) zr[u][r] = bload1s(rzp, voff_s, (32 * mt + (r & 3) + 8 * (r >> 2)) * 128);
+                            for (int r = 0; r < 16; ++r) zr[u][r] = bload1s(rzp, voff_s, 4 * brief_stash_tile_off(false, 32 * mt + (r & 3) + 8 * (r >> 2), 0));
                         }
                     }
 #pragma unroll
diff --git a/brief_pytorch_amd/csrc/brief_wgrad.inc b/brief_pytorch_amd/csrc/brief_wgrad.inc
--- a/brief_pytorch_amd/csrc/brief_wgrad.inc
+++ b/brief_pytorch_amd/csrc/brief_wgrad.inc
@@ -25,6 +25,9 @@
 #endif
 #ifndef BRIEF_WGRAD_FRAG_PIPE
 #define BRIEF_WGRAD_FRAG_PIPE 1
+#endif
+#ifndef BRIEF_WGRAD_BURST
+#define BRIEF_WGRAD_BURST 0
 #endif
 #ifndef BRIEF_WGRAD_FRAG_PIPE2
 #define BRIEF_WGRAD_FRAG_PIPE2 1
@@ -64,6 +67,8 @@
     constexpr int NLD = (QP * 8 + 511) / 512;
     constexpr int PANEL = QP * LDSW;
     constexpr bool FULL = (QP * 8) % 512 == 0;
+    constexpr bool V4 = !RTW && brief_stash_vec4_nt(NT);
+    static_assert(!V4 || (QT == 8 && FULL && BRIEF_WGRAD_STAGE_BIAS && BRIEF_WGRAD_FRAG_PIPE), "the vec4 stash layout is staged by the 8-tile pipelined loop");
     extern __shared__ __attribute__((aligned(16))) float smem[];
 
     const int tid = threadIdx.x;
@@ -128,9 +133,11 @@
 #define WG_ISSUE(cc)                                                                              \
     _Pragma("unroll") for (int i = 0; i < NLD; ++i) {                                             \
         const int e = tid + 512 * i;                                                              \
-        ra[i] = make_float4(0.f, 0.f, 0.f, 0.f);                                                  \
-        rb[i] = make_float4(0.f, 0.f, 0.f, 0.f);                                                  \
-        if (FULL || e < QP * 8) {                                                                 \
+        if constexpr (!FULL || RTW) {                       \
+            ra[i] = make_float4(0.f, 0.f, 0.f, 0.f);                                              \
+            rb[i] = make_float4(0.f, 0.f, 0.f, 0.f);                                              \
+        }                                                                                         \
+        if (FULL || e < QP * 8) {                                                              \
             if (!RTW || (e >> 3) < rows_m) ra[i] = bload4w(rsD, voffs[i], (int)((cc) * (FP * 128)));     \
             if (!RTW || (e >> 3) < rows_n) rb[i] = bload4w(rsZ, voffs[i], (int)((cc) * (FP * 128)));     \
         }                                                                                         \
@@ -138,7 +145,10 @@
 #define WG_STAGE_A(buf, i)                                                                        \
     {                                                                                             \
         const int e = tid + 512 * (i);                                                            \
-        if (FULL || e < QP * 8)                                                                   \
+        if constexpr (V4) {                                                                       \
+            float *p_ = smem + (buf) * 2 * PANEL + (e >> 5) * (4 * LDSW) + (e & 31);              \
+            p_[0] = ra[i].x; p_[LDSW] = ra[i].y; p_[2 * LDSW] = ra[i].z; p_[3 * LDSW] = ra[i].w;  \
+        } else if (FULL || e < QP * 8)                                                            \
             *reinterpret_cast<float4 *>(smem + (buf) * 2 * PANEL + (e >> 3) * LDSW + (e & 7) * 4) = ra[i]; \
     }
 #define WG_STAGE_B(buf, i)                                                                        \
@@ -148,15 +158,21 @@
             float4 h;                                                                             \
             h.x = BRIEF_SIN_REV(rb[i].x); h.y = BRIEF_SIN_REV(rb[i].y);    \
             h.z = BRIEF_SIN_REV(rb[i].z); h.w = BRIEF_SIN_REV(rb[i].w);                           \
-            *reinterpret_cast<float4 *>(smem + (buf) * 2 * PANEL + PANEL + (e >> 3) * LDSW + (e & 7) * 4) = h; \
+            if constexpr (V4) {                                                                   \
+                float *p_ = smem + (buf) * 2 * PANEL + PANEL + (e >> 5) * (4 * LDSW) + (e & 31);  \
+                p_[0] = h.x; p_[LDSW] = h.y; p_[2 * LDSW] = h.z; p_[3 * LDSW] = h.w;              \
+            } else                                                                                \
+                *reinterpret_cast<float4 *>(smem + (buf) * 2 * PANEL + PANEL + (e >> 3) * LDSW + (e & 7) * 4) = h; \
         }                                                                                         \
     }
+#define WG_BIAS_READ(P, i) (*reinterpret_cast<const float4 *>((P) + ((tid + 512 * (i)) >> 3) * LDSW + ((tid + 512 * (i)) & 7) * 4))
+#define WG_BIAS_V4(v_, i) { bsum[i] = __fmaf_rn(1.0f, ((v_).x + (v_).y) + ((v_).z + (v_).w), bsum[i]); }
 #define WG_BIAS_M(i, cm_) { bsum[i] = __fmaf_rn((cm_), (ra[i].x + ra[i].y) + (ra[i].z + ra[i].w), bsum[i]); }
 #define WG_BIAS(i) WG_BIAS_M(i, 1.0f)
     WG_ISSUE(c0)
 #pragma unroll
     for (int i = 0; i < NLD; ++i) { WG_STAGE_A(0, i) WG_STAGE_B(0, i) }
-    if (want_bias) {
+    if (!V4 && want_bias) {
 #pragma unroll
         for (int i = 0; i < NLD; ++i) WG_BIAS(i)
     }
@@ -311,7 +327,7 @@
             _Pragma("unroll") for (int i = 0; i < NLD; ++i)                                                            \
                 if ((i & 1) == ((gq_) & 1)) {                                                                          \
                     WG_STAGE_A(cur ^ 1, i) WG_STAGE_B(cur ^ 1, i)                                                      \
-                    if (SBIAS) WG_BIAS_M(i, cm_r)                                                                      \
+                    if (SBIAS && !V4) WG_BIAS_M(i, cm_r)                                                               \
                 }                                                                                                      \
         }
         if constexpr (BRIEF_WGRAD_FRAG_PIPE && WK == 1 && QT == 8) {
@@ -326,9 +342,23 @@
             WG_READ_FRAGS(3, af1, bf1)
             __builtin_amdgcn_sched_barrier(0);
             WG_MFMAS(af0, bf0)
-            WG_STAGE_NEXT(2)
-            WG_MFMAS(af1, bf1)
-            WG_STAGE_NEXT(3)
+            if constexpr (V4) {
+                float4 bv[NLD];
+#pragma unroll
+                for (int i = 0; i < NLD; ++i) bv[i] = WG_BIAS_READ(As, i);
+                if (BRIEF_WGRAD_BURST) __builtin_amdgcn_sched_barrier(0);
+                WG_STAGE_NEXT(2)
+                if (BRIEF_WGRAD_BURST) __builtin_amdgcn_sched_barrier(0);
+                WG_MFMAS(af1, bf1)
+                if (BRIEF_WGRAD_BURST) __builtin_amdgcn_sched_barrier(0);
+                WG_STAGE_NEXT(3)
+#pragma unroll
+                for (int i = 0; i < NLD; ++i) WG_BIAS_V4(bv[i], i)
+            } else {
+                WG_STAGE_NEXT(2)
+                WG_MFMAS(af1, bf1)
+                WG_STAGE_NEXT(3)
+            }
         } else if constexpr (BRIEF_WGRAD_FRAG_PIPE2 && WK == 2 && QT >= 4) {
             float4 af0[TM], bf0[TN], af1[TM], bf1[TN];
             WG_READ_FRAGS(wk, af0, bf0)
@@ -381,6 +411,8 @@
 #undef WG_STAGE_B
 #undef WG_BIAS
 #undef WG_BIAS_M
+#undef WG_BIAS_READ
+#undef WG_BIAS_V4
     if (WK > 1) {
         float *red = smem;
         float *redb = smem + (WK - 1) * NWv * TN * 1024;
diff --git a/brief_pytorch_amd/csrc/brief_wide.inc b/brief_pytorch_amd/csrc/brief_wide.inc
--- a/brief_pytorch_amd/csrc/brief_wide.inc
+++ b/brief_pytorch_amd/csrc/brief_wide.inc
@@ -89,7 +89,7 @@
     const float *headp = pk + brief_pk_head(d);
     const int64_t hstride = brief_pk_hidden_stride(d);
     const int plane_bytes = FP * 128;
-    const int voff = ln * 4 + hi * 512;
+    const int voff = 4 * brief_stash_tile_off(false, 4 * hi, ln);
     float *rec = a.rec + (((int64_t)blockIdx.x + a.rec_base) * 4 + wave) * (8 * TR + 32);
     if (TRAIN) {
         for (int e = lane; e < 8 * TR + 32; e += 64) rec[e] = 0.f;
@@ -186,7 +186,7 @@
                     for (int r = 0; r < 16; ++r) acc[0][t][r] = __builtin_amdgcn_fractf(acc[0][t][r]);
                     if (TRAIN) {
 #pragma unroll
-                        for (int r = 0; r < 16; ++r) bstore1(acc[0][t][r], rz, voff, (32 * mt + (r & 3) + 8 * (r >> 2)) * 128);
+                        for (int r = 0; r < 16; ++r) bstore1(acc[0][t][r], rz, voff, 4 * brief_stash_tile_off(false, 32 * mt + (r & 3) + 8 * (r >> 2), 0));
                     }
 #pragma unroll
                     for (int r = 0; r < 16; ++r) hv[r] = BRIEF_SIN_REV(acc[0][t][r]);
@@ -311,7 +311,7 @@
 #pragma unroll
                     for (int r = 0; r < 16; ++r) {
                         acc[0][t][r] = 0.f;
-                        if (tv[t]) acc[0][t][r] = bload1(rzl, voff, (32 * (wv + 4 * t) + (r & 3) + 8 * (r >> 2)) * 128);
+                        if (tv[t]) acc[0][t][r] = bload1(rzl, voff, 4 * brief_stash_tile_off(false, 32 * (wv + 4 * t) + (r & 3) + 8 * (r >> 2), 0));
                     }
                 }
 #pragma unroll
@@ -362,7 +362,7 @@
                     }
                     if (L - 2 >= 1) {
 #pragma unroll
-                        for (int r = 0; r < 16; ++r) bstore1(acc[0][t][r], rd, voff, (32 * mt + (r & 3) + 8 * (r >> 2)) * 128);
+                        for (int r = 0; r < 16; ++r) bstore1(acc[0][t][r], rd, voff, 4 * brief_stash_tile_off(false, 32 * mt + (r & 3) + 8 * (r >> 2), 0));
                         wide_store_image(iplane(L - 2), mt, lane, acc[0][t]);
                     }
                 }
@@ -402,7 +402,7 @@
 #pragma unroll
                         for (int r = 0; r < 16; ++r) {
                             zr[u][r] = 0.f;
-                            if (t2 + u < MTW && tv[t]) zr[u][r] = bload1s(rzp, voff, (32 * (wv + 4 * t) + (r & 3) + 8 * (r >> 2)) * 128);
+                            if (t2 + u < MTW && tv[t]) zr[u][r] = bload1s(rzp, voff, 4 * brief_stash_tile_off(false, 32 * (wv + 4 * t) + (r & 3) + 8 * (r >> 2), 0));
                         }
                     }
 #pragma unroll
@@ -419,7 +419,7 @@
                     for (int t = 0; t < MTW; ++t) {
                         if (!tv[t]) continue;
 #pragma unroll
-                        for (int r = 0; r < 16; ++r) bstore1(acc[0][t][r], rdout, voff, (32 * (wv + 4 * t) + (r & 3) + 8 * (r >> 2)) * 128);
+                        for (int r = 0; r < 16; ++r) bstore1(acc[0][t][r], rdout, voff, 4 * brief_stash_tile_off(false, 32 * (wv + 4 * t) + (r & 3) + 8 * (r >> 2), 0));
                         wide_store_image(iplane(l - 1), wv + 4 * t, lane, acc[0][t]);
                     }
                 } else {
diff --git a/brief_pytorch_amd/csrc/brief_x3.inc b/brief_pytorch_amd/csrc/brief_x3.inc
--- a/brief_pytorch_amd/csrc/brief_x3.inc
+++ b/brief_pytorch_amd/csrc/brief_x3.inc
@@ -321,7 +321,7 @@
 #pragma unroll
                 for (int c = 0; c < 4; ++c) pph[h][c] = 0.f;
                 if (h == 1 && !two) continue;
-                const int voff = (int)(((ht + h) * 32) * (FP * 4)) + ln * 4 + hi * 4 * 128;
+                const int voff = (int)(((ht + h) * 32) * (FP * 4)) + 4 * brief_stash_tile_off(false, 4 * hi, ln);
 #pragma unroll
                 for (int t = 0; t < 2; ++t) {
                     const int mt = wm + 4 * t;
@@ -333,7 +333,7 @@
                         const __amdgpu_buffer_rsrc_t rz =
                             __builtin_amdgcn_make_buffer_rsrc((void *)(a.Z + (int64_t)l * FP * npad), 0, stash_bytes, 0x00020000);
 #pragma unroll
-                        for (int r = 0; r < 16; ++r) bstore1s(acc[h][t][r], rz, voff, (32 * mt + (r & 3) + 8 * (r >> 2)) * 128);
+                        for (int r = 0; r < 16; ++r) bstore1s(acc[h][t][r], rz, voff, 4 * brief_stash_tile_off(false, 32 * mt + (r & 3) + 8 * (r >> 2), 0));
                         }
 #pragma unroll
                         for (int r = 0; r < 16; ++r) hv[r] = BRIEF_SIN_REV(acc[h][t][r]);
@@ -490,12 +490,12 @@
 #pragma unroll
             for (int h = 0; h < 2; ++h) {
                 if (h == 1 && !two) continue;
-                const int voff_s = (int)(((ht + h) * 32) * (FP * 4)) + ln * 4 + hi * 4 * 128;
+                const int voff_s = (int)(((ht + h) * 32) * (FP * 4)) + 4 * brief_stash_tile_off(false, 4 * hi, ln);
 #pragma unroll
                 for (int t = 0; t < 2; ++t) {
                     const int mt = wm + 4 * t;
 #pragma unroll
-                    for (int r = 0; r < 16; ++r) bstore1s(acc[h][t][r], rd, voff_s, (32 * mt + (r & 3) + 8 * (r >> 2)) * 128);
+                    for (int r = 0; r < 16; ++r) bstore1s(acc[h][t][r], rd, voff_s, 4 * brief_stash_tile_off(false, 32 * mt + (r & 3) + 8 * (r >> 2), 0));
                 }
             }
             STAMP(7)
@@ -519,12 +519,12 @@
             for (int h = 0; h < 2; ++h) {
                 if (h == 1 && !two) continue;
                 float zr[2][16];
-                const int voff_s = (int)(((ht + h) * 32) * (FP * 4)) + ln * 4 + hi * 4 * 128;
+                const int voff_s = (int)(((ht + h) * 32) * (FP * 4)) + 4 * brief_stash_tile_off(false, 4 * hi, ln);
 #pragma unroll
                 for (int t = 0; t < 2; ++t) {
                     const int mt = wm + 4 * t;
 #pragma unroll
-                    for (int r = 0; r < 16; ++r) zr[t][r] = bload1s(rzp, voff_s, (32 * mt + (r & 3) + 8 * (r >> 2)) * 128);
+                    for (int r = 0; r < 16; ++r) zr[t][r] = bload1s(rzp, voff_s, 4 * brief_stash_tile_off(false, 32 * mt + (r & 3) + 8 * (r >> 2), 0));
                 }
 #pragma unroll
                 for (int t = 0; t < 2; ++t)
```
